# helloybz/CLANE

Hardware: AMD Instinct MI355X
Metric: embedding-update iters/sec (Jacobi sweeps of Z <- X + gamma*P*Z, P frozen) (higher is better)
Workload: dtype f32; 1 GPU; R-MAT |V|=2000000 |E|=40000000 d=256 f32, gamma=0.76, CosineSimilarity (reference mode), seeds 3/4

## Files before the change

### clane_amd/_hip.py

```python
from __future__ import annotations

import abc
import ctypes as C
import os
import threading
from pathlib import Path
from typing import Optional

import torch

LIB_NAME = "libclane_hip.so"
LIB_PATH = Path(__file__).resolve().parent / LIB_NAME
ABI_VERSION = 5

SCORE_REFERENCE, SCORE_PER_EDGE, SCORE_RAW_DOT = 0, 1, 2
SPMM_SINKS_UNTOUCHED = 1
SPMM_TABLE_BEYOND_CACHE = 2
OWNED_EPILOGUE_AHEAD = 1 << 16
SCORE_FUSE_SOFTMAX = 1
SCORE_MODES = {"reference": SCORE_REFERENCE, "per_edge": SCORE_PER_EDGE, "raw_dot": SCORE_RAW_DOT}

_p, _i64, _i32 = C.c_void_p, C.c_int64, C.c_int32

SIGNATURES = {
    "clane_abi_version": (C.c_int, []),
    "clane_last_error": (C.c_char_p, []),
    "clane_build_info": (C.c_char_p, []),
    "clane_xcc_ids": (C.c_int, [_p, _i64, _i32, _p]),
    "clane_check_csr": (C.c_int, [_p, _p, _i64, _i64, _i64, _p, _p]),
    "clane_spmm_partials_len": (_i64, [_i64, _i64]),
    "clane_reduce_ws_len": (_i64, []),
    "clane_reduce_partials": (C.c_int, [_p, _i64, _p, _p, _p]),
    "clane_spmm_split_slab_len": (_i64, [_i64, _i32]),
    "clane_spmm_class_slab_len": (_i64, [_i64, _i32]),
    "clane_device_alloc": (C.c_int, [_i64, C.POINTER(_p)]),
    "clane_device_alloc_contiguous": (C.c_int, [_i64, C.POINTER(_p)]),
    "clane_device_free": (C.c_int, [_p]),
    "clane_ipc_export": (C.c_int, [_p, _p]),
    "clane_ipc_open": (C.c_int, [_p, C.POINTER(_p)]),
    "clane_ipc_close": (C.c_int, [_p]),
}
IPC_HANDLE_BYTES = 64
for _s in ("f32", "f64", "bf16"):
    SIGNATURES[f"clane_row_sqnorm_{_s}"] = (C.c_int, [_p, _i64, _i32, _i64, _p, _p])
    SIGNATURES[f"clane_edge_score_{_s}"] = (
        C.c_int, [_p, _p, _i64, _i64, _p, _i64, _i32, _i32, _p, _p, _p, _i32, _i64, _p, _i64, _p])
    _g = C.c_double if _s == "f64" else C.c_float
    SIGNATURES[f"clane_spmm_update_{_s}"] = (
        C.c_int, [_p, _p, _p, _i64, _i64, _p, _i64, _p, _i64, _g, _p, _i64, _i32, _i64, _i32, _p, _p, _p])
    SIGNATURES[f"clane_spmm_update_long_{_s}"] = (
        C.c_int, [_p, _p, _p, _p, _i64, _i32, _i64, _p, _i64, _p, _i64, _g, _p, _i64, _i32, _p, _p, _p])
    SIGNATURES[f"clane_spmm_update_split_{_s}"] = (
        C.c_int,
        [_p, _p, _p, _p, _p, _p, _i64, _i64, _i64, _i64, _p, _i64, _p, _i64, _g, _p, _i64, _i32, _p, _p, _p, _p])
    SIGNATURES[f"clane_spmm_update_class_{_s}"] = (
        C.c_int,
        [_p, _p, _p, _p, _p, _i64, _i32, _p, _p, _i64, _i64, _p, _i64, _p, _i64, _g, _p, _i64, _i32, _i32, _p, _p, _p, _p])
    SIGNATURES[f"clane_edge_score_class_{_s}"] = (
        C.c_int, [_p, _p, _p, _p, _p, _p, _i64, _i32, _p, _p, _i64, _i64, _p, _i64, _i32, _i32, _p, _p, _p, _i32, _p, _p])
    SIGNATURES[f"clane_gather_rows_{_s}"] = (C.c_int, [_p, _i64, _p, _i64, _i32, _p, _i64, _p])
    SIGNATURES[f"clane_l1_distance_{_s}"] = (C.c_int, [_p, _i64, _p, _i64, _i64, _i32, _p, _p, _p, _p])
SIGNATURES["clane_spmm_update_owned_f32"] = (
    C.c_int, [_p, _p, _p, _i32, _i64, _p, _i64, _p, _i64, C.c_float, _p, _i64, _i32, _i32, _p, _p])
SIGNATURES["clane_spmm_update_tiles_f32"] = (
    C.c_int, [_p, _p, _p, _i64, _i64, _p, _i64, _p, _i64, C.c_float, _p, _i64, _i32, _i32, _i64, _i32, _p, _i64, _p])
SIGNATURES["clane_spmm_update_class_tiles_f32"] = (
    C.c_int, [_p, _p, _p, _p, _p, _i64, _i32, _p, _p, _i64, _i64, _i64, _p, _i64, _p, _i64, C.c_float, _p, _i64, _i32, _i32,
              _i32, _p, _p, _i64, _p])
SIGNATURES["clane_spmm_update_owned_tiles_f32"] = (
    C.c_int, [_p, _p, _p, _i32, _i64, _p, _i64, _p, _i64, C.c_float, _p, _i64, _i32, _i32, _i32, _p, _i64, _p])
SIGNATURES["clane_row_weight_f32"] = SIGNATURES["clane_row_weight_f64"] = (C.c_int, [_p, _p, _i64, _p, _p, _p])
SIGNATURES["clane_spmm_update_rw_f32"] = (
    C.c_int, [_p, _p, _p, _i64, _i64, _p, _i64, _p, _i64, C.c_float, _p, _i64, _i32, _i64, _i32, _p, _p])
SIGNATURES["clane_spmm_update_tiles_rw_f32"] = SIGNATURES["clane_spmm_update_tiles_f32"]
SIGNATURES["clane_spmm_update_class_rw_f32"] = (
    C.c_int, [_p, _p, _p, _p, _p, _p, _i64, _i32, _p, _p, _i64, _i64, _p, _i64, _p, _i64, C.c_float, _p, _i64, _i32, _i32, _p,
              _p, _p])
SIGNATURES["clane_spmm_update_class_tiles_rw_f32"] = (
    C.c_int, [_p, _p, _p, _p, _p, _p, _i64, _i32, _p, _p, _i64, _i64, _i64, _p, _i64, _p, _i64, C.c_float, _p, _i64, _i32,
              _i32, _i32, _p, _p, _i64, _p])
SIGNATURES["clane_spmm_update_owned_rw_f32"] = (
    C.c_int, [_p, _p, _p, _p, _i32, _i64, _p, _i64, _p, _i64, C.c_float, _p, _i64, _i32, _i32, _p, _p])
SIGNATURES["clane_spmm_update_owned_tiles_rw_f32"] = (
    C.c_int, [_p, _p, _p, _p, _i32, _i64, _p, _i64, _p, _i64, C.c_float, _p, _i64, _i32, _i32, _i32, _p, _i64, _p])
for _s in ("f32", "f64"):
    SIGNATURES[f"clane_degree_weighted_sums_{_s}"] = (C.c_int, [_p, _p, _p, _i64, _p, _p, _p])
    SIGNATURES[f"clane_edge_score_finalize_{_s}"] = (C.c_int, [_p, _p, _i64, _i64, _i32, _p, _p, _p, _p])
    SIGNATURES[f"clane_segment_softmax_{_s}"] = (C.c_int, [_p, _i64, _p, _i64, _i64, _p, _i64, _p])
    SIGNATURES[f"clane_pair_cosine_{_s}"] = (C.c_int, [_p, _i64, _p, _i64, _i64, _i32, _p, _p, _p])
    SIGNATURES[f"clane_edge_score_pair_{_s}"] = (
        C.c_int, [_p, _p, _i64, _i64, _p, _i64, _p, _i64, _i32, _p, _i32, _i64, _p, _i64, _p])
    SIGNATURES[f"clane_edge_score_class_pair_{_s}"] = (
        C.c_int, [_p, _p, _p, _p, _p, _p, _i64, _i32, _p, _p, _i64, _i64, _p, _i64, _p, _i64, _i32, _p, _i32, _p, _p])
for _s in ("f32", "f64", "bf16"):
    SIGNATURES[f"clane_project_rows_{_s}"] = (C.c_int, [_p, _i64, _i32, _i64, _p, _p, _i64, _p])
    SIGNATURES[f"clane_pair_project_{_s}"] = (C.c_int, [_p, _i64, _i32, _i64, _p, _p, _i64, _p, _p, _p, _p])
    SIGNATURES[f"clane_pair_grad_{_s}"] = (C.c_int, [_p, _i64, _i32, _i64, _p, _p, _i64, _p, _p, _p, _p, _p, _p, _p])
for _s in ("f32", "f64"):
    SIGNATURES[f"clane_pair_loss_{_s}"] = (C.c_int, [_p, _p, _i64, _i32, _p, _p, _p, _p, _p, _p, _p])
    SIGNATURES[f"clane_adam_step_{_s}"] = (C.c_int, [_p, _p, _p, _p, _i64, C.c_double, _p, _p, _p])
SIGNATURES["clane_pair_grad_ws_len"] = (_i64, [_i64, _i32])
RANK_MAX_K = 32
for _s in ("f32", "f64", "bf16"):
    SIGNATURES[f"clane_rank_scores_{_s}"] = (
        C.c_int, [_p, _i64, _p, _i64, _i64, _i32, _p, _i64, _i32, _p, _p, _p, _p, _p, _i32, _i32, _i32, _p, _p, _p])
    SIGNATURES[f"clane_pair_score_{_s}"] = (C.c_int, [_p, _i64, _p, _i64, _i64, _i32, _p, _p, _i64, _i32, _p, _p, _p, _p])
    SIGNATURES[f"clane_rank_count_{_s}"] = (
        C.c_int, [_p, _i64, _p, _i64, _i64, _i32, _p, _p, _i64, _i32, _p, _p, _p, _p, _p, _i32, _i32, _p, _p, _p])
for _s in ("f32", "f64"):
    SIGNATURES[f"clane_rank_merge_{_s}"] = (C.c_int, [_p, _p, _i64, _i32, _i32, _p, _p, _p])
SIGNATURES["clane_pair_labels"] = (C.c_int, [_p, _p, _i64, _p, _p, _i64, _p, _p])
PROBE_MAX_CLASSES = 64
PROBE_WRITE_G, PROBE_WRITE_PRED = 1, 2
PROBE_PRED_TOPK = 4
for _s in ("f32", "f64", "bf16"):
    SIGNATURES[f"clane_probe_forward_{_s}"] = (
        C.c_int, [_p, _i64, _i32, _i64, _p, _p, _i64, _p, _i64, _p, _p, _i32, _i32, _i32, _p, _p, _p, _p, _i64, _p])
    SIGNATURES[f"clane_probe_grad_{_s}"] = (C.c_int, [_p, _i64, _i32, _i64, _p, _i64, _p, _i32, _p, _p, _p, _p])
    SIGNATURES[f"clane_probe_forward_ovr_{_s}"] = (
        C.c_int, [_p, _i64, _i32, _i64, _p, _p, _i64, _p, _i64, _p, _p, _p, _i32, _i32, _i32, _i32, _p, _p, _p, _p, _i64, _p])
    SIGNATURES[f"clane_probe_predict_{_s}"] = (
        C.c_int, [_p, _i64, _i32, _i64, _p, _i64, _p, _p, _p, _i32, _i32, _i32, _i32, _p, _p, _p, _p])
PREDICT_SIGMOID, PREDICT_WRITE_PROBA = 1, 2
PREDICT_MAX_TOP = 8
SIGNATURES["clane_probe_loss_ws_len"] = (_i64, [_i64, _i32])
SIGNATURES["clane_probe_grad_ws_len"] = (_i64, [_i64, _i32, _i32])
for _s in ("f32", "f64", "bf16"):
    SIGNATURES[f"clane_kmeans_assign_{_s}"] = (
        C.c_int, [_p, _i64, _i32, _i64, _p, _i64, _p, _p, _i32, _i32, _p, _i64, _p, _i64, _p])
    SIGNATURES[f"clane_kmeans_update_{_s}"] = (
        C.c_int, [_p, _i64, _i32, _i64, _p, _p, _i64, _i32, _i32, _p, _p, _p, _p, _p])
SIGNATURES["clane_kmeans_update_ws_len"] = (_i64, [_i64, _i32, _i32, _i32])
MIXTURE_MAX_COMPONENTS = 64
MIXTURE_WRITE_RESP, MIXTURE_WRITE_ASSIGN = 1, 2
for _s in ("f32", "f64", "bf16"):
    SIGNATURES[f"clane_mixture_estep_{_s}"] = (
        C.c_int, [_p, _i64, _i32, _i64, _p, _i64, _p, _p, _p, _i32, _i32, _i32, _p, _p, _p, _p, _i64, _p])
    SIGNATURES[f"clane_mixture_mstep_{_s}"] = (C.c_int, [_p, _i64, _i32, _i64, _p, _i64, _p, _p, _i32, _p, _p, _p, _p])
SIGNATURES["clane_mixture_ll_ws_len"] = (_i64, [_i64, _i32])
SIGNATURES["clane_mixture_mstep_ws_len"] = (_i64, [_i64, _i32, _i32])
for _s in ("f32", "f64", "bf16"):
    _g = C.c_double if _s == "f64" else C.c_float
    SIGNATURES[f"clane_embed_rows_{_s}"] = (
        C.c_int, [_p, _p, _i64, _p, _i64, _p, _i64, _i64, _i32, _i32, _p, _p, _p, _i64, _g, _i32, _i32, _i32, _p, _i64,
                  _p, _p, _p, _p])

PCA_ACCUMULATE = 1
for _s in ("f32", "f64", "bf16"):
    SIGNATURES[f"clane_column_sums_{_s}"] = (C.c_int, [_p, _i64, _i32, _i64, _p, _i64, _i32, _p, _p, _p])
    SIGNATURES[f"clane_gram_{_s}"] = (C.c_int, [_p, _i64, _i32, _i64, _p, _i64, _p, _i32, _p, _p, _p])
    SIGNATURES[f"clane_project_affine_{_s}"] = (C.c_int, [_p, _i64, _i32, _i64, _p, _i64, _p, _p, _i32, _p, _i64, _p])
SIGNATURES["clane_column_sums_ws_len"] = (_i64, [_i64, _i32])
SIGNATURES["clane_gram_ws_len"] = (_i64, [_i64, _i32])
CSR_MAX_L = 512
SIGNATURES["clane_csr_spmm_segment"] = (C.c_int, [])
SIGNATURES["clane_csr_spmm_ws_len"] = (_i64, [_i64, _i64, _i32])
SIGNATURES["clane_csr_spmm_f32"] = (
    C.c_int, [_p, _p, _p, _i64, _i64, _p, _i64, _i64, _i32, _p, _p, _p, _p, _p, _i64, _i64, _p, _i64, _p, _i64, _p])
SIGNATURES["clane_csr_row_sums_f32"] = (C.c_int, [_p, _p, _i64, _i64, _p, _p, _p, _i64, _i64, _p, _i64, _p, _p])
TSNE_MAX_POINTS = 65536
TSNE_FORCES_KL, TSNE_FORCES_CACHED = 1, 2
for _s in ("f32", "bf16"):
    SIGNATURES[f"clane_tsne_sqdist_{_s}"] = (C.c_int, [_p, _i64, _i32, _i64, _p, _i64, _p, _p, _p, _p])
SIGNATURES["clane_tsne_affinities_f32"] = (C.c_int, [_p, _i64, C.c_float, _p, _p])
SIGNATURES["clane_tsne_symmetrize_ws_len"] = (_i64, [_i64])
SIGNATURES["clane_tsne_symmetrize_f32"] = (C.c_int, [_p, _i64, _p, _p])
SIGNATURES["clane_tsne_forces_f32"] = (C.c_int, [_p, _p, _i64, _i32, _p, _p])
# ... 390 lines not shown

    def mixture_mstep_ws_len(self, n: int, K: int, d: int) -> int:
        raise NotImplementedError(f"{type(self).__name__} has no mixture_mstep_ws_len")

    def mixture_mstep(self, Z, d: int, rows, mean, resp, ws, S, nk):
        raise NotImplementedError(f"{type(self).__name__} has no mixture_mstep")

    def column_sums_ws_len(self, n: int, d: int) -> int:
        raise NotImplementedError(f"{type(self).__name__} has no column_sums_ws_len")

    def column_sums(self, Z, d: int, rows, ws, sums, accumulate: bool = False):
        raise NotImplementedError(f"{type(self).__name__} has no column_sums")

    def gram_ws_len(self, n: int, d: int) -> int:
        raise NotImplementedError(f"{type(self).__name__} has no gram_ws_len")

    def gram(self, Z, d: int, rows, mu, ws, G, accumulate: bool = False):
        raise NotImplementedError(f"{type(self).__name__} has no gram")

    def project_affine(self, Z, d: int, rows, mu, W, Y):
        raise NotImplementedError(f"{type(self).__name__} has no project_affine")

    def csr_spmm_segment(self) -> int:
        raise NotImplementedError(f"{type(self).__name__} has no csr_spmm_segment")

    def csr_spmm_ws_len(self, n_rows: int, nnz: int, l: int) -> int:
        raise NotImplementedError(f"{type(self).__name__} has no csr_spmm_ws_len")

    def csr_spmm(self, S, B, l: int, out, a=None, s=None, ws=None):
        raise NotImplementedError(f"{type(self).__name__} has no csr_spmm")

    def csr_row_sums(self, S, sums, ws=None):
        raise NotImplementedError(f"{type(self).__name__} has no csr_row_sums")

    def tsne_sqdist(self, Z, d: int, rows, mu, sq, D):
        raise NotImplementedError(f"{type(self).__name__} has no tsne_sqdist")

    def tsne_affinities(self, D, perplexity: float, beta):
        raise NotImplementedError(f"{type(self).__name__} has no tsne_affinities")

    def tsne_symmetrize_ws_len(self, n: int) -> int:
        raise NotImplementedError(f"{type(self).__name__} has no tsne_symmetrize_ws_len")

    def tsne_symmetrize(self, P, partials):
        raise NotImplementedError(f"{type(self).__name__} has no tsne_symmetrize")

    def tsne_forces(self, P, Y, F, kl: bool = True, cached: bool = False):
        raise NotImplementedError(f"{type(self).__name__} has no tsne_forces")

    def tsne_step(self, F, Y, alpha: float, momentum: float, lr: float, plogp: float, V, G, Y_next, stats):
        raise NotImplementedError(f"{type(self).__name__} has no tsne_step")

    def knn_sqdist(self, Z, d: int, rows, mu, sq, ids, sqdist, n_slabs: int = 1, cand_ids=None, cand_sqdist=None):
        raise NotImplementedError(f"{type(self).__name__} has no knn_sqdist")

    def tsne_nn_affinities(self, sqdist, ids, perplexity: float, p, beta):
        raise NotImplementedError(f"{type(self).__name__} has no tsne_nn_affinities")

    def tsne_nn_plogp(self, rowptr, val, row_plogp):
        raise NotImplementedError(f"{type(self).__name__} has no tsne_nn_plogp")

    def tsne_nn_attract(self, rowptr, cols, val, Y, F, kl: bool = True):
        raise NotImplementedError(f"{type(self).__name__} has no tsne_nn_attract")

    def tsne_repulse(self, Y, F):
        raise NotImplementedError(f"{type(self).__name__} has no tsne_repulse")

    def silhouette_norms(self, Z, d: int, order, mu, metric: str, nrm):
        raise NotImplementedError(f"{type(self).__name__} has no silhouette_norms")

    def silhouette_sums(self, Z, d: int, order, seg, mu, nrm, metric: str, p0: int, p1: int, S):
        raise NotImplementedError(f"{type(self).__name__} has no silhouette_sums")

    def has_spmm_owned(self, dtype, d: int) -> bool:
        return False

    def make_owned_plan(self, plan: dict, chunk: int, device):
        raise NotImplementedError(f"{type(self).__name__} has no make_owned_plan")

    def spmm_update_owned(self, colidx, P, plan, block_threads: int, row0: int, Z_old, X, gamma: float, Z_new, d: int,
                          partials, beyond_cache: bool = False, loads: int = 0, ahead: bool = False):
        raise NotImplementedError(f"{type(self).__name__} has no spmm_update_owned")

    def has_spmm_tiles(self, dtype, d: int, tile_cols: int) -> bool:
        return False

    owned_epilogue_ahead = False

    def spmm_update_tiles(self, rowptr, colidx, P, nrows: int, row0: int, Z_old, X, gamma: float, Z_new, d: int,
                          tile_cols: int, long_threshold: int, partials, partials_stride: int,
                          sinks_untouched: bool = False, beyond_cache: bool = False):
        raise NotImplementedError(f"{type(self).__name__} has no spmm_update_tiles")

    def spmm_update_class_tiles(self, colidx, P, item_e0, item_len, item_slot, items_per_block: int, class_rows, slot_ptr,
                                n_slots: int, row0: int, Z_old, X, gamma: float, Z_new, d: int, tile_cols: int, slab,
                                partials, partials_stride: int, beyond_cache: bool = False):
        raise NotImplementedError(f"{type(self).__name__} has no spmm_update_class_tiles")

    def spmm_update_owned_tiles(self, colidx, P, plan, block_threads: int, row0: int, Z_old, X, gamma: float, Z_new,
                                d: int, tile_cols: int, partials, partials_stride: int, beyond_cache: bool = False,
                                loads: int = 0, ahead: bool = False):
        raise NotImplementedError(f"{type(self).__name__} has no spmm_update_owned_tiles")

    def has_row_weight(self, dtype) -> bool:
        return False

    def row_weight(self, rowptr, P, nrows: int, w, mixed):
        raise NotImplementedError(f"{type(self).__name__} has no row_weight")

    def bind(self, method: str, *args, **kwargs):
        fn = getattr(self, method)
        return lambda: fn(*args, **kwargs)

    def embed_rows(self, rowptr, colidx, X_new, Z, table_rows: int, d: int, mode: int, sums2, sq, S, gamma: float,
                   tolerence: int, max_rounds: int, Z_out, rounds, delta, P_out=None, flags: int = 0):
        raise NotImplementedError(f"{type(self).__name__} has no embed_rows")


class HipKernels(KernelBackend):

    owned_epilogue_ahead = True

    def __init__(self, lib: Optional[C.CDLL] = None):
        self.lib = lib if lib is not None else load_library()
        self._tls = threading.local()

    def _invoke(self, fn, what: str, *cargs):
        rec = getattr(self._tls, "recording", None)
        if rec is not None:
            rec.append((fn, cargs, what))
        else:
            self._check(fn(*cargs), what)

    def bind(self, method: str, *args, **kwargs):
        self._tls.recording = []
        try:
            getattr(self, method)(*args, **kwargs)
            (fn, cargs, what), = self._tls.recording
        finally:
            self._tls.recording = None
        check = self._check
        return lambda: check(fn(*cargs), what)

    def _check(self, rc: int, what: str):
        if rc != 0:
            raise ClaneHipError(f"{what} failed ({rc}): {self.lib.clane_last_error().decode()}")

    @staticmethod
    def _stream(t: torch.Tensor):
        if not t.is_cuda:
            raise ClaneHipError("HipKernels needs tensors in GPU memory (got a CPU tensor); there is no CPU path")
        return torch.cuda.current_stream(t.device).cuda_stream

    def _fn(self, base: str, dtype: torch.dtype):
        try:
            return getattr(self.lib, f"{base}_{_SUFFIX[dtype]}")
        except KeyError:
            raise TypeError(f"{base}: unsupported dtype {dtype}") from None

    def spmm_partials_len(self, nrows: int, n_long: int) -> int:
        return int(self.lib.clane_spmm_partials_len(nrows, n_long))

    def xcc_ids(self, n_blocks: int, block_threads: int = 256, device=None) -> torch.Tensor:
        out = torch.full((n_blocks,), -1, dtype=torch.int32, device=device if device is not None else "cuda")
        self._check(self.lib.clane_xcc_ids(out.data_ptr(), n_blocks, block_threads, self._stream(out)), "clane_xcc_ids")
        return out
# ... 256 lines not shown
        return _vec(w, torch.float32, "row_weight")

    def spmm_update_rw(self, rowptr, colidx, row_weight, nrows: int, row0: int, Z_old, X, gamma: float, Z_new, d: int,
                       long_threshold: int, partials, sinks_untouched: bool = False, beyond_cache: bool = False):
        zo, ldz, xp, ldx, zn, ldo = self._tables("spmm_update_rw", Z_old, X, Z_new, f32_only=True)
        self._invoke(self.lib.clane_spmm_update_rw_f32, "clane_spmm_update_rw",
                     _vec(rowptr, torch.int64, "rowptr"), _vec(colidx, torch.int32, "colidx"),
                     self._row_weights("spmm_update_rw", row_weight, nrows), nrows, row0, zo, ldz, xp, ldx, gamma, zn, ldo,
                     d, long_threshold, self._spmm_flags(sinks_untouched, beyond_cache),
                     _vec(partials, torch.float64, "partials"), self._stream(Z_old))

    def spmm_update_tiles_rw(self, rowptr, colidx, row_weight, nrows: int, row0: int, Z_old, X, gamma: float, Z_new,
                             d: int, tile_cols: int, long_threshold: int, partials, partials_stride: int,
                             sinks_untouched: bool = False, beyond_cache: bool = False):
        zo, ldz, xp, ldx, zn, ldo = self._tile_args("spmm_update_tiles_rw", Z_old, X, Z_new, d, tile_cols, partials,
                                                    partials_stride, self.spmm_partials_len(nrows, 0))
        self._invoke(self.lib.clane_spmm_update_tiles_rw_f32, "clane_spmm_update_tiles_rw",
                     _vec(rowptr, torch.int64, "rowptr"), _vec(colidx, torch.int32, "colidx"),
                     self._row_weights("spmm_update_tiles_rw", row_weight, nrows), nrows, row0, zo, ldz, xp, ldx, gamma,
                     zn, ldo, d, tile_cols, long_threshold, self._spmm_flags(sinks_untouched, beyond_cache),
                     _vec(partials, torch.float64, "partials"), partials_stride, self._stream(Z_old))

    def spmm_update_class_rw(self, colidx, row_weight, item_e0, item_len, item_slot, item_row, items_per_block: int,
                             class_rows, slot_ptr, row0: int, Z_old, X, gamma: float, Z_new, d: int, slab, partials,
                             beyond_cache: bool = False):
        zo, ldz, xp, ldx, zn, ldo = self._tables("spmm_update_class_rw", Z_old, X, Z_new, f32_only=True)
        n_blocks = self._item_blocks("spmm_update_class_rw", items_per_block, item_e0, item_len, item_slot, item_row)
        rows = int(class_rows.max()) + 1 if class_rows.numel() else 0
        self._invoke(self.lib.clane_spmm_update_class_rw_f32, "clane_spmm_update_class_rw",
                     _vec(colidx, torch.int32, "colidx"), self._row_weights("spmm_update_class_rw", row_weight, rows),
                     _vec(item_e0, torch.int64, "item_e0"), _vec(item_len, torch.int32, "item_len"),
                     _vec(item_slot, torch.int32, "item_slot"), _vec(item_row, torch.int32, "item_row"), n_blocks,
                     items_per_block, _vec(class_rows, torch.int32, "class_rows"), _vec(slot_ptr, torch.int64, "slot_ptr"),
                     class_rows.numel(), row0, zo, ldz, xp, ldx, gamma, zn, ldo, d,
                     self._spmm_flags(beyond_cache=beyond_cache), _vec(slab, torch.float32, "slab"),
                     _vec(partials, torch.float64, "partials"), self._stream(Z_old))

    def spmm_update_class_tiles_rw(self, colidx, row_weight, item_e0, item_len, item_slot, item_row, items_per_block: int,
                                   class_rows, slot_ptr, n_slots: int, row0: int, Z_old, X, gamma: float, Z_new, d: int,
                                   tile_cols: int, slab, partials, partials_stride: int, beyond_cache: bool = False):
        zo, ldz, xp, ldx, zn, ldo = self._tile_args("spmm_update_class_tiles_rw", Z_old, X, Z_new, d, tile_cols, partials,
                                                    partials_stride, class_rows.numel())
        n_blocks = self._item_blocks("spmm_update_class_tiles_rw", items_per_block, item_e0, item_len, item_slot, item_row)
        if slab.numel() < -(-d // tile_cols) * self.spmm_class_slab_len(n_slots, tile_cols):
            raise ValueError("spmm_update_class_tiles_rw: the slab does not hold every tile's chunk sums")
        rows = int(class_rows.max()) + 1 if class_rows.numel() else 0
        self._invoke(self.lib.clane_spmm_update_class_tiles_rw_f32, "clane_spmm_update_class_tiles_rw",
                     _vec(colidx, torch.int32, "colidx"), self._row_weights("spmm_update_class_tiles_rw", row_weight, rows),
                     _vec(item_e0, torch.int64, "item_e0"), _vec(item_len, torch.int32, "item_len"),
                     _vec(item_slot, torch.int32, "item_slot"), _vec(item_row, torch.int32, "item_row"), n_blocks,
                     items_per_block, _vec(class_rows, torch.int32, "class_rows"), _vec(slot_ptr, torch.int64, "slot_ptr"),
                     class_rows.numel(), n_slots, row0, zo, ldz, xp, ldx, gamma, zn, ldo, d, tile_cols,
                     self._spmm_flags(beyond_cache=beyond_cache), _vec(slab, torch.float32, "slab"),
                     _vec(partials, torch.float64, "partials"), partials_stride, self._stream(Z_old))

    def spmm_update_owned_rw(self, colidx, row_weight, plan: OwnedPlan, block_threads: int, row0: int, Z_old, X,
                             gamma: float, Z_new, d: int, partials, beyond_cache: bool = False, loads: int = 0,
                             ahead: bool = False):
        zo, ldz, xp, ldx, zn, ldo = self._tables("spmm_update_owned_rw", Z_old, X, Z_new, f32_only=True)
        self._owned_plan_fits("spmm_update_owned_rw", plan, d, colidx, colidx, row0, Z_old, X, Z_new, partials)
        self._invoke(self.lib.clane_spmm_update_owned_rw_f32, "clane_spmm_update_owned_rw",
                     _vec(colidx, torch.int32, "colidx"),
                     self._row_weights("spmm_update_owned_rw", row_weight, plan.max_row + 1),
                     C.cast(C.pointer(plan.c), _p), _vec(plan.seg_row, torch.int32, "seg_row"), int(block_threads), row0,
                     zo, ldz, xp, ldx, gamma, zn, ldo, d,
                     self._spmm_flags(beyond_cache=beyond_cache, loads=loads, ahead=ahead),
                     _vec(partials, torch.float64, "partials"), self._stream(Z_old))

    def spmm_update_owned_tiles_rw(self, colidx, row_weight, plan: OwnedPlan, block_threads: int, row0: int, Z_old, X,
                                   gamma: float, Z_new, d: int, tile_cols: int, partials, partials_stride: int,
                                   beyond_cache: bool = False, loads: int = 0, ahead: bool = False):
        zo, ldz, xp, ldx, zn, ldo = self._tile_args("spmm_update_owned_tiles_rw", Z_old, X, Z_new, d, tile_cols, partials,
                                                    partials_stride, plan.max_part + 1)
        if not self.has_spmm_owned(torch.float32, tile_cols):
            raise ValueError(f"spmm_update_owned_tiles_rw: no owned instance for tiles of {tile_cols} columns")
        self._owned_plan_fits("spmm_update_owned_tiles_rw", plan, tile_cols, colidx, colidx, row0, Z_old, X, Z_new)
        self._invoke(self.lib.clane_spmm_update_owned_tiles_rw_f32, "clane_spmm_update_owned_tiles_rw",
                     _vec(colidx, torch.int32, "colidx"),
                     self._row_weights("spmm_update_owned_tiles_rw", row_weight, plan.max_row + 1),
                     C.cast(C.pointer(plan.c), _p), _vec(plan.seg_row, torch.int32, "seg_row"), int(block_threads), row0,
                     zo, ldz, xp, ldx, gamma, zn, ldo, d, tile_cols,
                     self._spmm_flags(beyond_cache=beyond_cache, loads=loads, ahead=ahead),
                     _vec(partials, torch.float64, "partials"), partials_stride, self._stream(Z_old))

    def reduce_partials(self, partials, n: int, ws, out):
        self._invoke(self.lib.clane_reduce_partials, "clane_reduce_partials",
                     _vec(partials, torch.float64, "partials"), n, _vec(ws, torch.float64, "ws"),
                     _vec(out, torch.float64, "out"), self._stream(out))

    def l1_distance(self, A, B, d: int, ws, out, sq_a: Optional[torch.Tensor] = None):
        ap, lda = _mat(A, "A")
        bp, ldb = _mat(B, "B")
        self._check(self._fn("clane_l1_distance", A.dtype)(
            ap, lda, bp, ldb, A.shape[0], d, self._sq_arg(sq_a, A.dtype), _vec(ws, torch.float64, "ws"),
            _vec(out, torch.float64, "out"), self._stream(A)), "clane_l1_distance")

    def gather_rows(self, src, idx, d: int, dst):
        sp, lds = _mat(src, "src")
        dp, ldd = _mat(dst, "dst")
        self._invoke(self._fn("clane_gather_rows", src.dtype), "clane_gather_rows",
                     sp, lds, _vec(idx, torch.int32, "idx"), idx.numel(), d, dp, ldd, self._stream(src))

    def project_rows(self, Z, d: int, W, Y):
        zp, ldz = _mat(Z, "Z")
        yp, ldy = _mat(Y, "Y")
        acc = acc_dtype(Z.dtype)
        if tuple(W.shape) != (2 * d, d):
            raise ValueError(f"project_rows: W must be [2d, d] = [{2 * d}, {d}], got {tuple(W.shape)}")
        if Y.dtype != acc or Y.shape[0] < Z.shape[0]:
            raise ValueError(f"project_rows: Y must be {acc} with at least {Z.shape[0]} rows")
        self._check(self._fn("clane_project_rows", Z.dtype)(
            zp, Z.shape[0], d, ldz, _vec(W, acc, "W"), yp, ldy, self._stream(Z)), "clane_project_rows")

    def edge_score_pair(self, rowptr, colidx, nrows: int, row0: int, S, N, d: int, scores, long_threshold: int = 0,
                        long_rows=None, fuse_softmax: bool = False):
        sp, lds = _mat(S, "S")
        np_, ldn = _mat(N, "N")
        if S.dtype != N.dtype:
            raise ValueError("edge_score_pair: S and N must share a dtype")
        n_long = 0 if long_rows is None else long_rows.numel()
        self._check(self._fn("clane_edge_score_pair", S.dtype)(
            _vec(rowptr, torch.int64, "rowptr"), _vec(colidx, torch.int32, "colidx"), nrows, row0, sp, lds, np_, ldn, d,
            _vec(scores, S.dtype, "scores"), SCORE_FUSE_SOFTMAX if fuse_softmax else 0, long_threshold,
            None if n_long == 0 else _vec(long_rows, torch.int32, "long_rows"), n_long,
            self._stream(S)), "clane_edge_score_pair")

    def edge_score_class_pair(self, rowptr, colidx, item_e0, item_len, item_slot, item_row, items_per_block: int,
                              class_rows, slot_ptr, row0: int, S, N, d: int, scores, stats=None,
                              fuse_softmax: bool = False, n_slots: Optional[int] = None, row_parts: int = 1):
        sp, lds = _mat(S, "S")
        np_, ldn = _mat(N, "N")
        if S.dtype != N.dtype:
            raise ValueError("edge_score_class_pair: S and N must share a dtype")
        n_blocks = self._item_blocks("edge_score_class_pair", items_per_block, item_e0, item_len, item_slot, item_row)
        if fuse_softmax and (stats is None or stats.numel() < 2 * (int(slot_ptr[-1]) if n_slots is None else n_slots)):
            raise ValueError("edge_score_class_pair: stats needs 2 elements per slot")
        self._check(self._fn("clane_edge_score_class_pair", S.dtype)(
            _vec(rowptr, torch.int64, "rowptr"), _vec(colidx, torch.int32, "colidx"),
            _vec(item_e0, torch.int64, "item_e0"), _vec(item_len, torch.int32, "item_len"),
            _vec(item_slot, torch.int32, "item_slot"), _vec(item_row, torch.int32, "item_row"),
            n_blocks, items_per_block, _vec(class_rows, torch.int32, "class_rows"),
            _vec(slot_ptr, torch.int64, "slot_ptr"), class_rows.numel(), row0, sp, lds, np_, ldn, d,
            _vec(scores, S.dtype, "scores"),
            (SCORE_FUSE_SOFTMAX | ((max(1, min(255, int(row_parts))) & 0xff) << 8)) if fuse_softmax else 0,
            None if stats is None else _vec(stats, S.dtype, "stats"), self._stream(S)), "clane_edge_score_class_pair")

    @staticmethod
    def _pairs(src, dst, what: str) -> int:
        if src.numel() != dst.numel():
            raise ValueError(f"{what}: src and dst must have one entry per pair")
        return src.numel()

    def _pair_mats(self, A, Bm, B: int, d: int, acc, what: str):
        for t, name in ((A, "A"), (Bm, "Bm")):
            if t.dtype != acc or not t.is_contiguous() or t.numel() < B * d:
                raise ValueError(f"{what}: {name} must be a contiguous {acc} tensor of at least B * d elements")
        return A.data_ptr(), Bm.data_ptr()

    def pair_project(self, Z, d: int, src, dst, W, A, Bm):
        zp, ldz = _mat(Z, "Z")
        acc = acc_dtype(Z.dtype)
        B = self._pairs(src, dst, "pair_project")
        if tuple(W.shape) != (2 * d, d):
            raise ValueError(f"pair_project: W must be [2d, d] = [{2 * d}, {d}], got {tuple(W.shape)}")
        ap, bp = self._pair_mats(A, Bm, B, d, acc, "pair_project")
        self._invoke(self._fn("clane_pair_project", Z.dtype), "clane_pair_project",
# ... 616 lines not shown
```

### clane_amd/blocks.py

```python
from __future__ import annotations

import itertools
from dataclasses import dataclass
from typing import NamedTuple, Optional

import numpy as np
import torch


class ClassItems(NamedTuple):
    rows: torch.Tensor
    slot_ptr: torch.Tensor
    e0: torch.Tensor
    len: torch.Tensor
    slot: torch.Tensor
    row: torch.Tensor
    items_per_block: int

    @classmethod
    def upload(cls, items: dict, rows: np.ndarray, device) -> "ClassItems":
        up = lambda name: torch.from_numpy(items[name]).to(device)
        return cls(torch.from_numpy(rows.astype(np.int32)).to(device), up("slot_ptr"), up("e0"), up("len"), up("slot"),
                   up("row"), items["items_per_block"])


class SplitRows(NamedTuple):
    rows: torch.Tensor
    seg_ptr: torch.Tensor
    seg_row: torch.Tensor


class OwnedRows(NamedTuple):
    plan: object
    rest: Optional[ClassItems]
    n_rest: int


@dataclass(frozen=True)
class PartialLayout:
    main: int
    mid: int
    hub: int
    split: int
    klass: int
    end: int

    @classmethod
    def of(cls, row_pass: int, n_mid: int, n_hub: int, n_split: int, n_class: int, length: int) -> "PartialLayout":
        starts = list(itertools.accumulate((row_pass, n_mid, n_hub, n_split, n_class), initial=0))
        assert starts[-1] == length, (starts, length)
        return cls(*starts)

    def owned(self, n_rest: int) -> int:
        return self.klass + n_rest

    def owned_slots(self, n_rest: int, n_owned: int) -> np.ndarray:
        assert self.owned(n_rest) + n_owned == self.end, (self, n_rest, n_owned)
        return self.owned(n_rest) - self.klass + np.arange(n_owned)


@dataclass
class BlockRows:
    long: Optional[torch.Tensor]
    k1_long: Optional[torch.Tensor]
    mid: Optional[torch.Tensor]
    hub: Optional[torch.Tensor]
    partials: PartialLayout
    split: Optional[SplitRows] = None
    klass: Optional[ClassItems] = None
    n_slots: int = 0
    owned: Optional[OwnedRows] = None
    owned_inputs: Optional[tuple] = None
```

### clane_amd/csrc/clane_abi.hip

```cpp
#include "../../include/clane_hip.h"

#include <hip/hip_runtime.h>

#include <climits>
#include <cstdarg>
#include <cstdio>
#include <cstring>

#include "build_p.h"
#include "content_pca.h"
#include "edge_score.h"
#include "device_utils.h"
#include "kmeans.h"
#include "label_predict.h"
#include "label_probe.h"
#include "multilabel_probe.h"
#include "new_rows.h"
#include "link_eval.h"
#include "link_rank.h"
#include "mixture.h"
#include "pair_train.h"
#include "projection.h"
#include "sparse_rows.h"
#include "spmm_update.h"
#include "silhouette.h"
#include "tsne.h"
#include "tsne_nn.h"

namespace {

using namespace clane;

thread_local char g_err[512] = "";

int fail(int code, const char *fmt, ...) {
    va_list ap;
    va_start(ap, fmt);
    vsnprintf(g_err, sizeof(g_err), fmt, ap);
    va_end(ap);
    return code;
}

int check_launch(const char *what) {
    const hipError_t e = hipGetLastError();
    if (e != hipSuccess) return fail(CLANE_ERR_LAUNCH, "%s: %s", what, hipGetErrorString(e));
    return CLANE_OK;
}

constexpr int kReduceGrid = 1024;
constexpr int64_t kReduceWs = 2 * kReduceGrid + 2;
#ifndef CLANE_LONG_U
#define CLANE_LONG_U CLANE_SPMM_U
#endif
#ifndef CLANE_SUBROW_U32
#define CLANE_SUBROW_U32 4
#endif
#ifndef CLANE_CLASS_U16B
#define CLANE_CLASS_U16B 4
#endif
#ifndef CLANE_CLASS_U32
#define CLANE_CLASS_U32 6
#endif
#ifndef CLANE_LONG_WAVES
#define CLANE_LONG_WAVES 16
#endif
constexpr int kLongWaves = CLANE_LONG_WAVES;
#ifndef CLANE_ROWS_PER_BLOCK
#define CLANE_ROWS_PER_BLOCK 32
#endif

inline bool aligned16(const void *p) { return (reinterpret_cast<uintptr_t>(p) & 15u) == 0; }

#ifndef CLANE_TARGET_GRID
#define CLANE_TARGET_GRID 32768
#endif
inline int rows_per_block(int64_t nrows) {
    const int64_t r = ceil_div(ceil_div(nrows, CLANE_TARGET_GRID), kWavesPerBlock) * kWavesPerBlock;
    return int(r < CLANE_ROWS_PER_BLOCK ? CLANE_ROWS_PER_BLOCK : r > kMaxRowsPerBlock ? kMaxRowsPerBlock : r);
}
inline int row_grid(int64_t nrows) { return int(ceil_div(nrows > 0 ? nrows : 1, rows_per_block(nrows))); }

inline int grid_for_waves(int64_t nwaves_wanted) {
    int64_t g = ceil_div(nwaves_wanted, kWavesPerBlock);
    if (g > kMaxGrid) g = kMaxGrid;
    if (g < 1) g = 1;
    return int(g);
}

struct Layout {
    bool vec;
    int lpr;
};

template <typename T>
Layout pick_layout(int d, std::initializer_list<const void *> ptrs, std::initializer_list<int64_t> lds) {
    constexpr int KV = Elem<T>::kVec;
    bool vec = true;
    for (const void *p : ptrs) vec = vec && aligned16(p);
    for (int64_t ld : lds) vec = vec && (ld % KV == 0);
    Layout L;
    L.vec = vec;
    if (vec) {
        const int packs = int(ceil_div(d, KV));
        L.lpr = packs <= 8 ? 8 : packs <= 16 ? 16 : packs <= 32 ? 32 : 64;
    } else {
        L.lpr = d <= 4 ? 4 : d <= 16 ? 16 : 64;
    }
    return L;
}

template <typename T, typename F>
void dispatch_layout(const Layout &L, F &&f) {
    constexpr int KV = Elem<T>::kVec;
    if (L.vec) {
        switch (L.lpr) {
            case 8: f.template operator()<KV, 8>(); break;
            case 16: f.template operator()<KV, 16>(); break;
            case 32: f.template operator()<KV, 32>(); break;
            default: f.template operator()<KV, 64>(); break;
        }
    } else {
        switch (L.lpr) {
            case 4: f.template operator()<1, 4>(); break;
            case 16: f.template operator()<1, 16>(); break;
            default: f.template operator()<1, 64>(); break;
        }
    }
}

template <typename T>
Mirror<T> make_mirror(const clane_mirror_t *m) {
    if (m == nullptr || m->row_ptr == nullptr) return Mirror<T>{nullptr, nullptr, nullptr, 0};
    return Mirror<T>{m->row_ptr, m->slot, reinterpret_cast<T *const *>(m->bufs), m->ld};
}
inline const void *mirror_alignment_probe(const clane_mirror_t *m, const void *aligned) {
    return (m && m->row_ptr && !m->aligned16) ? reinterpret_cast<const void *>(uintptr_t(1)) : aligned;
}
inline bool mirror_ok(const clane_mirror_t *m, int d) {
    return m == nullptr || m->row_ptr == nullptr || (m->slot != nullptr && m->bufs != nullptr && m->ld >= d);
}

// ... 375 lines not shown
            "spmm_update_split: null pointer");
    REQUIRE(!t.aliased(), "spmm_update_split: Z_new must not alias Z_old");
    REQUIRE(aligned16(slab), "spmm_update_split: slab must be 16-byte aligned");
    const Layout L = t.layout(d);
    const int64_t ld_slab = ceil_div(d, 8) * 8;
    dispatch_layout<T>(L, [&]<int VEC, int LPR>() {
        constexpr int U = VEC > 1 ? CLANE_LONG_U : 4;
        spmm_split_segment_kernel<T, PT, VEC, LPR, U, kLongWaves>
            <<<unsigned(n_segments), kLongWaves * kWave, 0, (hipStream_t)stream>>>(
                rowptr, colidx, P, split_rows, seg_ptr, seg_row, edges_per_segment, t.Z_old, t.ldz, d, slab, ld_slab);
        spmm_class_combine_kernel<T, VEC, LPR>
            <<<unsigned(ceil_div(n_split, kWave / LPR)), kCombineWaves * kWave, 0, (hipStream_t)stream>>>(
                split_rows, seg_ptr, n_split, row0, slab, ld_slab, t.Z_old, t.ldz, t.X, t.ldx, t.gamma, t.Z_new, t.ldo, d,
                t.mir(), false, delta_partials);
    });
    return check_launch("spmm_update_split");
}

template <typename T, typename PT, bool FUSED, bool UNIFORM = false>
int spmm_update_class_impl(const char *what, const int32_t *colidx, const PT *P, const int64_t *item_e0,
                           const int32_t *item_len, const int32_t *item_slot, int64_t n_blocks, int32_t items_per_block,
                           const int32_t *class_rows, const int64_t *slot_ptr, int64_t n_rows, int64_t n_slots,
                           int64_t row0, const Tables<T> &t, Tiles tiles, int32_t flags,
                           typename Elem<T>::acc_t *slab, double *delta_partials, void *stream,
                           const int32_t *item_row = nullptr) {
    const int32_t d = t.d;
    constexpr int kPad = FUSED ? 8 : 1;
    REQUIRE(t.mirror_complete(), "%s: incomplete mirror descriptor", what);
    REQUIRE(n_blocks >= 0 && n_blocks <= INT32_MAX - (FUSED ? 8 : 0) && n_rows >= 0 && n_rows <= INT32_MAX &&
                n_slots >= 0 && row0 >= 0 && d > 0, "%s: bad shape", what);
    if constexpr (FUSED) REQUIRE_TILES(T, d, tiles, what, true, "");
    REQUIRE(items_per_block >= kWavesPerBlock && items_per_block <= kMaxItemsPerBlock,
            "%s: items_per_block must be in [%d, %d]", what, kWavesPerBlock, kMaxItemsPerBlock);
    REQUIRE(t.wide_enough(), "%s: leading dimension < d", what);
    const int n_tiles = tile_count(d, tiles.cols);
    REQUIRE(tiles.part_stride >= (n_tiles > 1 ? n_rows : 0), "%s: the tiles' partials overlap", what);
    if (n_rows == 0) return CLANE_OK;
    REQUIRE(colidx && P && item_e0 && item_len && item_slot && class_rows && slot_ptr && t.present() && slab &&
                delta_partials, "%s: null pointer", what);
    if constexpr (UNIFORM) REQUIRE(item_row && t.mirror == nullptr, "%s: per-row weights need item_row and no mirror", what);
    REQUIRE(!t.aliased(), "%s: Z_new must not alias Z_old", what);
    REQUIRE(aligned16(slab), "%s: slab must be 16-byte aligned", what);
    const Layout L = t.layout(tiles.cols);
    if constexpr (FUSED) REQUIRE(L.vec, "%s: the tables must allow 16-byte packs", what);
    const int64_t ld_slab = ceil_div(tiles.cols, 8) * 8;
    const int64_t slab_stride = n_slots * ld_slab;
    const int chunk_blocks = int(ceil_div(n_blocks, kPad) * kPad);
    const bool beyond = (flags & CLANE_SPMM_TABLE_BEYOND_CACHE) != 0;
    REQUIRE(int64_t(n_tiles) * chunk_blocks <= INT32_MAX, "%s: grid too large", what);
    dispatch_layout<T>(L, [&]<int VEC, int LPR>() {
        constexpr int U = VEC > 1 ? CLANE_LONG_U : 4;
        constexpr int kDeepU = (LPR == 32 && VEC == 4 && sizeof(T) == 4) ? CLANE_CLASS_U32
                               : (LPR == 16 && VEC == 8 && sizeof(T) == 2) ? CLANE_CLASS_U16B : 0;
        const unsigned chunk_grid = unsigned(n_tiles) * unsigned(chunk_blocks);
        const int combine_blocks = int(ceil_div(n_rows, kWave / LPR));
        const unsigned combine_grid = unsigned(n_tiles) * unsigned(combine_blocks);
        auto chunks = [&]<int CU>() {
            if constexpr (!FUSED)
                spmm_class_chunk_kernel<T, PT, VEC, LPR, CU, UNIFORM><<<chunk_grid, kBlock, 0, (hipStream_t)stream>>>(
                    colidx, P, item_e0, item_len, item_slot, items_per_block, t.Z_old, t.ldz, d, slab, ld_slab, item_row);
            else if constexpr (VEC > 1)
                spmm_class_chunk_tiles_kernel<T, PT, VEC, LPR, CU, UNIFORM><<<chunk_grid, kBlock, 0, (hipStream_t)stream>>>(
                    colidx, P, item_e0, item_len, item_slot, int(n_blocks), items_per_block, t.Z_old, t.ldz, d, slab,
                    ld_slab, slab_stride, TileGrid{chunk_blocks, tiles.cols, 0}, item_row);
        };
        if (n_blocks > 0 && kDeepU > 0 && beyond) chunks.template operator()<(kDeepU > 0 ? kDeepU : U)>();
        else if (n_blocks > 0) chunks.template operator()<U>();
        if constexpr (!FUSED)
            spmm_class_combine_kernel<T, VEC, LPR><<<combine_grid, kCombineWaves * kWave, 0, (hipStream_t)stream>>>(
                class_rows, slot_ptr, n_rows, row0, slab, ld_slab, t.Z_old, t.ldz, t.X, t.ldx, t.gamma, t.Z_new, t.ldo, d,
                t.mir(), beyond, delta_partials);
        else if constexpr (VEC > 1)
            spmm_class_combine_tiles_kernel<T, VEC, LPR><<<combine_grid, kCombineWaves * kWave, 0, (hipStream_t)stream>>>(
                class_rows, slot_ptr, n_rows, row0, slab, ld_slab, slab_stride, t.Z_old, t.ldz, t.X, t.ldx, t.gamma,
                t.Z_new, t.ldo, d, beyond, TileGrid{combine_blocks, tiles.cols, tiles.part_stride}, delta_partials);
    });
    return check_launch(what);
}

constexpr int64_t kOwnedLdsReserve = 1024;
constexpr int64_t kLdsPerCU = 160 * 1024;
constexpr int64_t kLdsDefaultLimit = 64 * 1024;

template <typename T, typename PT, bool UNIFORM = false>
int spmm_update_owned_impl(const char *what, const int32_t *colidx, const PT *P, const clane_owned_plan_t *plan,
                           int32_t block_threads, int64_t row0, const Tables<T> &t, Tiles tiles, bool fused, int32_t flags,
                           double *delta_partials, void *stream, const int32_t *seg_row = nullptr) {
    using A = typename Elem<T>::acc_t;
    const int32_t d = tiles.cols;
    if (fused) REQUIRE_TILES(T, t.d, tiles, what, tiles.part_stride >= 0, ", the partials' stride >= 0");
    REQUIRE(plan, "spmm_update_owned: null plan");
    REQUIRE(plan->n_groups >= 0 && row0 >= 0 && d > 0, "spmm_update_owned: bad shape");
    REQUIRE(plan->n_steps >= 1 && plan->n_steps <= kOwnedMaxSteps, "spmm_update_owned: n_steps must be in [1, %d]",
            kOwnedMaxSteps);
    REQUIRE(plan->chunk >= kWave && plan->chunk % kWave == 0, "spmm_update_owned: chunk must be a positive multiple of 64");
    REQUIRE(block_threads >= kWave && block_threads <= kOwnedMaxBlock && block_threads % kWave == 0,
            "spmm_update_owned: block_threads must be a multiple of 64 in [64, %d]", kOwnedMaxBlock);
    REQUIRE(t.wide_enough(), "spmm_update_owned: leading dimension < d");
    REQUIRE(plan->max_batch_vrows >= 0, "spmm_update_owned: negative max_batch_vrows");
    if (plan->n_groups == 0) return CLANE_OK;
    REQUIRE(colidx && P && plan->grp_bat_ptr && plan->bat_vrow_ptr && plan->bat_row_ptr && plan->bat_seg_ptr &&
                plan->seg_e0 && plan->seg_len && plan->seg_vrow && plan->row_id && plan->row_part && plan->row_vptr &&
                t.present() && delta_partials,
            "spmm_update_owned: null pointer");
    if constexpr (UNIFORM) REQUIRE(seg_row, "spmm_update_owned: per-row weights need seg_row");
    REQUIRE(!t.aliased(), "spmm_update_owned: Z_new must not alias Z_old");
    const Layout L = t.layout(d);
    REQUIRE(L.vec && (L.lpr == 32 || L.lpr == 64) && d <= L.lpr * Elem<T>::kVec,
            "spmm_update_owned: no instance for d=%d with these operands (16-byte packs, 17..64 packs per row)", d);
    const int64_t lds = int64_t(plan->max_batch_vrows) * L.lpr * Elem<T>::kVec * int64_t(sizeof(A));
    REQUIRE(lds + kOwnedLdsReserve <= kLdsPerCU, "spmm_update_owned: %lld virtual rows per batch need %lld bytes of LDS",
            (long long)plan->max_batch_vrows, (long long)lds);
    const OwnedPlan op{plan->grp_bat_ptr, plan->bat_vrow_ptr, plan->bat_row_ptr, plan->bat_seg_ptr, plan->seg_e0,
                       plan->seg_len, plan->seg_vrow, plan->row_id, plan->row_part, plan->row_vptr, plan->n_steps,
                       plan->chunk};
    const bool beyond = (flags & CLANE_SPMM_TABLE_BEYOND_CACHE) != 0;
    int rc = CLANE_OK;
    auto launch = [&]<int VEC, int LPR, int U>() {
        auto *kernel = spmm_owned_kernel<T, PT, VEC, LPR, U, UNIFORM>;
        if (lds > kLdsDefaultLimit) {
            static int64_t granted = 0;
            if (lds > granted) {
                const hipError_t e = hipFuncSetAttribute(reinterpret_cast<const void *>(kernel),
                                                         hipFuncAttributeMaxDynamicSharedMemorySize, int(lds));
                if (e != hipSuccess) {
                    rc = fail(CLANE_ERR_LAUNCH, "spmm_update_owned: %lld bytes of LDS: %s", (long long)lds,
                              hipGetErrorString(e));
                    return;
                }
                granted = lds;
            }
        }
        kernel<<<unsigned(plan->n_groups), unsigned(block_threads), size_t(lds), (hipStream_t)stream>>>(
            colidx, P, op, row0, t.Z_old, t.ldz, t.X, t.ldx, t.gamma, t.Z_new, t.ldo, t.d, tiles.cols, tiles.part_stride,
            (flags & CLANE_OWNED_EPILOGUE_AHEAD) != 0, beyond, delta_partials, seg_row);
    };
    constexpr int KV = Elem<T>::kVec;
    const int asked = (flags >> 8) & 0xff;
    REQUIRE(asked == 0 || asked == 8 || asked == 12 || (L.lpr == 32 && asked == 6),
            "spmm_update_owned: no instance with %d row loads in flight", asked);
    const int loads = asked ? asked : (L.lpr == 32 && beyond) ? CLANE_CLASS_U32 : CLANE_LONG_U;
    if (L.lpr == 32) {
        if (loads == 6) launch.template operator()<KV, 32, 6>();
        else if (loads == 12) launch.template operator()<KV, 32, 12>();
        else launch.template operator()<KV, 32, 8>();
    } else {
        if (loads == 12) launch.template operator()<KV, 64, 12>();
        else launch.template operator()<KV, 64, 8>();
    }
    if (rc != CLANE_OK) return rc;
    return check_launch(what);
}

template <typename T>
int l1_distance(const T *A, int64_t lda, const T *B, int64_t ldb, int64_t nrows, int32_t d,
                typename Elem<T>::acc_t *sq_a, double *ws, double *out, void *stream) {
    REQUIRE(nrows >= 0 && d > 0 && lda >= d && ldb >= d, "l1_distance: bad shape");
    REQUIRE(ws && out, "l1_distance: null workspace/output");
    REQUIRE(nrows == 0 || (A && B), "l1_distance: null pointer");
    const Layout L = pick_layout<T>(d, {A, B}, {lda, ldb});
    if (sq_a != nullptr) {
        const Layout LA = pick_layout<T>(d, {A}, {lda});
        REQUIRE(LA.vec == L.vec && LA.lpr == L.lpr,
                "l1_distance: sq_a needs B as aligned as A (the lane layout of row_sqnorm on A)");
    }
    int grid = 1;
    dispatch_layout<T>(L, [&]<int VEC, int LPR>() {
        grid = grid_for_waves(ceil_div(nrows > 0 ? nrows : 1, (kWave / LPR) * stream_rows(LPR)));
        if (grid > kReduceGrid) grid = kReduceGrid;
        l1_distance_kernel<T, VEC, LPR><<<grid, kBlock, 0, (hipStream_t)stream>>>(A, lda, B, ldb, nrows, d, sq_a, ws);
    });
    reduce_fixed_kernel<<<1, 1024, 0, (hipStream_t)stream>>>(ws, grid, grid, 1, out);
    return check_launch("l1_distance");
}

template <typename T>
int gather_rows(const T *src, int64_t lds, const int32_t *idx, int64_t n, int32_t d, T *dst, int64_t ldd, void *stream) {
    REQUIRE(n >= 0 && d > 0 && lds >= d && ldd >= d, "gather_rows: bad shape");
    if (n == 0) return CLANE_OK;
    REQUIRE(src && idx && dst, "gather_rows: null pointer");
    const Layout L = pick_layout<T>(d, {src, dst}, {lds, ldd});
    dispatch_layout<T>(L, [&]<int VEC, int LPR>() {
        const int grid = grid_for_waves(ceil_div(n, kWave / LPR));
        gather_rows_kernel<T, VEC, LPR><<<grid, kBlock, 0, (hipStream_t)stream>>>(src, lds, idx, n, d, dst, ldd);
    });
    return check_launch("gather_rows");
}

template <typename T>
int pair_cosine(const T *A, int64_t lda, const T *B, int64_t ldb, int64_t nrows, int32_t d,
                typename Elem<T>::acc_t *out, double *ws, void *stream) {
    REQUIRE(nrows >= 0 && d > 0 && lda >= d && ldb >= d, "pair_cosine: bad shape");
    if (nrows == 0) return CLANE_OK;
    REQUIRE(A && B && out && ws, "pair_cosine: null pointer");
    const Layout L = pick_layout<T>(d, {A, B}, {lda, ldb});
    int grid = 1;
    dispatch_layout<T>(L, [&]<int VEC, int LPR>() {
        grid = grid_for_waves(ceil_div(nrows, kWave / LPR));
        if (grid > kReduceGrid) grid = kReduceGrid;
        pair_dot_kernel<T, VEC, LPR><<<grid, kBlock, 0, (hipStream_t)stream>>>(A, lda, B, ldb, nrows, d, out, ws);
    });
    double *sums2 = ws + 2 * kReduceGrid;
    reduce_fixed_kernel<<<1, 1024, 0, (hipStream_t)stream>>>(ws, grid, grid, 2, sums2);
    int sgrid = int(ceil_div(nrows, kBlock));
    if (sgrid > kMaxGrid) sgrid = kMaxGrid;
    pair_scale_kernel<typename Elem<T>::acc_t><<<sgrid, kBlock, 0, (hipStream_t)stream>>>(out, nrows, sums2);
    return check_launch("pair_cosine");
}

template <typename T, typename A>
int pair_project(const T *Z, int64_t table_rows, int32_t d, int64_t ldz, const int32_t *src, const int32_t *dst,
                 int64_t B, const A *W, A *PA, A *PB, void *stream) {
    REQUIRE(table_rows >= 0 && B >= 0 && d > 0 && d <= 32768 && ldz >= d, "pair_project: bad shape rows=%lld B=%lld d=%d ldz=%lld",
            (long long)table_rows, (long long)B, d, (long long)ldz);
    if (B == 0) return CLANE_OK;
    REQUIRE(Z && src && dst && W && PA && PB, "pair_project: null pointer");
    const int n_tiles = int(ceil_div(int64_t(d), int64_t(kProjBN)));
    const int64_t blocks = ceil_div(B, int64_t(kProjBM)) * n_tiles;
    REQUIRE(blocks <= INT32_MAX, "pair_project: %lld pairs is too many for one launch", (long long)B);
    pair_project_kernel<T, A><<<dim3(unsigned(blocks), 2), kBlock, 0, (hipStream_t)stream>>>(
        Z, table_rows, d, ldz, src, dst, B, W, PA, PB, n_tiles);
    return check_launch("pair_project");
}

template <typename A>
int pair_loss(const A *PA, const A *PB, int64_t B, int32_t d, const uint8_t *linked, const A *u, A *g, uint8_t *mask,
              double *ws, double *stats, void *stream) {
    REQUIRE(B >= 0 && d > 0, "pair_loss: bad shape B=%lld d=%d", (long long)B, d);
    REQUIRE(ws && stats, "pair_loss: null workspace/output");
    REQUIRE(B == 0 || (PA && PB && linked && u && g && mask), "pair_loss: null pointer");
    int grid = int(ceil_div(B > 0 ? B : 1, kBlock / kPairLanes));
// ... 898 lines not shown
                                      const float *X, int64_t ldx, float gamma, float *Z_new, int64_t ldo, int32_t d,
                                      int32_t tile_cols, int32_t flags, float *slab, double *delta_partials,
                                      int64_t partials_tile_stride, void *stream) {
    return spmm_update_class_impl<float, float, true>("spmm_update_class_tiles", colidx, P, item_e0, item_len, item_slot,
                                                      n_blocks, items_per_block, class_rows, slot_ptr, n_rows, n_slots,
                                                      row0, TABLES(float), Tiles{tile_cols, partials_tile_stride}, flags,
                                                      slab, delta_partials, stream);
}
int clane_spmm_update_owned_tiles_f32(const int32_t *colidx, const float *P, const clane_owned_plan_t *plan,
                                      int32_t block_threads, int64_t row0, const float *Z_old, int64_t ldz,
                                      const float *X, int64_t ldx, float gamma, float *Z_new, int64_t ldo, int32_t d,
                                      int32_t tile_cols, int32_t flags, double *delta_partials,
                                      int64_t partials_tile_stride, void *stream) {
    return spmm_update_owned_impl<float, float>("spmm_update_owned_tiles", colidx, P, plan, block_threads, row0,
                                                TABLES(float), Tiles{tile_cols, partials_tile_stride}, true, flags,
                                                delta_partials, stream);
}
int clane_row_weight_f32(const int64_t *rowptr, const float *P, int64_t nrows, float *row_weight, int32_t *mixed,
                         void *stream) {
    return row_weights<float>(rowptr, P, nrows, row_weight, mixed, stream);
}
int clane_row_weight_f64(const int64_t *rowptr, const double *P, int64_t nrows, double *row_weight, int32_t *mixed,
                         void *stream) {
    return row_weights<double>(rowptr, P, nrows, row_weight, mixed, stream);
}
int clane_spmm_update_rw_f32(const int64_t *rowptr, const int32_t *colidx, const float *row_weight, int64_t nrows,
                             int64_t row0, const float *Z_old, int64_t ldz, const float *X, int64_t ldx, float gamma,
                             float *Z_new, int64_t ldo, int32_t d, int64_t long_threshold, int32_t flags,
                             double *delta_partials, void *stream) {
    return spmm_update_impl<float, float, false, true>("spmm_update_rw", rowptr, colidx, row_weight, nrows, row0,
                                                       TABLES(float), Tiles{d, 0}, long_threshold, flags, delta_partials,
                                                       stream);
}
int clane_spmm_update_tiles_rw_f32(const int64_t *rowptr, const int32_t *colidx, const float *row_weight, int64_t nrows,
                                   int64_t row0, const float *Z_old, int64_t ldz, const float *X, int64_t ldx, float gamma,
                                   float *Z_new, int64_t ldo, int32_t d, int32_t tile_cols, int64_t long_threshold,
                                   int32_t flags, double *delta_partials, int64_t partials_tile_stride, void *stream) {
    return spmm_update_impl<float, float, true, true>("spmm_update_tiles_rw", rowptr, colidx, row_weight, nrows, row0,
                                                      TABLES(float), Tiles{tile_cols, partials_tile_stride}, long_threshold,
                                                      flags, delta_partials, stream);
}
int clane_spmm_update_class_rw_f32(const int32_t *colidx, const float *row_weight, const int64_t *item_e0,
                                   const int32_t *item_len, const int32_t *item_slot, const int32_t *item_row,
                                   int64_t n_blocks, int32_t items_per_block, const int32_t *class_rows,
                                   const int64_t *slot_ptr, int64_t n_rows, int64_t row0, const float *Z_old, int64_t ldz,
                                   const float *X, int64_t ldx, float gamma, float *Z_new, int64_t ldo, int32_t d,
                                   int32_t flags, float *slab, double *delta_partials, void *stream) {
    return spmm_update_class_impl<float, float, false, true>("spmm_update_class_rw", colidx, row_weight, item_e0, item_len,
                                                             item_slot, n_blocks, items_per_block, class_rows, slot_ptr,
                                                             n_rows, 0, row0, TABLES(float), Tiles{d, 0}, flags, slab,
                                                             delta_partials, stream, item_row);
}
int clane_spmm_update_class_tiles_rw_f32(const int32_t *colidx, const float *row_weight, const int64_t *item_e0,
                                         const int32_t *item_len, const int32_t *item_slot, const int32_t *item_row,
                                         int64_t n_blocks, int32_t items_per_block, const int32_t *class_rows,
                                         const int64_t *slot_ptr, int64_t n_rows, int64_t n_slots, int64_t row0,
                                         const float *Z_old, int64_t ldz, const float *X, int64_t ldx, float gamma,
                                         float *Z_new, int64_t ldo, int32_t d, int32_t tile_cols, int32_t flags,
                                         float *slab, double *delta_partials, int64_t partials_tile_stride,
                                         void *stream) {
    return spmm_update_class_impl<float, float, true, true>("spmm_update_class_tiles_rw", colidx, row_weight, item_e0,
                                                            item_len, item_slot, n_blocks, items_per_block, class_rows,
                                                            slot_ptr, n_rows, n_slots, row0, TABLES(float),
                                                            Tiles{tile_cols, partials_tile_stride}, flags, slab,
                                                            delta_partials, stream, item_row);
}
int clane_spmm_update_owned_rw_f32(const int32_t *colidx, const float *row_weight, const clane_owned_plan_t *plan,
                                   const int32_t *seg_row, int32_t block_threads, int64_t row0, const float *Z_old,
                                   int64_t ldz, const float *X, int64_t ldx, float gamma, float *Z_new, int64_t ldo,
                                   int32_t d, int32_t flags, double *delta_partials, void *stream) {
    return spmm_update_owned_impl<float, float, true>("spmm_update_owned_rw", colidx, row_weight, plan, block_threads, row0,
                                                      TABLES(float), Tiles{d, 0}, false, flags, delta_partials, stream,
                                                      seg_row);
}
int clane_spmm_update_owned_tiles_rw_f32(const int32_t *colidx, const float *row_weight, const clane_owned_plan_t *plan,
                                         const int32_t *seg_row, int32_t block_threads, int64_t row0, const float *Z_old,
                                         int64_t ldz, const float *X, int64_t ldx, float gamma, float *Z_new, int64_t ldo,
                                         int32_t d, int32_t tile_cols, int32_t flags, double *delta_partials,
                                         int64_t partials_tile_stride, void *stream) {
    return spmm_update_owned_impl<float, float, true>("spmm_update_owned_tiles_rw", colidx, row_weight, plan, block_threads,
                                                      row0, TABLES(float), Tiles{tile_cols, partials_tile_stride}, true,
                                                      flags, delta_partials, stream, seg_row);
}

int64_t clane_spmm_class_slab_len(int64_t n_slots, int32_t d) { return n_slots * (ceil_div(d, 8) * 8); }
int64_t clane_spmm_split_slab_len(int64_t n_segments, int32_t d) { return n_segments * (ceil_div(d, 8) * 8); }

CLANE_SPMM_WRAPPERS(f32, float, float, float, float)
CLANE_SPMM_WRAPPERS(f64, double, double, double, double)
CLANE_SPMM_WRAPPERS(bf16, uint16_t, bf16_t, float, float)
#undef CLANE_SPMM_WRAPPERS
#undef TABLES

int clane_reduce_partials(const double *partials, int64_t n, double *ws, double *out, void *stream) {
    if (n < 0 || !out || !ws || (n > 0 && !partials))
        return fail(CLANE_ERR_INVALID_ARGUMENT, "reduce_partials: bad arguments");
    if (n <= 8192) {
        reduce_fixed_kernel<<<1, 1024, 0, (hipStream_t)stream>>>(partials, n, n, 1, out);
    } else {
        const int64_t slice = ceil_div(n, kReduceGrid);
        const int grid = int(ceil_div(n, slice));
        reduce_slices_kernel<<<grid, kBlock, 0, (hipStream_t)stream>>>(partials, n, slice, ws);
        reduce_fixed_kernel<<<1, 1024, 0, (hipStream_t)stream>>>(ws, grid, grid, 1, out);
    }
    return check_launch("reduce_partials");
}

int clane_l1_distance_f32(const float *A, int64_t lda, const float *B, int64_t ldb, int64_t nrows, int32_t d,
                          float *sq_a, double *ws, double *out, void *stream) {
    return l1_distance<float>(A, lda, B, ldb, nrows, d, sq_a, ws, out, stream);
}
int clane_l1_distance_f64(const double *A, int64_t lda, const double *B, int64_t ldb, int64_t nrows, int32_t d,
                          double *sq_a, double *ws, double *out, void *stream) {
    return l1_distance<double>(A, lda, B, ldb, nrows, d, sq_a, ws, out, stream);
}
int clane_l1_distance_bf16(const uint16_t *A, int64_t lda, const uint16_t *B, int64_t ldb, int64_t nrows, int32_t d,
                           float *sq_a, double *ws, double *out, void *stream) {
    return l1_distance<bf16_t>(reinterpret_cast<const bf16_t *>(A), lda, reinterpret_cast<const bf16_t *>(B), ldb,
                               nrows, d, sq_a, ws, out, stream);
}

int clane_gather_rows_f32(const float *src, int64_t lds, const int32_t *idx, int64_t n, int32_t d, float *dst,
                          int64_t ldd, void *stream) {
    return gather_rows<float>(src, lds, idx, n, d, dst, ldd, stream);
}
int clane_gather_rows_f64(const double *src, int64_t lds, const int32_t *idx, int64_t n, int32_t d, double *dst,
                          int64_t ldd, void *stream) {
    return gather_rows<double>(src, lds, idx, n, d, dst, ldd, stream);
}
int clane_gather_rows_bf16(const uint16_t *src, int64_t lds, const int32_t *idx, int64_t n, int32_t d, uint16_t *dst,
                           int64_t ldd, void *stream) {
    return gather_rows<bf16_t>(reinterpret_cast<const bf16_t *>(src), lds, idx, n, d,
                               reinterpret_cast<bf16_t *>(dst), ldd, stream);
}

int clane_pair_cosine_f32(const float *A, int64_t lda, const float *B, int64_t ldb, int64_t nrows, int32_t d,
                          float *out, double *ws, void *stream) {
    return pair_cosine<float>(A, lda, B, ldb, nrows, d, out, ws, stream);
}
int clane_pair_cosine_f64(const double *A, int64_t lda, const double *B, int64_t ldb, int64_t nrows, int32_t d,
                          double *out, double *ws, void *stream) {
    return pair_cosine<double>(A, lda, B, ldb, nrows, d, out, ws, stream);
}

#define CLANE_PAIR_TRAIN_WRAPPERS(SUF, CT, T, AT)                                                                      \
    int clane_pair_project_##SUF(const CT *Z, int64_t table_rows, int32_t d, int64_t ldz, const int32_t *src,         \
                                 const int32_t *dst, int64_t B, const AT *W, AT *A, AT *Bm, void *stream) {           \
        return pair_project<T, AT>(reinterpret_cast<const T *>(Z), table_rows, d, ldz, src, dst, B, W, A, Bm,         \
                                   stream);                                                                           \
    }                                                                                                                 \
    int clane_pair_grad_##SUF(const CT *Z, int64_t table_rows, int32_t d, int64_t ldz, const int32_t *src,            \
                              const int32_t *dst, int64_t B, const AT *A, const AT *Bm, const AT *g,                  \
                              const double *stats, AT *ws, AT *dW, void *stream) {                                    \
        return pair_grad<T, AT>(reinterpret_cast<const T *>(Z), table_rows, d, ldz, src, dst, B, A, Bm, g, stats, ws, \
                                dW, stream);                                                                          \
    }
CLANE_PAIR_TRAIN_WRAPPERS(f32, float, float, float)
CLANE_PAIR_TRAIN_WRAPPERS(f64, double, double, double)
CLANE_PAIR_TRAIN_WRAPPERS(bf16, uint16_t, bf16_t, float)
#undef CLANE_PAIR_TRAIN_WRAPPERS
#define CLANE_PAIR_LOSS_WRAPPERS(SUF, AT)                                                                              \
    int clane_pair_loss_##SUF(const AT *A, const AT *Bm, int64_t B, int32_t d, const uint8_t *linked, const AT *u,    \
                              AT *g, uint8_t *mask, double *ws, double *stats, void *stream) {                        \
        return pair_loss<AT>(A, Bm, B, d, linked, u, g, mask, ws, stats, stream);                                     \
    }                                                                                                                 \
    int clane_adam_step_##SUF(AT *W, AT *m, AT *v, const AT *dW, int64_t n, double lr, const double *stats,           \
// ... 317 lines not shown
```

### clane_amd/csrc/spmm_update.h

```cpp
#pragma once

#include "device_utils.h"

#ifndef CLANE_SPMM_U
#define CLANE_SPMM_U 8
#endif
#ifndef CLANE_SPMM_DYNAMIC
#define CLANE_SPMM_DYNAMIC 1
#endif
#ifndef CLANE_COMBINE_WAVES
#define CLANE_COMBINE_WAVES 2
#endif
#ifndef CLANE_SPMM_PREFETCH
#define CLANE_SPMM_PREFETCH 1
#endif
#ifndef CLANE_SPMM_MIN_WAVES
#define CLANE_SPMM_MIN_WAVES 0
#endif

namespace clane {

template <typename A>
struct EdgeChunk {
    int c;
// ... 797 lines not shown
                }
            }
#pragma unroll 4
            for (; s < b; ++s) {
                const Pack<A, VEC> part = slab_load<A, VEC>(slab + s * ld_slab + c0);
#pragma unroll
                for (int k = 0; k < VEC; ++k) acc[k] += part.v[k];
            }
        }
        if constexpr (kCombineWaves > 1) {
            if (t0 > 0) __syncthreads();
            if (wave > 0) {
#pragma unroll
                for (int k = 0; k < VEC; ++k) s_part[wave - 1][lane][k] = acc[k];
            }
            __syncthreads();
        }
        if (wave == 0) {
            Pack<T, VEC> out{};
            if (ok) {
                if constexpr (kCombineWaves > 1) {
#pragma unroll
                    for (int w = 1; w < kCombineWaves; ++w) {
#pragma unroll
                        for (int k = 0; k < VEC; ++k) acc[k] += s_part[w - 1][lane][k];
                    }
                }
                const Pack<T, VEC> x = load_pack_stream<T, VEC>(X + r * ldx + c0);
                const Pack<T, VEC> zo = load_pack_stream<T, VEC>(Zold + (row0 + r) * ldz + c0);
                rsum += finish_pack<T, VEC>(x, zo, acc, gamma, true, Znew + r * ldo + c0, out, nt_store);
            }
            if (live) mirror_store<T, VEC, LPR>(mirror, r, c0, out, ok, sl, sub * LPR);
        }
    }
    if (wave == 0) {
        rsum = group_sum<LPR>(rsum);
        if (live && sl == 0) partials[i] = double(rsum);
    }
}

template <typename T, int VEC, int LPR>
__global__ __launch_bounds__(kCombineWaves *kWave) void spmm_class_combine_kernel(
    const int32_t *__restrict__ class_rows, const int64_t *__restrict__ slot_ptr, int64_t n_rows, int64_t row0,
    const typename Elem<T>::acc_t *__restrict__ slab, int64_t ld_slab, const T *__restrict__ Zold, int64_t ldz,
    const T *__restrict__ X, int64_t ldx, typename Elem<T>::acc_t gamma, T *__restrict__ Znew, int64_t ldo, int d,
    Mirror<T> mirror, bool nt_store, double *__restrict__ partials) {
    spmm_class_combine_block<T, VEC, LPR>(class_rows, slot_ptr, n_rows, row0, slab, ld_slab, Zold, ldz, X, ldx, gamma,
                                          Znew, ldo, d, mirror, nt_store, blockIdx.x, partials);
}

template <typename T, int VEC, int LPR>
__global__ __launch_bounds__(kCombineWaves *kWave) void spmm_class_combine_tiles_kernel(
    const int32_t *__restrict__ class_rows, const int64_t *__restrict__ slot_ptr, int64_t n_rows, int64_t row0,
    const typename Elem<T>::acc_t *__restrict__ slab, int64_t ld_slab, int64_t slab_stride, const T *__restrict__ Zold,
    int64_t ldz, const T *__restrict__ X, int64_t ldx, typename Elem<T>::acc_t gamma, T *__restrict__ Znew, int64_t ldo,
    int d, bool nt_store, TileGrid tg, double *__restrict__ partials) {
    const int tile = tg.tile();
    const int block = int(blockIdx.x) - tile * tg.per_tile;
    const int c = tile * tg.tile_cols;
    spmm_class_combine_block<T, VEC, LPR>(class_rows, slot_ptr, n_rows, row0, slab + tile * slab_stride, ld_slab, Zold + c,
                                          ldz, X + c, ldx, gamma, Znew + c, ldo, tg.width(tile, d),
                                          Mirror<T>{nullptr, nullptr, nullptr, 0}, nt_store, block,
                                          partials + tile * tg.part_stride);
}

constexpr int kOwnedMaxSteps = 64;
constexpr int kOwnedMaxBlock = 1024;

struct OwnedPlan {
    const int32_t *grp_bat_ptr;
    const int32_t *bat_vrow_ptr;
    const int32_t *bat_row_ptr;
    const int32_t *bat_seg_ptr;
    const int64_t *seg_e0;
    const int32_t *seg_len;
    const int32_t *seg_vrow;
    const int32_t *row_id;
    const int32_t *row_part;
    const int32_t *row_vptr;
    int n_steps;
    int chunk;
};

template <typename T, typename PT, int VEC, int LPR, int U, bool UNIFORM = false>
__global__ __launch_bounds__(kOwnedMaxBlock) void spmm_owned_kernel(
    const int32_t *__restrict__ colidx, const PT *__restrict__ P, OwnedPlan plan, int64_t row0,
    const T *__restrict__ Zold, int64_t ldz, const T *__restrict__ X, int64_t ldx, typename Elem<T>::acc_t gamma,
    T *__restrict__ Znew, int64_t ldo, int d_left, int tile_cols, int64_t part_stride, bool ahead, bool nt_store,
    double *__restrict__ partials, [[maybe_unused]] const int32_t *__restrict__ seg_row) {
    using A = typename Elem<T>::acc_t;
    constexpr int W = LPR * VEC;
    constexpr int kRows = kWave / LPR;
    extern __shared__ __align__(16) unsigned char s_owned_raw[];
    A *s_sum = reinterpret_cast<A *>(s_owned_raw);
    __shared__ int s_cnt[kOwnedMaxSteps];

    const int lane = lane_id();
    const int wave = __builtin_amdgcn_readfirstlane(threadIdx.x / kWave);
    const int nwaves = int(blockDim.x) / kWave;
    const int sub = lane / LPR, sl = lane % LPR;
    const int c0 = sl * VEC;
    const int n_steps = plan.n_steps;
    const int64_t chunk = plan.chunk;
    const int b0 = plan.grp_bat_ptr[blockIdx.x], b1 = plan.grp_bat_ptr[blockIdx.x + 1];

    for (; d_left > 0; d_left -= tile_cols, Zold += tile_cols, X += tile_cols, Znew += tile_cols, partials += part_stride) {
    const int d = d_left < tile_cols ? d_left : tile_cols;
    const bool col_ok = c0 < d;
    const T *zcol = Zold + (col_ok ? c0 : 0);
    for (int b = b0; b < b1; ++b) {
        const int v0 = plan.bat_vrow_ptr[b];
        const int nv = plan.bat_vrow_ptr[b + 1] - v0;
        for (int i = threadIdx.x; i < nv * W; i += int(blockDim.x)) s_sum[i] = A(0);
        if (int(threadIdx.x) < n_steps) s_cnt[threadIdx.x] = 0;
        __syncthreads();
        for (int s = 0; s < n_steps; ++s) {
            const int sa = plan.bat_seg_ptr[b * n_steps + s];
            const int n = plan.bat_seg_ptr[b * n_steps + s + 1] - sa;
            auto claim = [&]() -> int {
                int v = 0;
                if (lane == 0) v = atomicAdd(&s_cnt[s], 1);
                return __builtin_amdgcn_readfirstlane(v);
            };
            int cur = claim();
            int64_t e0 = 0, e1 = 0;
            int vr = 0;
            EdgeChunk<A> ch{0, A(0)};
            [[maybe_unused]] A w = A(0);
            if (cur < n) {
                e0 = plan.seg_e0[sa + cur];
                e1 = e0 + plan.seg_len[sa + cur];
                vr = plan.seg_vrow[sa + cur];
                ch = load_chunk<A, PT, UNIFORM>(colidx, P, e0, e0 + chunk < e1 ? e0 + chunk : e1);
                if constexpr (UNIFORM) w = A(P[seg_row[sa + cur]]);
            }
            while (cur < n) {
                const int nxt = claim();
                int64_t n0 = 0, n1 = 0;
                int vn = 0;
                EdgeChunk<A> chn{0, A(0)};
                [[maybe_unused]] A wn = A(0);
                if (nxt < n) {
                    n0 = plan.seg_e0[sa + nxt];
                    n1 = n0 + plan.seg_len[sa + nxt];
                    vn = plan.seg_vrow[sa + nxt];
                    chn = load_chunk<A, PT, UNIFORM>(colidx, P, n0, n0 + chunk < n1 ? n0 + chunk : n1);
                    if constexpr (UNIFORM) wn = A(P[seg_row[sa + nxt]]);
                }
                A *sum = s_sum + vr * W + c0;
                for (int64_t p = e0; p < e1; p += chunk) {
                    const int64_t pe = p + chunk < e1 ? p + chunk : e1;
                    A acc[VEC];
#pragma unroll
                    for (int k = 0; k < VEC; ++k) acc[k] = A(0);
                    gather_accumulate<T, PT, VEC, LPR, U, UNIFORM>(colidx, P, p, pe, zcol, ldz, col_ok, acc, ch, p == e0, w);
                    fold_subwaves<LPR>(acc);
                    if (col_ok && sub == 0) {
                        Pack<A, VEC> t = load_pack<A, VEC>(sum);
#pragma unroll
                        for (int k = 0; k < VEC; ++k) t.v[k] += acc[k];
                        store_pack<A, VEC>(sum, t);
                    }
                }
                cur = nxt;
                e0 = n0;
                e1 = n1;
                vr = vn;
                ch = chn;
                if constexpr (UNIFORM) w = wn;
            }
            __syncthreads();
        }
        const int r0 = plan.bat_row_ptr[b];
        const int nr = plan.bat_row_ptr[b + 1] - r0;
        if (ahead) {
            struct RowIds {
                int r, va, vb, part;
                bool live;
            };
            const int stride = nwaves * kRows;
            auto ids_of = [&](int j0) -> RowIds {
                RowIds m{0, 0, 0, 0, false};
                const int j = j0 + sub;
                if (j0 < nr && j < nr) {
                    m.r = plan.row_id[r0 + j];
                    m.va = plan.row_vptr[r0 + j] - v0;
                    m.vb = plan.row_vptr[r0 + j + 1] - v0;
                    m.part = plan.row_part[r0 + j];
                    m.live = true;
                }
                return m;
            };
            auto request = [&](const RowIds &m, Pack<T, VEC> &x, Pack<T, VEC> &zo) {
                if (m.live && col_ok) {
                    x = load_pack_stream<T, VEC>(X + int64_t(m.r) * ldx + c0);
                    zo = load_pack_stream<T, VEC>(Zold + (row0 + m.r) * ldz + c0);
                }
            };
            int j0 = wave * kRows;
            RowIds cur = ids_of(j0), nxt = ids_of(j0 + stride);
            Pack<T, VEC> x{}, zo{};
            request(cur, x, zo);
            for (; j0 < nr; j0 += stride) {
                const RowIds far = ids_of(j0 + 2 * stride);
                Pack<T, VEC> xn{}, zon{};
                request(nxt, xn, zon);
                A rsum = A(0);
                if (cur.live && col_ok) {
                    A acc[VEC];
                    const Pack<A, VEC> first = load_pack<A, VEC>(s_sum + cur.va * W + c0);
#pragma unroll
                    for (int k = 0; k < VEC; ++k) acc[k] = first.v[k];
                    for (int v = cur.va + 1; v < cur.vb; ++v) {
                        const Pack<A, VEC> t = load_pack<A, VEC>(s_sum + v * W + c0);
#pragma unroll
                        for (int k = 0; k < VEC; ++k) acc[k] += t.v[k];
                    }
                    Pack<T, VEC> out{};
                    rsum = finish_pack<T, VEC>(x, zo, acc, gamma, true, Znew + int64_t(cur.r) * ldo + c0, out, nt_store);
                }
                rsum = group_sum<LPR>(rsum);
                if (cur.live && sl == 0) partials[cur.part] = double(rsum);
                cur = nxt;
                nxt = far;
                x = xn;
                zo = zon;
            }
        } else
        for (int j0 = wave * kRows; j0 < nr; j0 += nwaves * kRows) {
            const int j = j0 + sub;
            const bool live = j < nr;
            const bool ok = live && col_ok;
            A rsum = A(0);
            if (ok) {
                const int64_t r = plan.row_id[r0 + j];
                const Pack<T, VEC> x = load_pack_stream<T, VEC>(X + r * ldx + c0);
                const Pack<T, VEC> zo = load_pack_stream<T, VEC>(Zold + (row0 + r) * ldz + c0);
                const int va = plan.row_vptr[r0 + j] - v0, vb = plan.row_vptr[r0 + j + 1] - v0;
                A acc[VEC];
                const Pack<A, VEC> first = load_pack<A, VEC>(s_sum + va * W + c0);
#pragma unroll
                for (int k = 0; k < VEC; ++k) acc[k] = first.v[k];
                for (int v = va + 1; v < vb; ++v) {
                    const Pack<A, VEC> t = load_pack<A, VEC>(s_sum + v * W + c0);
#pragma unroll
                    for (int k = 0; k < VEC; ++k) acc[k] += t.v[k];
                }
                Pack<T, VEC> out{};
                rsum = finish_pack<T, VEC>(x, zo, acc, gamma, true, Znew + r * ldo + c0, out, nt_store);
            }
            rsum = group_sum<LPR>(rsum);
            if (live && sl == 0) partials[plan.row_part[r0 + j]] = double(rsum);
        }
        __syncthreads();
    }
    }
}

}
```

### clane_amd/diagnostics.py

```python
from __future__ import annotations

import numpy as np

from .plan import lanes_per_row


class DiagnosticsMixin:

    def kernel_times_ms(self):
        t = np.array([(e0.elapsed_time(e4), e4.elapsed_time(e1), e1.elapsed_time(e2), e2.elapsed_time(e3))
                      for _, e0, e1, e2, e3, e4 in self.kernel_events]).reshape(-1, 4)
        self.kernel_events = []
        if not len(t):
            return {}
        per_sweep = t.reshape(-1, len(self.blocks), 4).sum(1).mean(0)
        return dict(zip(("split", "hub", "mid", "main"), per_sweep.tolist()))

    def collective_times_ms(self):
        ev, self.collective_events = self.collective_events, []
        if not ev:
            return {}
        t = np.array([(a.elapsed_time(b), b.elapsed_time(c)) for a, b, c in ev])
        return {"exchange_exposed": float(t[:, 0].mean()), "allreduce": float(t[:, 1].mean()), "sweeps_timed": len(ev)}

    def kernel_bytes(self):
        s, ps = self.Zcur.element_size(), self.P.element_size()
        deg = np.diff(self.local.rowptr)
        per_row = deg * (self.d * s + 4 + ps) + np.where(deg > 0, 3 * self.d * s, 0) + 8
        is_long = deg > self.long_threshold if self.long_threshold > 0 else np.zeros_like(deg, dtype=bool)
        is_class = deg > self.class_threshold if self.class_threshold > 0 else np.zeros_like(deg, dtype=bool)
        is_long = is_long | is_class
        is_split = (is_long & (deg > self.split_edges) if self.split_edges > 0 else np.zeros_like(is_long)) & ~is_class
        is_hub = is_long & (deg > self.hub_threshold) & ~is_split & ~is_class
        return {"main": int(per_row[~is_long].sum()) + 8,
                "mid": int(per_row[is_long & ~is_hub & ~is_split & ~is_class].sum()),
                "hub": int(per_row[is_hub].sum()), "split": int(per_row[is_split | is_class].sum())}

    def launches_per_sweep(self) -> int:
        return len(self.blocks) * (1 if getattr(self, "fused_tiles", None) else len(self.tiles))

    def kernel_names(self):
        narrow = self.d > 0 and lanes_per_row(self.d_plan if len(self.tiles) > 1 else self.d, self.dtype) < 64
        fused = getattr(self, "fused_tiles", frozenset())
        return {"main": ("spmm_update_subrow" if narrow else "spmm_update") + ("_tiles_kernel" if "row" in fused else "_kernel"),
                "mid": "spmm_long_kernel<4 waves>", "hub": "spmm_long_kernel<16 waves>",
                "split": ("spmm_owned_kernel+spmm_class_chunk_kernel+combine" if getattr(self, "class_owned", False)
                          else "spmm_class_chunk_kernel+combine") if self.class_threshold > 0
                else "spmm_split_segment_kernel+combine"}

    def estimated_sweep_seconds(self) -> float:
        s = self.Zcur.element_size()
        d = self.d_full
        total = self.E_total * (d * s + 8) + self.V * 3 * d * s
        return total / max(self.world, 1) / 8e12

    def _sweeps_read_row_weights(self) -> bool:
        if getattr(self, "uniform_weights", False) is False or not getattr(self, "P_valid", False):
            return False
        return self._uniform if self._uniform is not None else self._resolve_uniform()

    def kernel_config(self) -> dict:
        return {"build": self.k.build_info(), "dtype": str(self.dtype).replace("torch.", ""), "d": self.d,
                "lanes_per_row": lanes_per_row(self.d, self.dtype) if self.d > 0 else 0,
                "rows": int(self.part.n_local), "edges": int(self.E_loc), "launch_blocks": len(self.blocks),
                "long_threshold": self.long_threshold, "score_threshold": self.score_threshold,
                "hub_threshold": self.hub_threshold,
                "split_edges": self.split_edges, "segment_edges": self.segment_edges,
                "class_threshold": self.class_threshold, "class_chunk": self.class_chunk, "class_k1": self.class_k1,
                "class_phases": self.class_phases, "phase_threshold": self.phase_threshold,
                "class_of_row": "xor-fold of 3-bit groups" if self.class_threshold else None,
                "class_affinity": self.class_affinity, "mega_segment_edges": self.mega_segment_edges,
                "class_items_per_block": [c.items_per_block for c in self.class_rows if c is not None][:1],
                "column_tiles": len(self.tiles),
                "fewer_loads_in_flight": bool(self.beyond_cache and self.d > 0 and (str(self.dtype), lanes_per_row(
                    self.d_plan if len(self.tiles) > 1 else self.d, self.dtype)) in (("torch.float32", 32), ("torch.bfloat16", 16))),
                "hot_rows_first": self.hot_rows_first, "exchange": self.exchange,
                **({"class_owned": {"max_edges": self.owned_max_edges, "row_edges": self.owned_row_edges,
                                    "groups": self.owned_groups, "block_threads": self.owned_block_threads,
                                    "batch_vrows": self.owned_batch_vrows, "chunk": self.owned_chunk,
                                    "loads": self.owned_loads}}
                   if getattr(self, "class_owned", False) else {}),
                **({"fused_tiles": sorted(self.fused_tiles)} if getattr(self, "fused_tiles", None) else {}),
                **({"owned_ahead": True} if getattr(self, "class_owned", False) and getattr(self, "owned_ahead", False)
                   else {}),
                **({"uniform_weights": True} if self._sweeps_read_row_weights() else {}),
                }

    def exchange_bytes_per_sweep(self) -> int:
        s = self.Zcur.element_size()
        if self.halo:
            return self.part.recv_rows_per_sweep() * self.ld * s
        if self.columns:
            return 0
        return sum((b.span[1] - b.span[0] - b.nrows) * self.ld * s for b in self.blocks if b.span is not None)
```

### clane_amd/engine.py

```python
from __future__ import annotations

import contextlib
import itertools
import threading
from typing import List, Optional

import numpy as np
import torch

from . import _hip, fused, owned, uniform, xcd
from .blocks import BlockRows, ClassItems, PartialLayout, SplitRows
from .comm import TorchComm
from .diagnostics import DiagnosticsMixin
from .halo import build_halo_layout
from .partition import Block, HostCSR, LocalCSR, RowPartition, localize
from .plan import (HEAVY_ROW_EDGES, HUB_FACTOR, INFINITY_CACHE_BYTES, L2_BYTES_ALL_XCDS,
                   LONG_THRESHOLD_BY_ROWS_PER_WAVE, MIN_HOT_READ_SHARE, MIN_SEGMENT_EDGES, MIN_SLICE_ROW_BYTES,
                   SOFTMAX_EDGES_PER_WORKGROUP, SPLIT_EDGES, TARGET_SEGMENTS, UNSKEWED_LONG_THRESHOLD, _round_up,
                   column_slice, hot_read_share, lanes_per_row, pick_exchange)
from .staging import StagedZ, StagingMixin, place_piece
from .xcd import (CLASS_CHUNK, CLASS_THRESHOLD_BY_ROWS_PER_WAVE, PHASE_THRESHOLD, PHASES_BY_ROWS_PER_WAVE,
                  class_items)

class SweepEngine(StagingMixin, DiagnosticsMixin):
    STAGE_SLOTS = 3
    N_TABLES = 3
    MAX_TIMED_SWEEPS = 32

    EXCHANGES = ("auto", "columns", "halo", "halo_p2p", "allgather", "allgather_all")

    def __init__(self, csr: HostCSR, X: torch.Tensor, device, kernels=None, *, cosine_mode: str = "reference",
                 process_group=None, chunks: Optional[int] = None, long_threshold: Optional[int] = None,
                 hub_threshold: Optional[int] = None, shuffle: Optional[bool] = None, seed: int = 0,
                 exchange: str = "auto", comm=None, hot_rows_first: bool = True, split_hubs: bool = True,
                 overlap_chunks: bool = True, fused_pack: bool = True, class_threshold: Optional[int] = None,
                 class_chunk: int = CLASS_CHUNK, class_k1: bool = True, class_phases: Optional[int] = None,
                 phase_threshold: int = PHASE_THRESHOLD, delta_stream: bool = False, table_skew=None,
                 table_alloc: str = "torch", column_tiles: Optional[int] = None, class_owned: Optional[bool] = None,
                 owned_max_edges: int = xcd.OWNED_MAX_EDGES, owned_row_edges: int = xcd.OWNED_ROW_EDGES,
                 owned_groups: int = xcd.OWNED_GROUPS, owned_lds_bytes: int = xcd.OWNED_LDS_BYTES,
                 owned_block_threads: int = xcd.OWNED_BLOCK_THREADS, owned_chunk: Optional[int] = None,
                 owned_loads: int = xcd.OWNED_LOADS, owned_ahead: Optional[bool] = None, fused_tiles=None,
                 uniform_weights=None):
        if X.dim() != 2 or X.shape[0] != csr.num_vertices:
            raise ValueError(f"X must be [V, d] with V={csr.num_vertices}, got {tuple(X.shape)}")
        if cosine_mode not in ("reference", "per_edge"):
            raise ValueError(f"cosine_mode must be 'reference' or 'per_edge', got {cosine_mode!r}")
        csr.validate()
        csr.indeg(device)
        self.k = kernels if kernels is not None else _hip.kernels()
        self.device = torch.device(device)
        self.dtype = X.dtype
        self.acc_dtype = _hip.acc_dtype(X.dtype)
        self.cosine_mode = cosine_mode
        self.table_skew = table_skew
        if table_alloc not in ("torch", "contiguous"):
            raise ValueError("table_alloc must be 'torch' or 'contiguous'")
        self.table_alloc, self._own_tables, self.table_alloc_note = table_alloc, [], None
        self._column_tiles_asked = column_tiles
        X = self._choose_division(csr, X, process_group, comm, exchange)
        self._choose_class_pass(csr, class_threshold, class_chunk, class_k1, class_phases, phase_threshold)
        self._choose_owned(class_owned, owned_max_edges, owned_row_edges, owned_groups, owned_lds_bytes,
                           owned_block_threads, owned_chunk)
        self.owned_loads = int(owned_loads)
        ahead = xcd.OWNED_EPILOGUE_AHEAD if owned_ahead is None else bool(owned_ahead)
        self.owned_ahead = bool(ahead and self.k.owned_epilogue_ahead)
        self._choose_fused_tiles(fused_tiles)
        self._choose_uniform(uniform_weights)
        self._build_layout(csr, chunks, shuffle, seed, hot_rows_first)
        self._choose_row_bins(long_threshold, hub_threshold)
        deg = self._upload_structure()
        self._bin_rows(deg, split_hubs)
        self._setup_exchange(deg, fused_pack)
        self._alloc_tables(X, deg)
        self._alloc_scratch(delta_stream, overlap_chunks)
        self._Y = None

    def _choose_division(self, csr: HostCSR, X: torch.Tensor, process_group, comm, exchange: str) -> torch.Tensor:
        self.pg = process_group
        self.comm = comm if comm is not None else (TorchComm(process_group) if process_group is not None else None)
        self.world = self.comm.world if self.comm is not None else 1
        rank = self.comm.rank if self.comm is not None else 0
        if exchange not in self.EXCHANGES:
            raise ValueError("exchange must be 'auto', 'columns', 'halo', 'halo_p2p', 'allgather' or "
                             f"'allgather_all', got {exchange!r}")
        self._forced = self.world == 1 and self.comm is not None and bool(self.comm.force) and exchange in (
            "columns", "allgather", "allgather_all")
        divided = self.world > 1 or self._forced
        if exchange == "auto":
            exchange = pick_exchange(int(X.shape[1]), X.dtype, self.world)
        self._exchange_asked = exchange
        self.exchange = exchange if divided else "none"
        self.columns = divided and exchange == "columns"
        self.C = self.world if self.columns else 1
        self.c = rank if self.columns else 0
        self.V, self.d_full = csr.num_vertices, int(X.shape[1])
        self.E_total = csr.num_edges
        self.col0, self.col1 = column_slice(self.d_full, X.dtype, self.C, self.c) if self.columns else (0, self.d_full)
        if self.columns:
            X = X[:, self.col0:self.col1]
            self.ld_max = _round_up(column_slice(self.d_full, X.dtype, self.C, 0)[1], _hip.VEC_ELEMS[X.dtype])
        self.d = self.col1 - self.col0
        self.ld = _round_up(self.d, _hip.VEC_ELEMS[X.dtype])
        self.row_world, self.row_rank = (1, 0) if self.columns else (self.world, rank)
        self.halo = self.row_world > 1 and exchange in ("halo", "halo_p2p")
        self.p2p = self.halo and exchange == "halo_p2p"
        if self.p2p and self.world > 8:
            raise ValueError("halo_p2p addresses at most 8 GPUs (one box)")
        self.d_plan = self.d
        if self.columns:
            c0, c1 = column_slice(self.d_full, X.dtype, self.C, 0)
            self.d_plan = c1 - c0
        T = self._pick_tiles(csr, X.dtype) if not divided else 1
        cuts = [column_slice(self.d, X.dtype, T, t) for t in range(T)] if self.d > 0 else [(0, 0)]
        self.tiles = [c for c in cuts if c[1] > c[0]] or [(0, self.d)]
        if len(self.tiles) > 1:
            self.d_plan = max(c1 - c0 for c0, c1 in self.tiles)
        self.beyond_cache = csr.num_vertices * self.ld * torch.empty(0, dtype=X.dtype).element_size() > 2 * INFINITY_CACHE_BYTES
        self.ld_plan = _round_up(self.d_plan, _hip.VEC_ELEMS[X.dtype])
        self.rows_per_wave = 64 // lanes_per_row(self.d_plan, X.dtype) if self.d_plan > 0 else 1
        return X

    def _pick_tiles(self, csr: HostCSR, dtype: torch.dtype) -> int:
        asked = self._column_tiles_asked
        if asked is not None:
            if asked < 1:
                raise ValueError("column_tiles must be >= 1")
            return int(asked)
        if dtype != torch.float32 or self.d < 256 or self.d % 128:
            return 1
        if csr.num_vertices * self.ld * 4 <= 2 * INFINITY_CACHE_BYTES:
            return 1
        return min(8, self.d // 128) if hot_read_share(csr, 512) >= MIN_HOT_READ_SHARE else 1

    def _choose_class_pass(self, csr: HostCSR, class_threshold, class_chunk, class_k1, class_phases,
                           phase_threshold) -> None:
        row_bytes = self.ld_plan * torch.empty(0, dtype=self.dtype).element_size()
        self.hot_read_share = hot_read_share(csr, row_bytes) if self.d_plan > 0 else 1.0
        self.class_affinity = True
        if class_threshold is None:
            class_threshold = CLASS_THRESHOLD_BY_ROWS_PER_WAVE[self.rows_per_wave]
            if self.rows_per_wave == 2 and csr.num_vertices * row_bytes <= INFINITY_CACHE_BYTES:
                class_threshold = max(class_threshold, 128)
            if self.hot_read_share < MIN_HOT_READ_SHARE:
                class_threshold = max(class_threshold, HEAVY_ROW_EDGES)
                self.class_affinity = False
        self.class_threshold = int(class_threshold)
        self.class_chunk = int(class_chunk)
        self.class_k1 = bool(class_k1) and self.class_threshold > 0
        if class_phases is None:
            class_phases = (xcd.PHASES_UNDER_COLUMN_TILES if len(self.tiles) > 1 else 0) or \
                PHASES_BY_ROWS_PER_WAVE[self.rows_per_wave]
        self.class_phases = int(class_phases)
        if self.class_threshold == 0 or self.class_phases < 1:
            self.class_phases = 1
        if self.class_phases & (self.class_phases - 1) or self.class_phases > 8:
            raise ValueError("class_phases must be 1, 2, 4 or 8")
        self.phase_threshold = max(int(phase_threshold), self.class_threshold) if self.class_phases > 1 else 0
        if self.class_threshold and not (64 <= self.class_chunk <= 4096 and self.class_chunk % 64 == 0):
            raise ValueError("class_chunk must be a multiple of 64 in [64, 4096]")
        self.mega_segment_edges = int(L2_BYTES_ALL_XCDS // 8 // max(row_bytes, 1)) if self.d_plan > 0 else 0

    def _choose_owned(self, class_owned, max_edges, row_edges, groups, lds_bytes, block_threads, chunk) -> None:
        can = owned.possible(self)
        want = (xcd.OWNED_DEFAULT and self.beyond_cache and self.class_affinity) if class_owned is None else bool(class_owned)
        self.class_owned, self.owned_possible = bool(want and can), bool(can)
        self._lds_bytes = int(lds_bytes)
        self.owned_max_edges, self.owned_row_edges = int(max_edges), int(row_edges)
        self.owned_groups, self.owned_block_threads = int(groups), int(block_threads)
        self.owned_chunk = int(chunk) if chunk is not None else self.class_chunk
        if self.class_owned:
            self._check_owned_settings()

    FUSED_PASSES = ("row", "class", "owned")

    def _choose_fused_tiles(self, asked) -> None:
        w = self.tiles[0][1] - self.tiles[0][0]
        even = all(c0 == t * w and c1 == c0 + w for t, (c0, c1) in enumerate(self.tiles))
        self.fused_possible = bool(len(self.tiles) > 1 and even and self.world == 1 and not self._forced
                                   and self.dtype == torch.float32
                                   and fused.backend_has(self, w))
        if asked is None:
            want = xcd.FUSED_TILES_DEFAULT
        elif isinstance(asked, bool):
            want = self.FUSED_PASSES if asked else ()
        else:
            want = tuple(asked)
            if any(p not in self.FUSED_PASSES for p in want):
                raise ValueError(f"fused_tiles: passes are {self.FUSED_PASSES}, got {asked!r}")
        self.fused_tiles = frozenset(want) if self.fused_possible else frozenset()

    def _choose_uniform(self, asked) -> None:
        if asked is None:
            asked = xcd.UNIFORM_WEIGHTS_DEFAULT if self.beyond_cache else False
        if asked not in (False, True, "auto"):
            raise ValueError(f"uniform_weights must be None, True, False or 'auto', got {asked!r}")
        self.uniform_possible = uniform.possible(self)
        if asked is True and not self.uniform_possible:
            raise ValueError("uniform_weights=True: one GPU, fp32 tables and a backend with the per-row-weight calls only")
        self.uniform_weights = asked if self.uniform_possible else False
        self._uniform = None

    def set_uniform_weights(self, asked) -> None:
        if self.device.type == "cuda":
            torch.cuda.synchronize(self.device)
        self._choose_uniform(asked)

    @property
    def P_valid(self) -> bool:
        return self._P_valid

    @P_valid.setter
    def P_valid(self, ok: bool) -> None:
        self._P_valid = bool(ok)
        self._uniform = None

    def _resolve_uniform(self) -> bool:
        self._uniform = uniform.resolve(self)
        return self._uniform

    def set_fused_tiles(self, on, ahead: Optional[bool] = None) -> None:
        if self.device.type == "cuda":
            torch.cuda.synchronize(self.device)
        self._choose_fused_tiles(on)
        if ahead is not None:
            self.owned_ahead = bool(ahead and self.k.owned_epilogue_ahead)
        self._plans = {}

    def _check_owned_settings(self) -> None:
        widths = [c1 - c0 for c0, c1 in self.tiles]
        if self.owned_groups < 1 or self.owned_row_edges < 64 or not (
                64 <= self.owned_block_threads <= 1024 and self.owned_block_threads % 64 == 0):
            raise ValueError("owned_groups must be >= 1, owned_row_edges >= 64, owned_block_threads a multiple of 64 "
                             "in [64, 1024]")
        if not (64 <= self.owned_chunk <= 4096 and self.owned_chunk % 64 == 0):
            raise ValueError("owned_chunk must be a multiple of 64 in [64, 4096]")
        sum_bytes = 16 * lanes_per_row(max(widths), self.dtype)
        self.owned_batch_vrows = self._lds_bytes // sum_bytes
        if self.owned_batch_vrows < 1 or self.owned_batch_vrows * sum_bytes > _hip.OWNED_LDS_LIMIT:
            raise ValueError(f"owned_lds_bytes must hold one sum of {sum_bytes} bytes and stay within "
                             f"{_hip.OWNED_LDS_LIMIT}")

    def _build_layout(self, csr: HostCSR, chunks, shuffle, seed: int, hot_rows_first: bool) -> None:
        if chunks is None:
            chunks = 1 if self.row_world == 1 else 4
        self.hot_rows_first = bool(hot_rows_first)
        if self.halo:
            self.part = build_halo_layout(csr, self.row_world, self.row_rank, chunks, shuffle=shuffle is not False, seed=seed,
                                          hot_rows_first=hot_rows_first, class_threshold=self.class_threshold,
                                          phase_threshold=self.phase_threshold, phases=self.class_phases)
            self.blocks: List[Block] = self.part.blocks
            self.local: LocalCSR = self.part.local
        else:
            live = csr.live_mask() if (self.row_world > 1 and self._exchange_asked == "allgather") else None
            hot = csr.indeg() if (self.row_world == 1 and hot_rows_first and not shuffle) else None
            self.part = RowPartition.create(self.V, self.row_world, self.row_rank, chunks, live_mask=live, shuffle=shuffle,
                                            seed=seed, priority=hot)
            self.blocks = self.part.blocks(spans_for_one_rank=self._forced and not self.columns)
            self.local = localize(csr, self.part, self.device, class_threshold=self.class_threshold,
                                  phase_threshold=self.phase_threshold, phases=self.class_phases)
        if self.part.padded_vertices >= 2 ** 31:
            raise ValueError(f"{self.part.padded_vertices} table rows: column indices are 32-bit (ABI v1); divide the "
                             "rows over more GPUs (exchange='halo') or wait for 64-bit indices")

    def _choose_row_bins(self, long_threshold, hub_threshold) -> None:
        if long_threshold is None:
            long_threshold = LONG_THRESHOLD_BY_ROWS_PER_WAVE[self.rows_per_wave]
            if self.rows_per_wave == 1 and self.class_threshold and self.class_affinity:
                long_threshold = max(long_threshold, self.class_threshold)
            elif self.rows_per_wave == 1 and not self.class_affinity:
                long_threshold = max(long_threshold, UNSKEWED_LONG_THRESHOLD)
            if self.rows_per_wave > 1:
                by_size = 1 << max(7, int(self.local.colidx.shape[0] // 32768).bit_length() - 1)
                long_threshold = min(long_threshold, by_size)
        self.score_threshold = int(long_threshold)
        self.k1_threshold = (min(self.score_threshold, self.class_threshold) if self.score_threshold > 0
                             else self.class_threshold) if self.class_k1 else self.score_threshold
        if self.class_threshold:
            long_threshold = min(long_threshold, self.class_threshold) if long_threshold > 0 else self.class_threshold
        self.long_threshold = int(long_threshold)
        self.hub_threshold = int(hub_threshold) if hub_threshold is not None else HUB_FACTOR * self.long_threshold

    def _upload_structure(self) -> np.ndarray:
        dev = self.device
        self.rowptr = torch.from_numpy(self.local.rowptr).to(dev)
        self.colidx = torch.from_numpy(self.local.colidx).to(dev)
        if self.colidx.numel() == 0:
            self.colidx = torch.zeros(1, dtype=torch.int32, device=dev)
        self.indeg = torch.from_numpy(self.local.indeg).to(dev)
        self.E_loc = int(self.local.colidx.shape[0])
        self.k.check_csr(self.rowptr, self.colidx, self.part.n_local, self.E_loc, self.part.padded_vertices)
        self.P = torch.zeros(max(self.E_loc, 1), dtype=self.acc_dtype, device=dev)
        self.P_valid = False
        deg = np.diff(self.local.rowptr)
        self.max_degree = int(deg.max()) if deg.size else 0
        self.softmax_row_parts = int(min(64, max(1, -(-self.max_degree // SOFTMAX_EDGES_PER_WORKGROUP))))
        return deg

    def _bin_rows(self, deg: np.ndarray, split_hubs: bool) -> None:
        dev = self.device
        self.block_rows: List[BlockRows] = []
        self.split_edges = SPLIT_EDGES if split_hubs else 0
        hub_edges = int(deg[deg > SPLIT_EDGES].sum()) // max(1, len(self.blocks))
        self.segment_edges = int(min(SPLIT_EDGES, max(MIN_SEGMENT_EDGES, hub_edges // TARGET_SEGMENTS // 1024 * 1024)))
        max_segments = max_slots = 0
        to_dev = lambda a: torch.from_numpy(a.astype(np.int32)).to(dev) if a.size else None
        for b in self.blocks:
            db = deg[b.local_start:b.local_start + b.nrows]
            is_long = db > self.long_threshold if self.long_threshold > 0 else np.zeros_like(db, dtype=bool)
            is_class = db > self.class_threshold if self.class_threshold > 0 else np.zeros_like(db, dtype=bool)
            is_long = is_long | is_class
            is_split = (is_long & (db > self.split_edges) if self.split_edges > 0 else np.zeros_like(is_long)) & ~is_class
            is_hub = is_long & (db > self.hub_threshold) & ~is_split & ~is_class
            is_mid = is_long & ~is_hub & ~is_split & ~is_class
            k1_long = (db > self.k1_threshold) & ~(is_class if self.class_k1 else np.zeros_like(is_class)) \
                if self.k1_threshold > 0 else np.zeros_like(is_class)
            rows_c, rows_s = np.nonzero(is_class)[0], np.nonzero(is_split)[0]
            layout = PartialLayout.of(row_pass=self.k.spmm_partials_len(b.nrows, 0), n_mid=int(is_mid.sum()),
                                      n_hub=int(is_hub.sum()), n_split=rows_s.size, n_class=rows_c.size,
                                      length=self.k.spmm_partials_len(b.nrows, int(is_long.sum())))
            rows = BlockRows(long=to_dev(np.nonzero(db > self.score_threshold)[0] if self.score_threshold > 0
                                         else np.empty(0, dtype=np.int64)),
                             k1_long=to_dev(np.nonzero(k1_long)[0]), mid=to_dev(np.nonzero(is_mid)[0]),
                             hub=to_dev(np.nonzero(is_hub)[0]), partials=layout)
            if rows_c.size:
                rows_abs = rows_c + b.local_start
                phased = dict(phase_threshold=self.phase_threshold, phases=self.class_phases,
                              mega_segment_edges=self.mega_segment_edges,
                              mega_min_edges=self.part.padded_vertices // 4)
                segments = xcd.row_segments(self.local.rowptr, self.local.colidx, rows_abs, self.colidx,
                                            self.phase_threshold, self.class_phases)
                items = class_items(self.local.rowptr, self.local.colidx, rows_abs, self.class_chunk, None,
                                    row_ids=rows_c, colidx_dev=self.colidx, segments=segments, **phased)
                if self.owned_possible:
                    rows.owned_inputs = (rows_c, rows_abs, segments, phased)
                if self.class_owned:
                    rows.owned = owned.plan_block(self, layout, *rows.owned_inputs)
                rows.klass, rows.n_slots = ClassItems.upload(items, rows_c, dev), int(items["slot_ptr"][-1])
                max_slots = max(max_slots, rows.n_slots)
            if rows_s.size:
                nseg = -(-db[rows_s] // self.segment_edges)
                seg_ptr = np.zeros(rows_s.size + 1, dtype=np.int64)
                np.cumsum(nseg, out=seg_ptr[1:])
                seg_row = np.repeat(np.arange(rows_s.size, dtype=np.int32), nseg)
                rows.split = SplitRows(to_dev(rows_s), torch.from_numpy(seg_ptr).to(dev), torch.from_numpy(seg_row).to(dev))
                max_segments = max(max_segments, int(seg_ptr[-1]))
            self.block_rows.append(rows)
        self.partials = torch.zeros(self.partial_off[-1] * len(self.tiles), dtype=torch.float64, device=dev)
        slab_len = max(1, self.k.spmm_split_slab_len(max_segments, max(self.d_plan, 1)))
        if max_slots:
            slab_len = max(slab_len, (len(self.tiles) if self.fused_possible else 1)
                           * self.k.spmm_class_slab_len(max_slots, max(self.d_plan, 1)), 2 * max_slots)
        self.slabs = [torch.zeros(slab_len, dtype=self.acc_dtype, device=dev)
                      for _ in range(2 if len(self.blocks) > 1 else 1)]

    def _per_block(name):
        return property(lambda self: [getattr(r, name) for r in self.block_rows])

    long_rows, k1_long_rows = _per_block("long"), _per_block("k1_long")
    mid_rows, hub_rows, split_rows = _per_block("mid"), _per_block("hub"), _per_block("split")
    class_rows, class_slots, owned_rows = _per_block("klass"), _per_block("n_slots"), _per_block("owned")
    del _per_block

    @property
    def partial_off(self) -> List[int]:
        return list(itertools.accumulate((r.partials.end for r in self.block_rows), initial=0))

    def set_owned(self, on: bool, **settings) -> None:
        if on and not self.owned_possible:
            raise ValueError("this engine has no owned pass: one GPU, fp32, rows or tiles of 65..256 elements")
        if self.device.type == "cuda":
            torch.cuda.synchronize(self.device)
        for name, value in settings.items():
            if name == "lds_bytes":
                self._lds_bytes = int(value)
            elif name in ("max_edges", "row_edges", "groups", "block_threads", "chunk", "loads"):
                setattr(self, "owned_" + name, int(value))
            else:
                raise TypeError(f"set_owned: unknown setting {name!r}")
        self.class_owned = bool(on)
        if on:
            self._check_owned_settings()
        for r in self.block_rows:
            r.owned = owned.plan_block(self, r.partials, *r.owned_inputs) if on and r.owned_inputs is not None else None
        self._plans = {}

    def _setup_exchange(self, deg: np.ndarray, fused_pack: bool) -> None:
        dev = self.device
        self.send_rows: List[Optional[torch.Tensor]] = []
        self.send_buf: List[Optional[torch.Tensor]] = []
        self.mirrors: List[Optional[object]] = []
        self.fused_pack = bool(fused_pack)
        for b in self.blocks:
            ex = b.exchange
            has = ex is not None and ex.send_rows.size > 0 and not self.p2p
            self.send_rows.append(torch.from_numpy(ex.send_rows).to(dev) if has else None)
            self.send_buf.append(torch.zeros(ex.send_rows.size, self.ld, dtype=self.dtype, device=dev) if has
                                 else (torch.zeros(0, self.ld, dtype=self.dtype, device=dev) if ex is not None else None))
            mirror = None
            if has and self.fused_pack:
                rel = ex.send_rows.astype(np.int64) - b.local_start
                if rel.min() < 0 or rel.max() >= b.nrows or (deg[ex.send_rows] == 0).any():
                    raise AssertionError("halo send list holds a row outside its chunk or a row that never changes")
                row_ptr = np.zeros(b.nrows + 1, dtype=np.int64)
                np.cumsum(np.bincount(rel, minlength=b.nrows), out=row_ptr[1:])
                slot = np.argsort(rel, kind="stable").astype(np.int32)
                mirror = self._make_mirror(torch.from_numpy(row_ptr).to(dev), torch.from_numpy(slot).to(dev),
                                           self.send_buf[-1])
            self.mirrors.append(mirror)

    def _new_table(self, tag: str, rows: int) -> torch.Tensor:
        skew = (self.table_skew or {}).get(tag)
        if self.table_alloc == "contiguous":
            try:
                buf = self.k.contiguous_matrix((rows, self.ld), self.dtype, self.device)
                self._own_tables.append(buf)
                return buf.tensor
            except _hip.ClaneHipError as exc:
                self.table_alloc_note = f"{tag}: {exc}"
        if skew is None or self.device.type != "cuda":
            return torch.zeros(rows, self.ld, dtype=self.dtype, device=self.device)
        es = torch.empty(0, dtype=self.dtype).element_size()
        nbytes = rows * self.ld * es
        raw = torch.zeros(nbytes + (4 << 20) + int(skew), dtype=torch.uint8, device=self.device)
        start = (-raw.data_ptr()) % (2 << 20) + int(skew)
        return raw[start:start + nbytes].view(self.dtype).view(rows, self.ld)

    def _alloc_tables(self, X: torch.Tensor, deg: np.ndarray) -> None:
        dev = self.device
        if self.halo:
            self.table_vertex = torch.from_numpy(self.part.table_vertex).to(dev)
            self.slot = torch.from_numpy(self.part.vertex_slot).to(dev)
        else:
            self.pos = torch.from_numpy(self.part.position_of_vertex()).to(dev)
        if self.p2p:
            self._shared = [self.k.shareable_matrix((self.part.padded_vertices, self.ld), self.dtype, dev)
                            for _ in range(self.N_TABLES)]
            self.Zbuf = [b.tensor for b in self._shared]
            self.peer_tables, self._mapped = self.comm.share_matrices(self.k, self._shared)
            self._build_p2p_mirrors(deg)
        else:
            self.Zbuf = [self._new_table(f"Z{i}", self.part.padded_vertices) for i in range(2)]
        self.cur, self.hold, self._prev_cur, self._tick = 0, None, 0, 0
        Xd = X.to(dev)
        verts = torch.from_numpy(self.local.vertex).to(dev)
        ok = verts >= 0
        self.X_loc = self._new_table("X", self.part.n_local)
        self.X_loc[ok, :self.d] = Xd[verts[ok]]
        self.quiet_stale = False
        self._load_Z(Xd)

    def _alloc_scratch(self, delta_stream: bool, overlap_chunks: bool) -> None:
        dev = self.device
        self.ws = torch.zeros(self.k.reduce_ws_len(), dtype=torch.float64, device=dev)
        self.sums2 = torch.zeros(2, dtype=torch.float64, device=dev)
        self.delta = torch.zeros(1, dtype=torch.float64, device=dev)
        self.delta_pp = torch.zeros(2, dtype=torch.float64, device=dev)
        self._delta_host = torch.zeros(2, dtype=torch.float64)
        self._delta_ev = None
        if self.device.type == "cuda":
            self._delta_host = self._delta_host.pin_memory()
            self._delta_ev = [torch.cuda.Event() for _ in range(2)]
        self._delta_stream = None
        self._delta_busy = [False, False]
        if self.device.type == "cuda" and (self.world > 1 or self._forced) and delta_stream:
            self._delta_stream = torch.cuda.Stream(self.device)
        self.block_out = torch.zeros(len(self.blocks), dtype=torch.float64, device=dev)
# ... 161 lines not shown
                    k.edge_score_class(rp, self.colidx, it.e0, it.len, it.slot, it.row, it.items_per_block, it.rows,
                                       it.slot_ptr, b.row0, Z, self.d, mode, self.sums2, sq, self.P,
                                       self.slabs[i % len(self.slabs)], fuse_softmax=True,
                                       n_slots=rows.n_slots, row_parts=self.softmax_row_parts)
        elif self.E_loc > 0:
            if busy:
                for b, rows in zip(self.blocks, self.block_rows):
                    k.edge_score(self.rowptr[b.local_start:], self.colidx, b.nrows, b.row0, Z, self.d,
                                 _hip.SCORE_RAW_DOT, None, None, self.P, self.k1_threshold, rows.k1_long)
                    if self.class_k1 and rows.klass is not None:
                        it = rows.klass
                        k.edge_score_class(self.rowptr[b.local_start:], self.colidx, it.e0, it.len, it.slot, it.row,
                                           it.items_per_block, it.rows, it.slot_ptr, b.row0, Z, self.d,
                                           _hip.SCORE_RAW_DOT, None, None, self.P)
            else:
                self.P.zero_()
            self._all_reduce(self.P)
            for b, rows in zip(self.blocks, self.block_rows):
                rp = self.rowptr[b.local_start:]
                k.edge_score_finalize(rp, self.colidx, b.nrows, b.row0, mode, self.sums2, sq, self.P)
                k.segment_softmax(rp, b.nrows, self.P, 0, self.score_threshold if rows.long is not None else 0,
                                  rows.long)
        self.P_valid = True

    def build_P_bilinear(self, W: torch.Tensor) -> None:
        from .bilinear import build_P_bilinear
        build_P_bilinear(self, W)

    def similarity_trainer(self, W0: torch.Tensor, lr: float, batch_size: int = 4):
        from .train import SimilarityTrainer
        return SimilarityTrainer(self, W0, lr, batch_size)

    def set_cosine_mode(self, mode: str) -> None:
        if mode not in ("reference", "per_edge"):
            raise ValueError(f"cosine_mode must be 'reference' or 'per_edge', got {mode!r}")
        if mode != self.cosine_mode:
            self.cosine_mode, self.P_valid = mode, False

    def P_global(self) -> torch.Tensor:
        out = torch.zeros(int(self.local.edge_origin.max()) + 1 if self.E_loc else 0, dtype=self.acc_dtype)
        out[torch.from_numpy(self.local.edge_origin)] = self.P[:self.E_loc].to("cpu")
        return out

    def _bind(self, method: str, *args, **kwargs):
        return self.k.bind(method, *args, **kwargs)

    def _build_plan(self, cur: int, dst: int, tick: int, gamma: float, per_row: bool = False):
        Zold, Znew = self.Zbuf[cur], self.Zbuf[dst]
        per_block = []
        partial_off = self.partial_off
        for i, (b, rows) in enumerate(zip(self.blocks, self.block_rows)):
            steps = []
            ctx = torch.cuda.stream(self.side_streams[i % 2]) if self.side_streams else contextlib.nullcontext()
            with ctx:
                rp, Xb, Zn = self.rowptr[b.local_start:], self.X_loc[self._rows(b)], self._zrows(Znew, b)
                po, lay = partial_off[i], rows.partials
                mir = self.mirrors_p2p[dst][i] if self.p2p else self.mirrors[i]
                w = self.row_w[b.local_start:] if per_row else None
                steps.append(("event", i, 0))
                if self.d == 0:
                    per_block.append(steps + [("event", i, e) for e in (4, 1, 2, 3)])
                    continue
                T = len(self.tiles)
                if mir is not None and T > 1:
                    raise AssertionError("column tiles and mirrored launches do not combine")
                cut = (lambda M, t: M) if T == 1 else (lambda M, t: M[:, self.tiles[t][0]:self.tiles[t][1]])
                cuts = [fused.Tables(cut(Zold, t), cut(Xb, t), cut(Zn, t), self.d if T == 1 else c1 - c0, t)
                        for t, (c0, c1) in enumerate(self.tiles)]
                on = self.fused_tiles if (T > 1 and mir is None) else frozenset()
                whole = fused.Tables(Zold, Xb, Zn, self.d, 0, (cuts[0].d,), (partial_off[-1],))
                slab = self.slabs[i % len(self.slabs)]

                def over_tiles(name, listed, start, bind):
                    call = lambda v: ("call", bind(v, self.partials[v.tile * partial_off[-1] + po + start:]))
                    if listed is None:
                        return [], [[]] * T
                    return ([call(whole)], [[]] * T) if name in on else ([], [[call(v)] for v in cuts])

                def long_rows(listed, waves, start):
                    return sum(over_tiles(None, listed, start, lambda v, p: self._bind(
                        "spmm_update_long", rp, self.colidx, self.P, listed, waves, b.row0, v.Zold, v.X, gamma, v.Znew, v.d,
                        p, mirror=mir))[1], [])
                own, split = rows.owned, rows.split
                klass = rows.klass if own is None else own.rest
                own_all, own_t = over_tiles("owned", own, lay.klass, lambda v, p: owned.bind_launch(
                    self, own.plan, b.row0, v, gamma, p, w))
                class_all, class_t = over_tiles("class", klass, lay.klass, lambda v, p: fused.bind_class(
                    self, klass, b.row0, v, gamma, slab, p, mir, w))
                _, split_t = over_tiles(None, split, lay.split, lambda v, p: self._bind(
                    "spmm_update_split", rp, self.colidx, self.P, split.rows, split.seg_ptr, split.seg_row,
                    self.segment_edges, b.row0, v.Zold, v.X, gamma, v.Znew, v.d, slab, p, mirror=mir))
                steps += own_all + class_all
                for t in range(T):
                    steps += own_t[t] + class_t[t] + split_t[t]
                steps.append(("event", i, 4))
                steps += long_rows(rows.hub, 16, lay.hub)
                steps.append(("event", i, 1))
                steps += long_rows(rows.mid, 4, lay.mid)
                steps.append(("event", i, 2))
                row_all, row_t = over_tiles("row", b, lay.main, lambda v, p: fused.bind_row(
                    self, rp, b.nrows, b.row0, v, gamma, p, mir, w))
                steps += sum(row_t, row_all)
                steps.append(("event", i, 3))
                if b.span is not None:
                    steps.append(("allgather", Znew[b.span[0]:b.span[1]], Zn))
                elif b.exchange is not None and not self.p2p:
                    ex = b.exchange
                    if self.send_rows[i] is not None and mir is None:
                        steps.append(("call", self._bind("gather_rows", Znew, self.send_rows[i], self.d,
                                                         self.send_buf[i])))
                    steps.append(("alltoall", Znew[ex.recv_start:ex.recv_start + ex.recv_rows], self.send_buf[i],
                                  ex.out_splits, ex.in_splits))
            per_block.append(steps)
        final = self._bind("reduce_partials", self.partials, self.partials.numel(), self.ws,
                           self.delta_pp[tick:tick + 1])
        return per_block, final

    def sweep(self, gamma: float) -> float:
        return self.sweep_wait(self.sweep_launch(gamma))

    def sweep_launch(self, gamma: float) -> int:
        if not self.P_valid:
            raise RuntimeError("sweep() before build_P()")
        stream = torch.cuda.current_stream(self.device).cuda_stream if self.device.type == "cuda" else 0
        src = self.cur
        dst = next(i for i in range(len(self.Zbuf)) if i != src and i != self.hold)
        parity = self._tick
        self._tick ^= 1
        if self._delta_stream is not None and self._delta_busy[parity]:
            torch.cuda.current_stream(self.device).wait_event(self._delta_ev[parity])
            self._delta_busy[parity] = False
        per_row = self._uniform if self._uniform is not None else self._resolve_uniform()
        key = (src, dst, parity, float(gamma), stream, per_row)
        plan = self._plans.get(key)
        if plan is None:
            plan = self._plans[key] = self._build_plan(src, dst, parity, float(gamma), per_row)
        events = None
        if self.time_kernels and len(self.kernel_events) < self.MAX_TIMED_SWEEPS * len(self.blocks):
            events = [[torch.cuda.Event(enable_timing=True) for _ in range(5)] for _ in self.blocks]
            self.kernel_events.extend((i,) + tuple(ev) for i, ev in enumerate(events))
        per_block, final = plan
        works = []
        side = self.side_streams
        if side:
            main = torch.cuda.current_stream(self.device)
            start = torch.cuda.Event()
            start.record(main)
            for st in side:
                st.wait_event(start)
        for i, steps in enumerate(per_block):
            ctx = torch.cuda.stream(side[i % 2]) if side else contextlib.nullcontext()
            with ctx:
                for step in steps:
                    kind = step[0]
                    if kind == "call":
                        step[1]()
                    elif kind == "event":
                        if events is not None:
                            events[step[1]][step[2]].record()
                    elif kind == "allgather":
                        works.append(self.comm.all_gather_into(step[1], step[2], async_op=True))
                    else:
                        works.append(self.comm.all_to_all_rows(step[1], step[2], step[3], step[4], async_op=True))
        if side:
            for st in side:
                done = torch.cuda.Event()
                done.record(st)
                main.wait_event(done)
        final()
        mine = self.delta_pp[parity:parity + 1]
        cev = None
        if self.time_collectives and self._delta_stream is None and len(self.collective_events) < self.MAX_TIMED_SWEEPS:
            cev = [torch.cuda.Event(enable_timing=True) for _ in range(3)]
            self.collective_events.append(cev)
            cev[0].record()
        for w in works:
            w.wait()
# ... 64 lines not shown
```

### clane_amd/fused.py

```python
from __future__ import annotations

from dataclasses import dataclass
from typing import Any


@dataclass(frozen=True)
class Tables:
    Zold: Any
    X: Any
    Znew: Any
    d: int
    tile: int = 0
    cols: tuple = ()
    strides: tuple = ()

    @property
    def fused(self) -> bool:
        return bool(self.cols)

    def method(self, per_tile: str, w=None) -> str:
        return per_tile + ("_tiles" if self.fused else "") + ("_rw" if w is not None else "")

    def mirrored(self, mirror) -> dict:
        assert not (self.fused and mirror is not None)
        return {} if self.fused else {"mirror": mirror}


def backend_has(eng, tile_cols: int) -> bool:
    return bool(eng.k.has_spmm_tiles(eng.dtype, eng.d, tile_cols))


def bind_row(eng, rowptr, nrows: int, row0: int, v: Tables, gamma: float, partials, mirror=None, w=None):
    assert w is None or mirror is None
    return eng._bind(v.method("spmm_update", w), rowptr, eng.colidx, eng.P if w is None else w, nrows, row0, v.Zold, v.X,
                     gamma, v.Znew, v.d, *v.cols, eng.long_threshold, partials, *v.strides, sinks_untouched=True,
                     **({} if w is not None else v.mirrored(mirror)), beyond_cache=eng.beyond_cache)


def bind_class(eng, items, row0: int, v: Tables, gamma: float, slab, partials, mirror=None, w=None):
    assert w is None or mirror is None
    n_slots = (int(items.slot_ptr[-1]),) if v.fused else ()
    item_row = () if w is None else (items.row,)
    return eng._bind(v.method("spmm_update_class", w), eng.colidx, eng.P if w is None else w, items.e0, items.len,
                     items.slot, *item_row, items.items_per_block, items.rows, items.slot_ptr, *n_slots, row0, v.Zold, v.X,
                     gamma, v.Znew, v.d, *v.cols, slab, partials, *v.strides,
                     **({} if w is not None else v.mirrored(mirror)), beyond_cache=eng.beyond_cache)
```

### clane_amd/owned.py

```python
from __future__ import annotations

from typing import Optional

import numpy as np

from . import xcd
from .blocks import ClassItems, OwnedRows, PartialLayout


def possible(eng) -> bool:
    widths = [c1 - c0 for c0, c1 in eng.tiles]
    return bool(eng.world == 1 and not eng._forced and eng.class_threshold > 0 and eng.d > 0
                and all(eng.k.has_spmm_owned(eng.dtype, w) for w in widths))


def plan_block(eng, layout: PartialLayout, rows_c: np.ndarray, rows_abs: np.ndarray, segments,
               phased: dict) -> Optional[OwnedRows]:
    dev = eng.device
    sizes, seg_len, seg_e0 = segments
    NS = seg_len.size // max(1, sizes.size)
    own = sizes <= eng.owned_max_edges
    if not own.any():
        return None
    n_rest = int((~own).sum())
    pick = lambda a, m: a.reshape(sizes.size, NS)[m].reshape(-1)
    plan = xcd.owned_plan(sizes[own], pick(seg_len, own), pick(seg_e0, own), rows_c[own],
                          layout.owned_slots(n_rest, int(own.sum())), row_edges=eng.owned_row_edges,
                          groups=eng.owned_groups, batch_vrows=eng.owned_batch_vrows)
    eng.owned_balance = plan["group_step_edges"]
    rest = None
    if n_rest:
        keep = ~own
        items = xcd.class_items(eng.local.rowptr, eng.local.colidx, rows_abs[keep], eng.class_chunk, None,
                                row_ids=rows_c[keep], segments=(sizes[keep], pick(seg_len, keep), pick(seg_e0, keep)),
                                **phased)
        rest = ClassItems.upload(items, rows_c[keep], dev)
    return OwnedRows(eng.k.make_owned_plan(plan, eng.owned_chunk, dev), rest, n_rest)


def bind_launch(eng, plan, row0: int, v, gamma: float, partials, w=None):
    ahead = {"ahead": True} if getattr(eng, "owned_ahead", False) else {}
    return eng._bind(v.method("spmm_update_owned", w), eng.colidx, eng.P if w is None else w, plan,
                     eng.owned_block_threads, row0, v.Zold, v.X, gamma, v.Znew, v.d, *v.cols, partials, *v.strides,
                     beyond_cache=eng.beyond_cache, loads=eng.owned_loads, **ahead)
```

### clane_amd/partition.py

```python
from __future__ import annotations

from dataclasses import dataclass, field
from typing import List, Optional, Tuple

import numpy as np

from .xcd import XCD_CLASSES, row_pieces, xcd_subclass


@dataclass
class HostCSR:
    num_vertices: int
    rowptr: np.ndarray
    colidx: np.ndarray
    _indeg: Optional[np.ndarray] = field(default=None, repr=False, compare=False)

    @property
    def num_edges(self) -> int:
        return int(self.colidx.shape[0])

    def validate(self) -> None:
        V, rp, ci = self.num_vertices, self.rowptr, self.colidx
        if rp.dtype != np.int64 or ci.dtype != np.int32 or rp.shape != (V + 1,) or ci.ndim != 1:
            raise ValueError("HostCSR: rowptr must be int64 [V + 1] and colidx int32 [E]")
# ... 57 lines not shown
            shuffle = world_size > 1
        if world_size == 1 or live_mask is None:
            live = np.ones(num_vertices, dtype=bool)
        else:
            live = np.asarray(live_mask, dtype=bool)
            if live.shape != (num_vertices,):
                raise ValueError("live_mask must have one entry per vertex")
        rng = np.random.default_rng(seed)
        slot = np.empty(num_vertices, dtype=np.int64)
        for mask in (live, ~live):
            ids = np.nonzero(mask)[0]
            if shuffle:
                order = rng.permutation(ids.size)
            elif priority is not None:
                order = np.argsort(-np.asarray(priority)[ids], kind="stable")
            else:
                order = np.arange(ids.size)
            slot[ids[order]] = np.arange(ids.size, dtype=np.int64)
        n_live, n_quiet = int(live.sum()), int((~live).sum())
        live_per_rank = max(1, -(-n_live // world_size))
        lc = -(-live_per_rank // chunks)
        q = -(-n_quiet // world_size)
        return cls(num_vertices, world_size, rank, chunks, lc, q, live_per_rank, slot, live)

    @property
    def live_total(self) -> int:
        return self.world_size * self.chunks * self.live_per_chunk

    @property
    def n_local(self) -> int:
        return self.chunks * self.live_per_chunk + self.quiet_per_rank

    @property
    def padded_vertices(self) -> int:
        return self.live_total + self.world_size * self.quiet_per_rank

    def _live_position(self, r, l):
        c, i = np.divmod(l, self.live_per_chunk)
        return c * (self.world_size * self.live_per_chunk) + r * self.live_per_chunk + i

    def position_of_vertex(self) -> np.ndarray:
        s = self.vertex_slot
        r_live, l_live = np.divmod(s, self.live_per_rank)
        pos_live = self._live_position(r_live, l_live)
        pos_quiet = self.live_total + s
        return np.where(self.vertex_live, pos_live, pos_quiet).astype(np.int64)

    def local_positions(self, rank: Optional[int] = None) -> np.ndarray:
        r = self.rank if rank is None else rank
        live = self._live_position(r, np.arange(self.chunks * self.live_per_chunk, dtype=np.int64))
        quiet = self.live_total + r * self.quiet_per_rank + np.arange(self.quiet_per_rank, dtype=np.int64)
        return np.concatenate([live, quiet])

    def blocks(self, spans_for_one_rank: bool = False) -> List[Block]:
        lc, w = self.live_per_chunk, self.world_size
        out = []
        for c in range(self.chunks):
            b = c * w * lc
            span = (b, b + w * lc) if (w > 1 or spans_for_one_rank) else None
            out.append(Block(c * lc, lc, b + self.rank * lc, span))
        if self.quiet_per_rank:
            out.append(Block(self.chunks * lc, self.quiet_per_rank,
                             self.live_total + self.rank * self.quiet_per_rank, None))
        return out

    def quiet_span(self) -> Optional[Tuple[int, int, int]]:
        if self.world_size == 1 or self.quiet_per_rank == 0:
            return None
        return self.live_total, self.padded_vertices, self.quiet_per_rank


@dataclass
class LocalCSR:
    rowptr: np.ndarray
    colidx: np.ndarray
    indeg: np.ndarray
    vertex: np.ndarray
    edge_origin: np.ndarray


LOCALIZE_PIECE_EDGES = 1 << 28


def edge_order(row_of, cols, sub, table_rows: int, n_sub: int = XCD_CLASSES, two_pass: Optional[bool] = None):
    import torch
    n_rows = int(row_of.max()) + 1 if row_of.numel() else 1
    width = table_rows * (n_sub if sub is not None else 1)
    if two_pass is None:
        two_pass = n_rows * width >= 2 ** 62
    if not two_pass:
        key = row_of * width + cols
        if sub is not None:
            key = key + sub * table_rows
        return torch.argsort(key)
    first = torch.argsort(cols, stable=True)
    major = row_of if sub is None else row_of * n_sub + sub
    return first[torch.argsort(major[first], stable=True)]


def localize(csr: HostCSR, part: RowPartition, device=None, class_threshold: int = 0, phase_threshold: int = 0,
             phases: int = 1) -> LocalCSR:
    V = csr.num_vertices
    if V != part.num_vertices:
        raise ValueError("partition built for a different vertex count")
    pos = part.position_of_vertex()
    vertex_at = np.full(part.padded_vertices, -1, dtype=np.int64)
    vertex_at[pos] = np.arange(V, dtype=np.int64)
    verts = vertex_at[part.local_positions()]
    valid = verts >= 0
    safe = np.where(valid, verts, 0)
    deg = np.where(valid, csr.outdeg()[safe], 0).astype(np.int64)
    rowptr = np.zeros(part.n_local + 1, dtype=np.int64)
    np.cumsum(deg, out=rowptr[1:])
    indeg = np.where(valid, csr.indeg()[safe], 0).astype(np.int32)
    by_class = deg > class_threshold if class_threshold > 0 else np.zeros_like(deg, dtype=bool)
    identity = (part.world_size == 1 and part.chunks == 1 and not by_class.any()
                and np.array_equal(pos, np.arange(V)))
    if identity:
        return LocalCSR(rowptr, csr.colidx.astype(np.int32), indeg, verts, np.arange(csr.num_edges, dtype=np.int64))
    import torch
    dev = torch.device(device) if device is not None and torch.device(device).type == "cuda" else torch.device("cpu")
    t = lambda a: torch.from_numpy(np.ascontiguousarray(a)).to(dev)
    pos_t, start_t = t(pos), t(csr.rowptr[safe])
    colidx_t = t(csr.colidx)
    E_loc = int(rowptr[-1])
    cols_out = np.empty(E_loc, dtype=np.int32)
    origin_out = np.empty(E_loc, dtype=np.int64)
    for a, b in row_pieces(rowptr, LOCALIZE_PIECE_EDGES):
        e0, e1 = int(rowptr[a]), int(rowptr[b])
        if e1 == e0:
            continue
        deg_t = t(deg[a:b])
        row_of = torch.repeat_interleave(torch.arange(b - a, device=dev), deg_t)
        origin = start_t[a:b][row_of] + (torch.arange(e1 - e0, device=dev) - (t(rowptr[a:b]) - e0)[row_of])
        cols = pos_t[colidx_t[origin].long()]
        sub = (xcd_subclass(cols, deg_t[row_of], class_threshold, phase_threshold, phases)
               if by_class[a:b].any() else None)
        order = edge_order(row_of, cols, sub, part.padded_vertices, XCD_CLASSES * max(1, phases))
        cols_out[e0:e1] = cols[order].to(torch.int32).cpu().numpy()
        origin_out[e0:e1] = origin[order].cpu().numpy()
    return LocalCSR(rowptr, cols_out, indeg, verts, origin_out)
```

### clane_amd/plan.py

```python
from __future__ import annotations

import numpy as np
import torch

from . import _hip
from .partition import HostCSR

LONG_THRESHOLD_BY_ROWS_PER_WAVE = {1: 32, 2: 1024, 4: 1024, 8: 512}
HUB_FACTOR = 1
SPLIT_EDGES = 4096
MIN_SEGMENT_EDGES = 1024
TARGET_SEGMENTS = 512
SOFTMAX_EDGES_PER_WORKGROUP = 1 << 17
L2_BYTES_ALL_XCDS = 8 * 4 * 1024 * 1024
INFINITY_CACHE_BYTES = 256 * 1024 * 1024
MIN_HOT_READ_SHARE = 0.2
HEAVY_ROW_EDGES = 4096
UNSKEWED_LONG_THRESHOLD = 128


def hot_read_share(csr: HostCSR, row_bytes: int) -> float:
    V, E = csr.num_vertices, csr.num_edges
    k = L2_BYTES_ALL_XCDS // max(int(row_bytes), 1)
    if E == 0 or k >= V:
        return 1.0
    indeg = csr.indeg()
    return float(np.partition(indeg, V - k)[V - k:].sum(dtype=np.int64)) / E


def lanes_per_row(d: int, dtype: torch.dtype) -> int:
    packs = -(-d // _hip.VEC_ELEMS[dtype])
    return 8 if packs <= 8 else 16 if packs <= 16 else 32 if packs <= 32 else 64


def _round_up(a: int, b: int) -> int:
    return -(-a // b) * b


MIN_SLICE_ROW_BYTES = 64


def pick_exchange(d: int, dtype: torch.dtype, world: int) -> str:
    row_bytes = d * torch.empty(0, dtype=dtype).element_size()
    return "columns" if row_bytes // max(world, 1) >= MIN_SLICE_ROW_BYTES else "halo"


def column_slice(d: int, dtype: torch.dtype, world: int, rank: int):
    vec = _hip.VEC_ELEMS[dtype]
    packs = -(-d // vec)
    base, rem = divmod(packs, world)
    p0 = rank * base + min(rank, rem)
    p1 = p0 + base + (1 if rank < rem else 0)
    return min(d, p0 * vec), min(d, p1 * vec)


RANK_QUERY_TILE = 128
RANK_CANDIDATE_TILE = 128
RANK_WORKGROUPS_PER_CU = 4
COMPUTE_UNITS = 256


def rank_slabs(n_queries: int, table_rows: int, query_tile: int = RANK_QUERY_TILE) -> int:
    q_tiles = max(1, -(-int(n_queries) // query_tile))
    tiles = max(1, -(-int(table_rows) // RANK_CANDIDATE_TILE))
    want = -(-RANK_WORKGROUPS_PER_CU * COMPUTE_UNITS // q_tiles)
    return max(1, min(want, tiles))
```

### clane_amd/xcd.py

```python
from __future__ import annotations

from typing import Optional

import numpy as np
import torch

XCD_CLASSES = 8


def xcd_class(position):
    p = position
    return (p ^ (p >> 3) ^ (p >> 6) ^ (p >> 9)) & (XCD_CLASSES - 1)


def xcd_subclass(position, row_degree, class_threshold: int, phase_threshold: int = 0, phases: int = 1):
    cls = xcd_class(position)
    if phases > 1 and phase_threshold > 0:
        cls = cls + XCD_CLASSES * (((position >> 6) % phases) * (row_degree > phase_threshold))
    return cls * (row_degree > class_threshold)


CLASS_THRESHOLD_BY_ROWS_PER_WAVE = {1: 64, 2: 64, 4: 256, 8: 256}
CLASS_CHUNK = 256
PHASES_BY_ROWS_PER_WAVE = {1: 4, 2: 2, 4: 1, 8: 1}
PHASES_UNDER_COLUMN_TILES = 0
PHASE_THRESHOLD = 512
CLASS_ITEMS_PIECE_EDGES = 1 << 28
CLASS_ITEMS_PER_BLOCK = 16



def row_pieces(rowptr: np.ndarray, max_edges: int):
    n = rowptr.size - 1
    a = 0
    while a < n:
        b = int(np.searchsorted(rowptr, rowptr[a] + max_edges, side="right")) - 1
        b = min(max(b, a + 1), n)
        yield a, b
        a = b


def class_items(rowptr: np.ndarray, colidx: np.ndarray, rows: np.ndarray, chunk: int, items_per_block: Optional[int],
                row_ids: Optional[np.ndarray] = None, colidx_dev: Optional[torch.Tensor] = None,
                phase_threshold: int = 0, phases: int = 1, mega_segment_edges: int = 0, mega_min_edges: int = 0,
                segments=None) -> dict:
    n = rows.size
    NS = XCD_CLASSES * max(1, phases)
    sizes, seg_len, seg_e0 = segments if segments is not None else \
        row_segments(rowptr, colidx, rows, colidx_dev, phase_threshold, phases)
    nchunk = -(-seg_len // chunk)
    tot = int(nchunk.sum())
    if items_per_block is None:
        items_per_block = items_per_block_for(tot)
    seg_of = np.repeat(np.arange(n * NS), nchunk)
    within = np.arange(tot, dtype=np.int64) - np.repeat(np.cumsum(nchunk) - nchunk, nchunk)
    e0 = seg_e0[seg_of] + within * chunk
    ln = np.minimum(chunk, seg_len[seg_of] - within * chunk)
    slot_ptr = np.zeros(n + 1, dtype=np.int64)
    np.cumsum(nchunk.reshape(n, NS).sum(1), out=slot_ptr[1:])
    item_cls = (seg_of % NS) % XCD_CLASSES
    heavy = sizes > phase_threshold if (phases > 1 and phase_threshold > 0) else np.zeros(n, dtype=bool)
    mega = ((sizes > mega_segment_edges * XCD_CLASSES * np.where(heavy, max(1, phases), 1)) & (sizes >= mega_min_edges)) \
        if mega_segment_edges > 0 else np.zeros(n, dtype=bool)
    item_group = np.where(heavy[seg_of // NS], (seg_of % NS) // XCD_CLASSES, max(1, phases))
    ids = (rows if row_ids is None else row_ids).astype(np.int32)
    item_row = ids[seg_of // NS]
    pieces = []
    for g in range(max(1, phases) + 1):
        in_group = item_group == g
        if not in_group.any():
            continue
        per_class = [np.nonzero(in_group & (item_cls == c))[0] for c in range(XCD_CLASSES)]
        if mega.any():
            ordered = []
            for pc in per_class:
                is_mega = mega[seg_of[pc] // NS]
                first = pc[is_mega]
                ordered.append(np.concatenate([first[np.argsort(colidx[e0[first]], kind="stable")], pc[~is_mega]]))
            per_class = ordered
        nblk = max(-(-len(pc) // items_per_block) for pc in per_class)
        flat = XCD_CLASSES * nblk * items_per_block
        g_e0 = np.zeros(flat, dtype=np.int64)
        g_len = np.zeros(flat, dtype=np.int32)
        g_slot = np.full(flat, -1, dtype=np.int32)
        g_row = np.zeros(flat, dtype=np.int32)
        for c, pc in enumerate(per_class):
            t = np.arange(len(pc))
            where = (t // items_per_block) * (XCD_CLASSES * items_per_block) + c * items_per_block + t % items_per_block
            g_e0[where], g_len[where], g_slot[where], g_row[where] = e0[pc], ln[pc], pc, item_row[pc]
        pieces.append((g_e0, g_len, g_slot, g_row))
    if not pieces:
        flat = XCD_CLASSES * items_per_block
        pieces.append((np.zeros(flat, dtype=np.int64), np.zeros(flat, dtype=np.int32),
                       np.full(flat, -1, dtype=np.int32), np.zeros(flat, dtype=np.int32)))
    out_e0, out_len, out_slot, out_row = (np.concatenate([p[i] for p in pieces]) for i in range(4))
    return {"e0": out_e0, "len": out_len, "slot": out_slot, "row": out_row, "slot_ptr": slot_ptr,
            "items_per_block": int(items_per_block)}


def row_segments(rowptr: np.ndarray, colidx: np.ndarray, rows: np.ndarray, colidx_dev: Optional[torch.Tensor] = None,
                 phase_threshold: int = 0, phases: int = 1):
    n = rows.size
    NS = XCD_CLASSES * max(1, phases)
    sizes = (rowptr[rows + 1] - rowptr[rows]).astype(np.int64)
    start = np.concatenate([[0], np.cumsum(sizes)[:-1]])
    if colidx_dev is not None and colidx_dev.is_cuda:
        dev = colidx_dev.device
        seg_len = np.empty(n * NS, dtype=np.int64)
        unsorted = False
        bounds = np.concatenate([[0], np.cumsum(sizes)])
        for a, b in row_pieces(bounds, CLASS_ITEMS_PIECE_EDGES):
            if bounds[b] == bounds[a]:
                seg_len[a * NS:b * NS] = 0
                continue
            sizes_t = torch.from_numpy(sizes[a:b]).to(dev)
            rid = torch.repeat_interleave(torch.arange(b - a, device=dev), sizes_t)
            idx = (torch.from_numpy(rowptr[rows[a:b]] - (start[a:b] - bounds[a])).to(dev)[rid]
                   + torch.arange(int(bounds[b] - bounds[a]), device=dev))
            sub = xcd_subclass(colidx_dev[idx].long(), sizes_t[rid], 0, phase_threshold, phases)
            key = rid * NS + sub
            unsorted = unsorted or (bool((key[1:] < key[:-1]).any()) if key.numel() > 1 else False)
            seg_len[a * NS:b * NS] = torch.bincount(key, minlength=(b - a) * NS).cpu().numpy()
    else:
        idx = np.repeat(rowptr[rows] - start, sizes) + np.arange(int(sizes.sum()), dtype=np.int64)
        rid = np.repeat(np.arange(n, dtype=np.int64), sizes)
        sub = xcd_subclass(colidx[idx].astype(np.int64), sizes[rid], 0, phase_threshold, phases)
        unsorted = idx.size > 1 and bool((np.diff(rid * NS + sub) < 0).any())
        seg_len = np.bincount(rid * NS + sub, minlength=n * NS)
    if unsorted:
        raise AssertionError("class rows must have their edges sorted by (xcd_subclass(column), column)")
    seg_e0 = np.repeat(rowptr[rows], NS) + (np.cumsum(seg_len) - seg_len - np.repeat(start, NS))
    return sizes, seg_len.astype(np.int64), seg_e0


def items_per_block_for(n_items: int) -> int:
    return int(min(CLASS_ITEMS_PER_BLOCK, max(4, 4 * -(-n_items // (4 * 4096)))))


OWNED_MAX_EDGES = 512
OWNED_ROW_EDGES = 1024
OWNED_GROUPS = 256
OWNED_BLOCK_THREADS = 1024
OWNED_LDS_BYTES = 152 * 1024
OWNED_LOADS = 12
OWNED_DEFAULT = True
FUSED_TILES_DEFAULT = ("row", "class", "owned")
UNIFORM_WEIGHTS_DEFAULT = "auto"
OWNED_EPILOGUE_AHEAD = True


def owned_plan(sizes: np.ndarray, seg_len: np.ndarray, seg_e0: np.ndarray, row_ids: np.ndarray, row_parts: np.ndarray,
               *, row_edges: int, groups: int, batch_vrows: int) -> Optional[dict]:
    n = int(sizes.size)
    if n == 0:
        return None
    if groups < 1 or row_edges < 64:
        raise ValueError("owned_plan: groups must be >= 1 and row_edges >= 64")
    NS = seg_len.size // n
    seg_len = seg_len.reshape(n, NS).astype(np.int64)
    seg_e0 = seg_e0.reshape(n, NS).astype(np.int64)
    keys = np.nonzero(seg_len.sum(0) > 0)[0]
    if keys.size == 0:
        keys = np.zeros(1, dtype=np.int64)
    S = int(keys.size)
    seg_len, seg_e0 = seg_len[:, keys], seg_e0[:, keys]
    nv = np.maximum(1, -(-sizes // row_edges)).astype(np.int64)
    while True:
        over = (-(-seg_len // nv[:, None])).sum(1) > row_edges
        if not over.any():
            break
        nv[over] += 1
    if int(nv.max()) > batch_vrows:
        raise ValueError(f"owned_plan: a row of {int(nv.max())} virtual rows does not fit a batch of {batch_vrows}")
    row_cum = np.cumsum(seg_len, 1).astype(np.float64)
    share = np.maximum(row_cum.sum(0) / groups, 1.0)
    row_cum /= share
    cum = np.zeros((groups, S))
    group_of = np.empty(n, dtype=np.int64)
    dealt = np.argsort(-sizes, kind="stable")
    for i in dealt.tolist():
        g = int((cum + row_cum[i]).max(1).argmin())
        group_of[i] = g
        cum[g] += row_cum[i]
    order = dealt[np.argsort(group_of[dealt], kind="stable")]
    g_sorted, nv_sorted = group_of[order], nv[order]
    bat_of_row = np.empty(n, dtype=np.int64)
    b, used, g_prev = -1, 0, -1
    for j, (g, k) in enumerate(zip(g_sorted.tolist(), nv_sorted.tolist())):
        if g != g_prev or used + k > batch_vrows:
            b, used, g_prev = b + 1, 0, g
        used += k
        bat_of_row[j] = b
    B = b + 1
    bat_row_ptr = np.zeros(B + 1, dtype=np.int64)
    np.cumsum(np.bincount(bat_of_row, minlength=B), out=bat_row_ptr[1:])
    row_vptr = np.zeros(n + 1, dtype=np.int64)
    np.cumsum(nv_sorted, out=row_vptr[1:])
    bat_vrow_ptr = row_vptr[bat_row_ptr]
    bat_group = g_sorted[bat_row_ptr[:-1]]
    grp_bat_ptr = np.zeros(groups + 1, dtype=np.int64)
    np.cumsum(np.bincount(bat_group, minlength=groups), out=grp_bat_ptr[1:])
    nvirt = int(row_vptr[-1])
    v_row = np.repeat(np.arange(n), nv_sorted)
    v_j = np.arange(nvirt) - row_vptr[v_row]
    L, E0, NV = seg_len[order][v_row], seg_e0[order][v_row], nv_sorted[v_row][:, None]
    lo = (v_j[:, None] * L) // NV
    hi = ((v_j[:, None] + 1) * L) // NV
    v_len, v_e0 = hi - lo, E0 + lo
    v_idx, s_idx = np.nonzero(v_len > 0)
    v_bat = bat_of_row[v_row]
    key = v_bat[v_idx] * S + s_idx
    by = np.lexsort((v_idx, key))
    v_idx, s_idx, key = v_idx[by], s_idx[by], key[by]
    bat_seg_ptr = np.zeros(B * S + 1, dtype=np.int64)
    np.cumsum(np.bincount(key, minlength=B * S), out=bat_seg_ptr[1:])
    group_step = np.zeros((groups, S), dtype=np.int64)
    np.add.at(group_step, (g_sorted[v_row][v_idx], s_idx), v_len[v_idx, s_idx])
    i32 = lambda a: np.ascontiguousarray(a, dtype=np.int32)
    return {"grp_bat_ptr": i32(grp_bat_ptr), "bat_vrow_ptr": i32(bat_vrow_ptr), "bat_row_ptr": i32(bat_row_ptr),
            "bat_seg_ptr": i32(bat_seg_ptr), "seg_e0": np.ascontiguousarray(v_e0[v_idx, s_idx], dtype=np.int64),
            "seg_len": i32(v_len[v_idx, s_idx]), "seg_vrow": i32(v_idx - bat_vrow_ptr[v_bat[v_idx]]),
            "row_id": i32(row_ids[order]), "row_part": i32(row_parts[order]), "row_vptr": i32(row_vptr),
            "n_groups": int(groups), "n_steps": S, "max_batch_vrows": int(np.diff(bat_vrow_ptr).max()),
            "steps": keys.astype(np.int64), "group_step_edges": group_step}
```

### include/clane_hip.h

```cpp
#ifndef CLANE_HIP_H_
#define CLANE_HIP_H_

#include <stdint.h>

#ifdef __cplusplus
extern "C" {
#endif

#define CLANE_ABI_VERSION 5

#define CLANE_OK 0
#define CLANE_ERR_INVALID_ARGUMENT (-1)
#define CLANE_ERR_LAUNCH (-2)

#define CLANE_SCORE_REFERENCE 0
#define CLANE_SCORE_PER_EDGE 1
#define CLANE_SCORE_RAW_DOT 2

#define CLANE_SCORE_FUSE_SOFTMAX 1
#define CLANE_SCORE_ROW_PARTS(n) (((n) & 0xff) << 8)

#define CLANE_SPMM_SINKS_UNTOUCHED 1
#define CLANE_SPMM_TABLE_BEYOND_CACHE 2

// ... 132 lines not shown
                                double *delta_partials, void *stream);
int clane_spmm_update_class_bf16(const int32_t *colidx, const float *P, const int64_t *item_e0, const int32_t *item_len,
                                 const int32_t *item_slot, int64_t n_blocks, int32_t items_per_block,
                                 const int32_t *class_rows, const int64_t *slot_ptr, int64_t n_rows, int64_t row0,
                                 const uint16_t *Z_old, int64_t ldz, const uint16_t *X, int64_t ldx, float gamma,
                                 uint16_t *Z_new, int64_t ldo, int32_t d, int32_t flags, float *slab, const clane_mirror_t *mirror,
                                 double *delta_partials, void *stream);

#define CLANE_OWNED_LOADS(n) (((n) & 0xff) << 8)
#define CLANE_OWNED_EPILOGUE_AHEAD (1 << 16)
typedef struct {
    const int32_t *grp_bat_ptr;
    const int32_t *bat_vrow_ptr;
    const int32_t *bat_row_ptr;
    const int32_t *bat_seg_ptr;
    const int64_t *seg_e0;
    const int32_t *seg_len;
    const int32_t *seg_vrow;
    const int32_t *row_id;
    const int32_t *row_part;
    const int32_t *row_vptr;
    int32_t n_groups;
    int32_t n_steps;
    int32_t chunk;
    int32_t max_batch_vrows;
} clane_owned_plan_t;
int clane_spmm_update_owned_f32(const int32_t *colidx, const float *P, const clane_owned_plan_t *plan,
                                int32_t block_threads, int64_t row0, const float *Z_old, int64_t ldz, const float *X,
                                int64_t ldx, float gamma, float *Z_new, int64_t ldo, int32_t d, int32_t flags,
                                double *delta_partials, void *stream);

int clane_spmm_update_tiles_f32(const int64_t *rowptr, const int32_t *colidx, const float *P, int64_t nrows, int64_t row0,
                                const float *Z_old, int64_t ldz, const float *X, int64_t ldx, float gamma, float *Z_new,
                                int64_t ldo, int32_t d, int32_t tile_cols, int64_t long_threshold, int32_t flags,
                                double *delta_partials, int64_t partials_tile_stride, void *stream);
int clane_spmm_update_class_tiles_f32(const int32_t *colidx, const float *P, const int64_t *item_e0,
                                      const int32_t *item_len, const int32_t *item_slot, int64_t n_blocks,
                                      int32_t items_per_block, const int32_t *class_rows, const int64_t *slot_ptr,
                                      int64_t n_rows, int64_t n_slots, int64_t row0, const float *Z_old, int64_t ldz,
                                      const float *X, int64_t ldx, float gamma, float *Z_new, int64_t ldo, int32_t d,
                                      int32_t tile_cols, int32_t flags, float *slab, double *delta_partials,
                                      int64_t partials_tile_stride, void *stream);
int clane_spmm_update_owned_tiles_f32(const int32_t *colidx, const float *P, const clane_owned_plan_t *plan,
                                      int32_t block_threads, int64_t row0, const float *Z_old, int64_t ldz,
                                      const float *X, int64_t ldx, float gamma, float *Z_new, int64_t ldo, int32_t d,
                                      int32_t tile_cols, int32_t flags, double *delta_partials,
                                      int64_t partials_tile_stride, void *stream);

int clane_row_weight_f32(const int64_t *rowptr, const float *P, int64_t nrows, float *row_weight, int32_t *mixed,
                         void *stream);
int clane_row_weight_f64(const int64_t *rowptr, const double *P, int64_t nrows, double *row_weight, int32_t *mixed,
                         void *stream);
int clane_spmm_update_rw_f32(const int64_t *rowptr, const int32_t *colidx, const float *row_weight, int64_t nrows,
                             int64_t row0, const float *Z_old, int64_t ldz, const float *X, int64_t ldx, float gamma,
                             float *Z_new, int64_t ldo, int32_t d, int64_t long_threshold, int32_t flags,
                             double *delta_partials, void *stream);
int clane_spmm_update_tiles_rw_f32(const int64_t *rowptr, const int32_t *colidx, const float *row_weight, int64_t nrows,
                                   int64_t row0, const float *Z_old, int64_t ldz, const float *X, int64_t ldx, float gamma,
                                   float *Z_new, int64_t ldo, int32_t d, int32_t tile_cols, int64_t long_threshold,
                                   int32_t flags, double *delta_partials, int64_t partials_tile_stride, void *stream);
int clane_spmm_update_class_rw_f32(const int32_t *colidx, const float *row_weight, const int64_t *item_e0,
                                   const int32_t *item_len, const int32_t *item_slot, const int32_t *item_row,
                                   int64_t n_blocks, int32_t items_per_block, const int32_t *class_rows,
                                   const int64_t *slot_ptr, int64_t n_rows, int64_t row0, const float *Z_old, int64_t ldz,
                                   const float *X, int64_t ldx, float gamma, float *Z_new, int64_t ldo, int32_t d,
                                   int32_t flags, float *slab, double *delta_partials, void *stream);
int clane_spmm_update_class_tiles_rw_f32(const int32_t *colidx, const float *row_weight, const int64_t *item_e0,
                                         const int32_t *item_len, const int32_t *item_slot, const int32_t *item_row,
                                         int64_t n_blocks, int32_t items_per_block, const int32_t *class_rows,
                                         const int64_t *slot_ptr, int64_t n_rows, int64_t n_slots, int64_t row0,
                                         const float *Z_old, int64_t ldz, const float *X, int64_t ldx, float gamma,
                                         float *Z_new, int64_t ldo, int32_t d, int32_t tile_cols, int32_t flags,
                                         float *slab, double *delta_partials, int64_t partials_tile_stride,
                                         void *stream);
int clane_spmm_update_owned_rw_f32(const int32_t *colidx, const float *row_weight, const clane_owned_plan_t *plan,
                                   const int32_t *seg_row, int32_t block_threads, int64_t row0, const float *Z_old,
                                   int64_t ldz, const float *X, int64_t ldx, float gamma, float *Z_new, int64_t ldo,
                                   int32_t d, int32_t flags, double *delta_partials, void *stream);
int clane_spmm_update_owned_tiles_rw_f32(const int32_t *colidx, const float *row_weight, const clane_owned_plan_t *plan,
                                         const int32_t *seg_row, int32_t block_threads, int64_t row0, const float *Z_old,
                                         int64_t ldz, const float *X, int64_t ldx, float gamma, float *Z_new, int64_t ldo,
                                         int32_t d, int32_t tile_cols, int32_t flags, double *delta_partials,
                                         int64_t partials_tile_stride, void *stream);

int clane_reduce_partials(const double *partials, int64_t n, double *ws, double *out, void *stream);

int clane_l1_distance_f32(const float *A, int64_t lda, const float *B, int64_t ldb, int64_t nrows, int32_t d,
                          float *sq_a, double *ws, double *out, void *stream);
int clane_l1_distance_f64(const double *A, int64_t lda, const double *B, int64_t ldb, int64_t nrows, int32_t d,
                          double *sq_a, double *ws, double *out, void *stream);
int clane_l1_distance_bf16(const uint16_t *A, int64_t lda, const uint16_t *B, int64_t ldb, int64_t nrows, int32_t d,
                           float *sq_a, double *ws, double *out, void *stream);

int clane_gather_rows_f32(const float *src, int64_t lds, const int32_t *idx, int64_t n, int32_t d, float *dst,
                          int64_t ldd, void *stream);
int clane_gather_rows_f64(const double *src, int64_t lds, const int32_t *idx, int64_t n, int32_t d, double *dst,
                          int64_t ldd, void *stream);
int clane_gather_rows_bf16(const uint16_t *src, int64_t lds, const int32_t *idx, int64_t n, int32_t d, uint16_t *dst,
                           int64_t ldd, void *stream);

int clane_pair_cosine_f32(const float *A, int64_t lda, const float *B, int64_t ldb, int64_t nrows, int32_t d,
                          float *out, double *ws, void *stream);
int clane_pair_cosine_f64(const double *A, int64_t lda, const double *B, int64_t ldb, int64_t nrows, int32_t d,
                          double *out, double *ws, void *stream);

int clane_project_rows_f32(const float *Z, int64_t rows, int32_t d, int64_t ldz, const float *W, float *Y, int64_t ldy,
                           void *stream);
int clane_project_rows_f64(const double *Z, int64_t rows, int32_t d, int64_t ldz, const double *W, double *Y,
                           int64_t ldy, void *stream);
int clane_project_rows_bf16(const uint16_t *Z, int64_t rows, int32_t d, int64_t ldz, const float *W, float *Y,
                            int64_t ldy, void *stream);

int clane_edge_score_pair_f32(const int64_t *rowptr, const int32_t *colidx, int64_t nrows, int64_t row0, const float *S,
                              int64_t lds, const float *N, int64_t ldn, int32_t d, float *scores, int32_t flags,
                              int64_t long_threshold, const int32_t *long_rows, int64_t n_long, void *stream);
int clane_edge_score_pair_f64(const int64_t *rowptr, const int32_t *colidx, int64_t nrows, int64_t row0,
                              const double *S, int64_t lds, const double *N, int64_t ldn, int32_t d, double *scores,
                              int32_t flags, int64_t long_threshold, const int32_t *long_rows, int64_t n_long,
                              void *stream);
int clane_edge_score_class_pair_f32(const int64_t *rowptr, const int32_t *colidx, const int64_t *item_e0,
                                    const int32_t *item_len, const int32_t *item_slot, const int32_t *item_row,
                                    int64_t n_blocks, int32_t items_per_block, const int32_t *class_rows,
                                    const int64_t *slot_ptr, int64_t n_rows, int64_t row0, const float *S, int64_t lds,
                                    const float *N, int64_t ldn, int32_t d, float *scores, int32_t flags, float *stats,
                                    void *stream);
int clane_edge_score_class_pair_f64(const int64_t *rowptr, const int32_t *colidx, const int64_t *item_e0,
                                    const int32_t *item_len, const int32_t *item_slot, const int32_t *item_row,
                                    int64_t n_blocks, int32_t items_per_block, const int32_t *class_rows,
                                    const int64_t *slot_ptr, int64_t n_rows, int64_t row0, const double *S,
                                    int64_t lds, const double *N, int64_t ldn, int32_t d, double *scores,
                                    int32_t flags, double *stats, void *stream);

int clane_pair_project_f32(const float *Z, int64_t table_rows, int32_t d, int64_t ldz, const int32_t *src,
                           const int32_t *dst, int64_t B, const float *W, float *A, float *Bm, void *stream);
int clane_pair_project_f64(const double *Z, int64_t table_rows, int32_t d, int64_t ldz, const int32_t *src,
                           const int32_t *dst, int64_t B, const double *W, double *A, double *Bm, void *stream);
int clane_pair_project_bf16(const uint16_t *Z, int64_t table_rows, int32_t d, int64_t ldz, const int32_t *src,
                            const int32_t *dst, int64_t B, const float *W, float *A, float *Bm, void *stream);
int clane_pair_loss_f32(const float *A, const float *Bm, int64_t B, int32_t d, const uint8_t *linked, const float *u,
                        float *g, uint8_t *mask, double *ws, double *stats, void *stream);
int clane_pair_loss_f64(const double *A, const double *Bm, int64_t B, int32_t d, const uint8_t *linked, const double *u,
                        double *g, uint8_t *mask, double *ws, double *stats, void *stream);
int64_t clane_pair_grad_ws_len(int64_t B, int32_t d);
int clane_pair_grad_f32(const float *Z, int64_t table_rows, int32_t d, int64_t ldz, const int32_t *src,
                        const int32_t *dst, int64_t B, const float *A, const float *Bm, const float *g,
                        const double *stats, float *ws, float *dW, void *stream);
int clane_pair_grad_f64(const double *Z, int64_t table_rows, int32_t d, int64_t ldz, const int32_t *src,
                        const int32_t *dst, int64_t B, const double *A, const double *Bm, const double *g,
                        const double *stats, double *ws, double *dW, void *stream);
int clane_pair_grad_bf16(const uint16_t *Z, int64_t table_rows, int32_t d, int64_t ldz, const int32_t *src,
                         const int32_t *dst, int64_t B, const float *A, const float *Bm, const float *g,
                         const double *stats, float *ws, float *dW, void *stream);
int clane_adam_step_f32(float *W, float *m, float *v, const float *dW, int64_t n, double lr, const double *stats,
                        double *state, void *stream);
int clane_adam_step_f64(double *W, double *m, double *v, const double *dW, int64_t n, double lr, const double *stats,
                        double *state, void *stream);
int clane_pair_labels(const int64_t *rowptr, const int32_t *colidx, int64_t nrows, const int32_t *src,
                      const int32_t *dst, int64_t B, uint8_t *linked, void *stream);

#define CLANE_RANK_MAX_K 32
int clane_rank_scores_f32(const float *S, int64_t lds, const float *N, int64_t ldn, int64_t table_rows, int32_t d,
                          const int32_t *q_rows, int64_t Q, int32_t mode, const double *sums2, const float *sq,
                          const int32_t *label, const int64_t *excl_rowptr, const int32_t *excl_colidx,
                          int32_t exclude_self, int32_t k, int32_t n_slabs, float *cand_score, int32_t *cand_id,
                          void *stream);
int clane_rank_scores_f64(const double *S, int64_t lds, const double *N, int64_t ldn, int64_t table_rows, int32_t d,
// ... 241 lines not shown
```

Measured before the change: 289.3 sweeps/s.

## Add held-rows SpMM path keeping mid-degree row accumulators in LDS per block

Adds a 'held' variant of the owned-rows SpMM update kernel for 32-lane-per-row tiles (d or tile width up to 128), which processes two rows per wave instruction. Rows in a degree band below the class threshold are assigned to groups with a capacity limit so their accumulators stay resident in LDS. A held_cutoff heuristic picks that band, and localize gains a separate sort threshold. The aim is to cut scattered slab/partial traffic and launch fragmentation for mid-degree rows. In exchange it adds planner complexity, capacity constraints that can raise errors, and another kernel instance with its own load-depth choices.

```diff
diff --git a/clane_amd/_hip.py b/clane_amd/_hip.py
--- a/clane_amd/_hip.py
+++ b/clane_amd/_hip.py
@@ -83,6 +83,8 @@
     C.c_int, [_p, _p, _p, _p, _i32, _i64, _p, _i64, _p, _i64, C.c_float, _p, _i64, _i32, _i32, _p, _p])
 SIGNATURES["clane_spmm_update_owned_tiles_rw_f32"] = (
     C.c_int, [_p, _p, _p, _p, _i32, _i64, _p, _i64, _p, _i64, C.c_float, _p, _i64, _i32, _i32, _i32, _p, _i64, _p])
+for _s in ("", "_tiles", "_rw", "_tiles_rw"):
+    SIGNATURES[f"clane_spmm_update_held{_s}_f32"] = SIGNATURES[f"clane_spmm_update_owned{_s}_f32"]
 for _s in ("f32", "f64"):
     SIGNATURES[f"clane_degree_weighted_sums_{_s}"] = (C.c_int, [_p, _p, _p, _i64, _p, _p, _p])
     SIGNATURES[f"clane_edge_score_finalize_{_s}"] = (C.c_int, [_p, _p, _i64, _i64, _i32, _p, _p, _p, _p])
@@ -639,6 +641,13 @@
                           partials, beyond_cache: bool = False, loads: int = 0, ahead: bool = False):
         raise NotImplementedError(f"{type(self).__name__} has no spmm_update_owned")
 
+    def has_spmm_held(self, dtype, d: int) -> bool:
+        return False
+
+    def spmm_update_held(self, colidx, P, plan, block_threads: int, row0: int, Z_old, X, gamma: float, Z_new, d: int,
+                         partials, beyond_cache: bool = False, loads: int = 0, ahead: bool = False):
+        raise NotImplementedError(f"{type(self).__name__} has no spmm_update_held")
+
     def has_spmm_tiles(self, dtype, d: int, tile_cols: int) -> bool:
         return False
 
@@ -1061,6 +1070,60 @@
                      zo, ldz, xp, ldx, gamma, zn, ldo, d, tile_cols,
                      self._spmm_flags(beyond_cache=beyond_cache, loads=loads, ahead=ahead),
                      _vec(partials, torch.float64, "partials"), partials_stride, self._stream(Z_old))
+
+    HELD_LOADS = (0, 4, 8)
+
+    def has_spmm_held(self, dtype, d: int) -> bool:
+        return dtype == torch.float32 and 64 < d <= 128
+
+    def _held(self, form: str, colidx, P, plan: OwnedPlan, block_threads: int, row0: int, Z_old, X, gamma: float, Z_new,
+              d: int, tile, partials, stride, beyond_cache: bool, loads: int, ahead: bool):
+        name = "spmm_update_held" + form
+        rw = form.endswith("_rw")
+        if loads not in self.HELD_LOADS:
+            raise ValueError(f"{name}: no instance with {loads} row loads in flight")
+        if not (64 <= int(block_threads) <= 1024 and int(block_threads) % 64 == 0):
+            raise ValueError(f"{name}: block_threads must be a multiple of 64 in [64, 1024]")
+        if tile:
+            zo, ldz, xp, ldx, zn, ldo = self._tile_args(name, Z_old, X, Z_new, d, tile[0], partials, stride[0],
+                                                        plan.max_part + 1)
+        else:
+            zo, ldz, xp, ldx, zn, ldo = self._tables(name, Z_old, X, Z_new, f32_only=True)
+        width = tile[0] if tile else d
+        if not self.has_spmm_held(torch.float32, width):
+            raise ValueError(f"{name}: no held instance for rows or tiles of {width} columns")
+        self._owned_plan_fits(name, plan, width, colidx, colidx if rw else P, row0, Z_old, X, Z_new,
+                              None if tile else partials)
+        weights = ((self._row_weights(name, P, plan.max_row + 1), C.cast(C.pointer(plan.c), _p),
+                    _vec(plan.seg_row, torch.int32, "seg_row")) if rw
+                   else (_vec(P, torch.float32, "P"), C.cast(C.pointer(plan.c), _p)))
+        self._invoke(getattr(self.lib, f"clane_{name}_f32"), f"clane_{name}", _vec(colidx, torch.int32, "colidx"),
+                     *weights, int(block_threads), row0, zo, ldz, xp, ldx, gamma, zn, ldo, d, *tile,
+                     self._spmm_flags(beyond_cache=beyond_cache, loads=loads, ahead=ahead),
+                     _vec(partials, torch.float64, "partials"), *stride, self._stream(Z_old))
+
+    def spmm_update_held(self, colidx, P, plan: OwnedPlan, block_threads: int, row0: int, Z_old, X, gamma: float, Z_new,
+                         d: int, partials, beyond_cache: bool = False, loads: int = 0, ahead: bool = False):
+        self._held("", colidx, P, plan, block_threads, row0, Z_old, X, gamma, Z_new, d, (), partials, (), beyond_cache,
+                   loads, ahead)
+
+    def spmm_update_held_tiles(self, colidx, P, plan: OwnedPlan, block_threads: int, row0: int, Z_old, X, gamma: float,
+                               Z_new, d: int, tile_cols: int, partials, partials_stride: int, beyond_cache: bool = False,
+                               loads: int = 0, ahead: bool = False):
+        self._held("_tiles", colidx, P, plan, block_threads, row0, Z_old, X, gamma, Z_new, d, (tile_cols,), partials,
+                   (partials_stride,), beyond_cache, loads, ahead)
+
+    def spmm_update_held_rw(self, colidx, row_weight, plan: OwnedPlan, block_threads: int, row0: int, Z_old, X,
+                            gamma: float, Z_new, d: int, partials, beyond_cache: bool = False, loads: int = 0,
+                            ahead: bool = False):
+        self._held("_rw", colidx, row_weight, plan, block_threads, row0, Z_old, X, gamma, Z_new, d, (), partials, (),
+                   beyond_cache, loads, ahead)
+
+    def spmm_update_held_tiles_rw(self, colidx, row_weight, plan: OwnedPlan, block_threads: int, row0: int, Z_old, X,
+                                  gamma: float, Z_new, d: int, tile_cols: int, partials, partials_stride: int,
+                                  beyond_cache: bool = False, loads: int = 0, ahead: bool = False):
+        self._held("_tiles_rw", colidx, row_weight, plan, block_threads, row0, Z_old, X, gamma, Z_new, d, (tile_cols,),
+                   partials, (partials_stride,), beyond_cache, loads, ahead)
 
     def reduce_partials(self, partials, n: int, ws, out):
         self._invoke(self.lib.clane_reduce_partials, "clane_reduce_partials",
diff --git a/clane_amd/blocks.py b/clane_amd/blocks.py
--- a/clane_amd/blocks.py
+++ b/clane_amd/blocks.py
@@ -30,6 +30,11 @@
     seg_row: torch.Tensor
 
 
+class HeldRows(NamedTuple):
+    plan: object
+    n_rows: int
+
+
 class OwnedRows(NamedTuple):
     plan: object
     rest: Optional[ClassItems]
@@ -44,18 +49,24 @@
     split: int
     klass: int
     end: int
+    held: Optional[int] = None
 
     @classmethod
-    def of(cls, row_pass: int, n_mid: int, n_hub: int, n_split: int, n_class: int, length: int) -> "PartialLayout":
-        starts = list(itertools.accumulate((row_pass, n_mid, n_hub, n_split, n_class), initial=0))
+    def of(cls, row_pass: int, n_mid: int, n_hub: int, n_split: int, n_class: int, length: int,
+           n_held: int = 0) -> "PartialLayout":
+        starts = list(itertools.accumulate((row_pass, n_mid, n_hub, n_split, n_class, n_held), initial=0))
         assert starts[-1] == length, (starts, length)
-        return cls(*starts)
+        return cls(*starts[:5], starts[6], starts[5] if n_held else None)
+
+    @property
+    def class_end(self) -> int:
+        return self.end if self.held is None else self.held
 
     def owned(self, n_rest: int) -> int:
         return self.klass + n_rest
 
     def owned_slots(self, n_rest: int, n_owned: int) -> np.ndarray:
-        assert self.owned(n_rest) + n_owned == self.end, (self, n_rest, n_owned)
+        assert self.owned(n_rest) + n_owned == self.class_end, (self, n_rest, n_owned)
         return self.owned(n_rest) - self.klass + np.arange(n_owned)
 
 
@@ -71,3 +82,5 @@
     n_slots: int = 0
     owned: Optional[OwnedRows] = None
     owned_inputs: Optional[tuple] = None
+    held: Optional[HeldRows] = None
+    held_inputs: Optional[tuple] = None
diff --git a/clane_amd/csrc/clane_abi.hip b/clane_amd/csrc/clane_abi.hip
--- a/clane_amd/csrc/clane_abi.hip
+++ b/clane_amd/csrc/clane_abi.hip
@@ -57,6 +57,9 @@
 #endif
 #ifndef CLANE_CLASS_U16B
 #define CLANE_CLASS_U16B 4
+#endif
+#ifndef CLANE_HELD_U
+#define CLANE_HELD_U 8
 #endif
 #ifndef CLANE_CLASS_U32
 #define CLANE_CLASS_U32 6
@@ -598,7 +601,7 @@
 constexpr int64_t kLdsPerCU = 160 * 1024;
 constexpr int64_t kLdsDefaultLimit = 64 * 1024;
 
-template <typename T, typename PT, bool UNIFORM = false>
+template <typename T, typename PT, bool UNIFORM = false, bool HELD = false>
 int spmm_update_owned_impl(const char *what, const int32_t *colidx, const PT *P, const clane_owned_plan_t *plan,
                            int32_t block_threads, int64_t row0, const Tables<T> &t, Tiles tiles, bool fused, int32_t flags,
                            double *delta_partials, void *stream, const int32_t *seg_row = nullptr) {
@@ -624,6 +627,7 @@
     const Layout L = t.layout(d);
     REQUIRE(L.vec && (L.lpr == 32 || L.lpr == 64) && d <= L.lpr * Elem<T>::kVec,
             "spmm_update_owned: no instance for d=%d with these operands (16-byte packs, 17..64 packs per row)", d);
+    if constexpr (HELD) REQUIRE(L.lpr == 32, "%s: no instance for d=%d (17..32 packs per row: two rows per instruction)", what, d);
     const int64_t lds = int64_t(plan->max_batch_vrows) * L.lpr * Elem<T>::kVec * int64_t(sizeof(A));
     REQUIRE(lds + kOwnedLdsReserve <= kLdsPerCU, "spmm_update_owned: %lld virtual rows per batch need %lld bytes of LDS",
             (long long)plan->max_batch_vrows, (long long)lds);
@@ -633,7 +637,10 @@
     const bool beyond = (flags & CLANE_SPMM_TABLE_BEYOND_CACHE) != 0;
     int rc = CLANE_OK;
     auto launch = [&]<int VEC, int LPR, int U>() {
-        auto *kernel = spmm_owned_kernel<T, PT, VEC, LPR, U, UNIFORM>;
+        auto *kernel = [] {
+            if constexpr (HELD) return spmm_held_kernel<T, PT, VEC, LPR, U, UNIFORM>;
+            else return spmm_owned_kernel<T, PT, VEC, LPR, U, UNIFORM>;
+        }();
         if (lds > kLdsDefaultLimit) {
             static int64_t granted = 0;
             if (lds > granted) {
@@ -653,16 +660,22 @@
     };
     constexpr int KV = Elem<T>::kVec;
     const int asked = (flags >> 8) & 0xff;
-    REQUIRE(asked == 0 || asked == 8 || asked == 12 || (L.lpr == 32 && asked == 6),
-            "spmm_update_owned: no instance with %d row loads in flight", asked);
-    const int loads = asked ? asked : (L.lpr == 32 && beyond) ? CLANE_CLASS_U32 : CLANE_LONG_U;
-    if (L.lpr == 32) {
-        if (loads == 6) launch.template operator()<KV, 32, 6>();
-        else if (loads == 12) launch.template operator()<KV, 32, 12>();
+    if constexpr (HELD) {
+        REQUIRE(asked == 0 || asked == 4 || asked == 8, "%s: no instance with %d row loads in flight", what, asked);
+        if ((asked ? asked : CLANE_HELD_U) == 4) launch.template operator()<KV, 32, 4>();
         else launch.template operator()<KV, 32, 8>();
     } else {
-        if (loads == 12) launch.template operator()<KV, 64, 12>();
-        else launch.template operator()<KV, 64, 8>();
+        REQUIRE(asked == 0 || asked == 8 || asked == 12 || (L.lpr == 32 && asked == 6),
+                "spmm_update_owned: no instance with %d row loads in flight", asked);
+        const int loads = asked ? asked : (L.lpr == 32 && beyond) ? CLANE_CLASS_U32 : CLANE_LONG_U;
+        if (L.lpr == 32) {
+            if (loads == 6) launch.template operator()<KV, 32, 6>();
+            else if (loads == 12) launch.template operator()<KV, 32, 12>();
+            else launch.template operator()<KV, 32, 8>();
+        } else {
+            if (loads == 12) launch.template operator()<KV, 64, 12>();
+            else launch.template operator()<KV, 64, 8>();
+        }
     }
     if (rc != CLANE_OK) return rc;
     return check_launch(what);
@@ -1727,6 +1740,41 @@
                                                       row0, TABLES(float), Tiles{tile_cols, partials_tile_stride}, true,
                                                       flags, delta_partials, stream, seg_row);
 }
+int clane_spmm_update_held_f32(const int32_t *colidx, const float *P, const clane_owned_plan_t *plan,
+                               int32_t block_threads, int64_t row0, const float *Z_old, int64_t ldz, const float *X,
+                               int64_t ldx, float gamma, float *Z_new, int64_t ldo, int32_t d, int32_t flags,
+                               double *delta_partials, void *stream) {
+    return spmm_update_owned_impl<float, float, false, true>("spmm_update_held", colidx, P, plan, block_threads, row0,
+                                                             TABLES(float), Tiles{d, 0}, false, flags, delta_partials,
+                                                             stream);
+}
+int clane_spmm_update_held_tiles_f32(const int32_t *colidx, const float *P, const clane_owned_plan_t *plan,
+                                     int32_t block_threads, int64_t row0, const float *Z_old, int64_t ldz,
+                                     const float *X, int64_t ldx, float gamma, float *Z_new, int64_t ldo, int32_t d,
+                                     int32_t tile_cols, int32_t flags, double *delta_partials,
+                                     int64_t partials_tile_stride, void *stream) {
+    return spmm_update_owned_impl<float, float, false, true>("spmm_update_held_tiles", colidx, P, plan, block_threads,
+                                                             row0, TABLES(float), Tiles{tile_cols, partials_tile_stride},
+                                                             true, flags, delta_partials, stream);
+}
+int clane_spmm_update_held_rw_f32(const int32_t *colidx, const float *row_weight, const clane_owned_plan_t *plan,
+                                  const int32_t *seg_row, int32_t block_threads, int64_t row0, const float *Z_old,
+                                  int64_t ldz, const float *X, int64_t ldx, float gamma, float *Z_new, int64_t ldo,
+                                  int32_t d, int32_t flags, double *delta_partials, void *stream) {
+    return spmm_update_owned_impl<float, float, true, true>("spmm_update_held_rw", colidx, row_weight, plan,
+                                                            block_threads, row0, TABLES(float), Tiles{d, 0}, false, flags,
+                                                            delta_partials, stream, seg_row);
+}
+int clane_spmm_update_held_tiles_rw_f32(const int32_t *colidx, const float *row_weight, const clane_owned_plan_t *plan,
+                                        const int32_t *seg_row, int32_t block_threads, int64_t row0, const float *Z_old,
+                                        int64_t ldz, const float *X, int64_t ldx, float gamma, float *Z_new, int64_t ldo,
+                                        int32_t d, int32_t tile_cols, int32_t flags, double *delta_partials,
+                                        int64_t partials_tile_stride, void *stream) {
+    return spmm_update_owned_impl<float, float, true, true>("spmm_update_held_tiles_rw", colidx, row_weight, plan,
+                                                            block_threads, row0, TABLES(float),
+                                                            Tiles{tile_cols, partials_tile_stride}, true, flags,
+                                                            delta_partials, stream, seg_row);
+}
 
 int64_t clane_spmm_class_slab_len(int64_t n_slots, int32_t d) { return n_slots * (ceil_div(d, 8) * 8); }
 int64_t clane_spmm_split_slab_len(int64_t n_segments, int32_t d) { return n_segments * (ceil_div(d, 8) * 8); }
diff --git a/clane_amd/csrc/spmm_update.h b/clane_amd/csrc/spmm_update.h
--- a/clane_amd/csrc/spmm_update.h
+++ b/clane_amd/csrc/spmm_update.h
@@ -903,6 +903,103 @@
     int chunk;
 };
 
+template <typename T, int VEC, int LPR>
+__device__ __forceinline__ void owned_epilogue(const OwnedPlan &plan, int b, int v0,
+                                               const typename Elem<T>::acc_t *s_sum, int64_t row0,
+                                               const T *__restrict__ Zold, int64_t ldz, const T *__restrict__ X, int64_t ldx,
+                                               typename Elem<T>::acc_t gamma, T *__restrict__ Znew, int64_t ldo, bool col_ok,
+                                               bool ahead, bool nt_store, double *__restrict__ partials) {
+    using A = typename Elem<T>::acc_t;
+    constexpr int W = LPR * VEC;
+    constexpr int kRows = kWave / LPR;
+    const int lane = lane_id();
+    const int wave = __builtin_amdgcn_readfirstlane(threadIdx.x / kWave);
+    const int nwaves = int(blockDim.x) / kWave;
+    const int sub = lane / LPR, sl = lane % LPR;
+    const int c0 = sl * VEC;
+    const int r0 = plan.bat_row_ptr[b];
+    const int nr = plan.bat_row_ptr[b + 1] - r0;
+    if (ahead) {
+        struct RowIds {
+            int r, va, vb, part;
+            bool live;
+        };
+        const int stride = nwaves * kRows;
+        auto ids_of = [&](int j0) -> RowIds {
+            RowIds m{0, 0, 0, 0, false};
+            const int j = j0 + sub;
+            if (j0 < nr && j < nr) {
+                m.r = plan.row_id[r0 + j];
+                m.va = plan.row_vptr[r0 + j] - v0;
+                m.vb = plan.row_vptr[r0 + j + 1] - v0;
+                m.part = plan.row_part[r0 + j];
+                m.live = true;
+            }
+            return m;
+        };
+        auto request = [&](const RowIds &m, Pack<T, VEC> &x, Pack<T, VEC> &zo) {
+            if (m.live && col_ok) {
+                x = load_pack_stream<T, VEC>(X + int64_t(m.r) * ldx + c0);
+                zo = load_pack_stream<T, VEC>(Zold + (row0 + m.r) * ldz + c0);
+            }
+        };
+        int j0 = wave * kRows;
+        RowIds cur = ids_of(j0), nxt = ids_of(j0 + stride);
+        Pack<T, VEC> x{}, zo{};
+        request(cur, x, zo);
+        for (; j0 < nr; j0 += stride) {
+            const RowIds far = ids_of(j0 + 2 * stride);
+            Pack<T, VEC> xn{}, zon{};
+            request(nxt, xn, zon);
+            A rsum = A(0);
+            if (cur.live && col_ok) {
+                A acc[VEC];
+                const Pack<A, VEC> first = load_pack<A, VEC>(s_sum + cur.va * W + c0);
+#pragma unroll
+                for (int k = 0; k < VEC; ++k) acc[k] = first.v[k];
+                for (int v = cur.va + 1; v < cur.vb; ++v) {
+                    const Pack<A, VEC> t = load_pack<A, VEC>(s_sum + v * W + c0);
+#pragma unroll
+                    for (int k = 0; k < VEC; ++k) acc[k] += t.v[k];
+                }
+                Pack<T, VEC> out{};
+                rsum = finish_pack<T, VEC>(x, zo, acc, gamma, true, Znew + int64_t(cur.r) * ldo + c0, out, nt_store);
+            }
+            rsum = group_sum<LPR>(rsum);
+            if (cur.live && sl == 0) partials[cur.part] = double(rsum);
+            cur = nxt;
+            nxt = far;
+            x = xn;
+            zo = zon;
+        }
+    } else
+    for (int j0 = wave * kRows; j0 < nr; j0 += nwaves * kRows) {
+        const int j = j0 + sub;
+        const bool live = j < nr;
+        const bool ok = live && col_ok;
+        A rsum = A(0);
+        if (ok) {
+            const int64_t r = plan.row_id[r0 + j];
+            const Pack<T, VEC> x = load_pack_stream<T, VEC>(X + r * ldx + c0);
+            const Pack<T, VEC> zo = load_pack_stream<T, VEC>(Zold + (row0 + r) * ldz + c0);
+            const int va = plan.row_vptr[r0 + j] - v0, vb = plan.row_vptr[r0 + j + 1] - v0;
+            A acc[VEC];
+            const Pack<A, VEC> first = load_pack<A, VEC>(s_sum + va * W + c0);
+#pragma unroll
+            for (int k = 0; k < VEC; ++k) acc[k] = first.v[k];
+            for (int v = va + 1; v < vb; ++v) {
+                const Pack<A, VEC> t = load_pack<A, VEC>(s_sum + v * W + c0);
+#pragma unroll
+                for (int k = 0; k < VEC; ++k) acc[k] += t.v[k];
+            }
+            Pack<T, VEC> out{};
+            rsum = finish_pack<T, VEC>(x, zo, acc, gamma, true, Znew + r * ldo + c0, out, nt_store);
+        }
+        rsum = group_sum<LPR>(rsum);
+        if (live && sl == 0) partials[plan.row_part[r0 + j]] = double(rsum);
+    }
+}
+
 template <typename T, typename PT, int VEC, int LPR, int U, bool UNIFORM = false>
 __global__ __launch_bounds__(kOwnedMaxBlock) void spmm_owned_kernel(
     const int32_t *__restrict__ colidx, const PT *__restrict__ P, OwnedPlan plan, int64_t row0,
@@ -911,14 +1008,11 @@
     double *__restrict__ partials, [[maybe_unused]] const int32_t *__restrict__ seg_row) {
     using A = typename Elem<T>::acc_t;
     constexpr int W = LPR * VEC;
-    constexpr int kRows = kWave / LPR;
     extern __shared__ __align__(16) unsigned char s_owned_raw[];
     A *s_sum = reinterpret_cast<A *>(s_owned_raw);
     __shared__ int s_cnt[kOwnedMaxSteps];
 
     const int lane = lane_id();
-    const int wave = __builtin_amdgcn_readfirstlane(threadIdx.x / kWave);
-    const int nwaves = int(blockDim.x) / kWave;
     const int sub = lane / LPR, sl = lane % LPR;
     const int c0 = sl * VEC;
     const int n_steps = plan.n_steps;
@@ -992,87 +1086,145 @@
             }
             __syncthreads();
         }
-        const int r0 = plan.bat_row_ptr[b];
-        const int nr = plan.bat_row_ptr[b + 1] - r0;
-        if (ahead) {
-            struct RowIds {
-                int r, va, vb, part;
-                bool live;
+        owned_epilogue<T, VEC, LPR>(plan, b, v0, s_sum, row0, Zold, ldz, X, ldx, gamma, Znew, ldo, col_ok, ahead, nt_store,
+                                    partials);
+        __syncthreads();
+    }
+    }
+}
+
+template <typename T, typename PT, int VEC, int LPR, int U, bool UNIFORM = false>
+__global__ __launch_bounds__(kOwnedMaxBlock) void spmm_held_kernel(
+    const int32_t *__restrict__ colidx, const PT *__restrict__ P, OwnedPlan plan, int64_t row0,
+    const T *__restrict__ Zold, int64_t ldz, const T *__restrict__ X, int64_t ldx, typename Elem<T>::acc_t gamma,
+    T *__restrict__ Znew, int64_t ldo, int d_left, int tile_cols, int64_t part_stride, bool ahead, bool nt_store,
+    double *__restrict__ partials, [[maybe_unused]] const int32_t *__restrict__ seg_row) {
+    using A = typename Elem<T>::acc_t;
+    static_assert(LPR < kWave, "held rows are walked by sub-waves");
+    static_assert(LPR % U == 0, "a sub-wave's edge buffer is consumed in whole groups of U");
+    constexpr int W = LPR * VEC;
+    extern __shared__ __align__(16) unsigned char s_held_raw[];
+    A *s_sum = reinterpret_cast<A *>(s_held_raw);
+    __shared__ int s_cnt[kOwnedMaxSteps];
+
+    const int lane = lane_id();
+    const int sl = lane % LPR;
+    const int sub_base = lane - sl;
+    const int c0 = sl * VEC;
+    const int n_steps = plan.n_steps;
+    const int b0 = plan.grp_bat_ptr[blockIdx.x], b1 = plan.grp_bat_ptr[blockIdx.x + 1];
+
+    for (; d_left > 0; d_left -= tile_cols, Zold += tile_cols, X += tile_cols, Znew += tile_cols, partials += part_stride) {
+    const int d = d_left < tile_cols ? d_left : tile_cols;
+    const bool col_ok = c0 < d;
+    const T *zcol = Zold + (col_ok ? c0 : 0);
+    for (int b = b0; b < b1; ++b) {
+        const int v0 = plan.bat_vrow_ptr[b];
+        const int nv = plan.bat_vrow_ptr[b + 1] - v0;
+        for (int i = threadIdx.x; i < nv * W; i += int(blockDim.x)) s_sum[i] = A(0);
+        if (int(threadIdx.x) < n_steps) s_cnt[threadIdx.x] = 0;
+        __syncthreads();
+        for (int s = 0; s < n_steps; ++s) {
+            const int sa = plan.bat_seg_ptr[b * n_steps + s];
+            const int n = plan.bat_seg_ptr[b * n_steps + s + 1] - sa;
+            auto claim = [&]() -> int {
+                int v = 0;
+                if (sl == 0) v = atomicAdd(&s_cnt[s], 1);
+                return lane_get(v, sub_base);
             };
-            const int stride = nwaves * kRows;
-            auto ids_of = [&](int j0) -> RowIds {
-                RowIds m{0, 0, 0, 0, false};
-                const int j = j0 + sub;
-                if (j0 < nr && j < nr) {
-                    m.r = plan.row_id[r0 + j];
-                    m.va = plan.row_vptr[r0 + j] - v0;
-                    m.vb = plan.row_vptr[r0 + j + 1] - v0;
-                    m.part = plan.row_part[r0 + j];
-                    m.live = true;
-                }
-                return m;
+            int nxt = 0, n_len = 0, n_vr = 0, n_c = 0;
+            int64_t n_e0 = 0;
+            A n_p = A(0);
+            auto request = [&]() {
+                nxt = claim();
+                n_e0 = 0, n_len = 0, n_vr = 0, n_c = 0, n_p = A(0);
+                if (nxt < n) {
+                    n_e0 = plan.seg_e0[sa + nxt];
+                    n_len = plan.seg_len[sa + nxt];
+                    n_vr = plan.seg_vrow[sa + nxt];
+                    if constexpr (UNIFORM) n_p = A(P[seg_row[sa + nxt]]);
+                    if (sl < n_len) {
+                        n_c = colidx[n_e0 + sl];
+                        if constexpr (!UNIFORM) n_p = A(P[n_e0 + sl]);
+                    }
+                }
             };
-            auto request = [&](const RowIds &m, Pack<T, VEC> &x, Pack<T, VEC> &zo) {
-                if (m.live && col_ok) {
-                    x = load_pack_stream<T, VEC>(X + int64_t(m.r) * ldx + c0);
-                    zo = load_pack_stream<T, VEC>(Zold + (row0 + m.r) * ldz + c0);
-                }
-            };
-            int j0 = wave * kRows;
-            RowIds cur = ids_of(j0), nxt = ids_of(j0 + stride);
-            Pack<T, VEC> x{}, zo{};
-            request(cur, x, zo);
-            for (; j0 < nr; j0 += stride) {
-                const RowIds far = ids_of(j0 + 2 * stride);
-                Pack<T, VEC> xn{}, zon{};
-                request(nxt, xn, zon);
-                A rsum = A(0);
-                if (cur.live && col_ok) {
-                    A acc[VEC];
-                    const Pack<A, VEC> first = load_pack<A, VEC>(s_sum + cur.va * W + c0);
-#pragma unroll
-                    for (int k = 0; k < VEC; ++k) acc[k] = first.v[k];
-                    for (int v = cur.va + 1; v < cur.vb; ++v) {
-                        const Pack<A, VEC> t = load_pack<A, VEC>(s_sum + v * W + c0);
-#pragma unroll
-                        for (int k = 0; k < VEC; ++k) acc[k] += t.v[k];
+            request();
+            bool have = false, done = false;
+            int64_t e_next = 0, e_end = 0;
+            int nbuf = 0, pos = 0, c = 0, vr = 0;
+            A p = A(0);
+            A acc[VEC];
+#pragma unroll
+            for (int k = 0; k < VEC; ++k) acc[k] = A(0);
+            for (;;) {
+                if (pos >= nbuf && !done) {
+                    if (e_next == e_end) {
+                        if (have) {
+                            if (col_ok) {
+                                A *sum = s_sum + vr * W + c0;
+                                Pack<A, VEC> t = load_pack<A, VEC>(sum);
+#pragma unroll
+                                for (int k = 0; k < VEC; ++k) t.v[k] += acc[k];
+                                store_pack<A, VEC>(sum, t);
+                            }
+                            have = false;
+                        }
+                        pos = 0, nbuf = 0, c = 0;
+                        if constexpr (!UNIFORM) p = A(0);
+                        if (nxt >= n) {
+                            done = true;
+                        } else {
+                            e_next = n_e0;
+                            e_end = n_e0 + n_len;
+                            vr = n_vr;
+                            c = n_c;
+                            p = n_p;
+                            nbuf = n_len < LPR ? n_len : LPR;
+                            e_next += nbuf;
+#pragma unroll
+                            for (int k = 0; k < VEC; ++k) acc[k] = A(0);
+                            have = true;
+                            request();
+                        }
+                    } else {
+                        const int64_t left = e_end - e_next;
+                        nbuf = left < LPR ? int(left) : LPR;
+                        pos = 0, c = 0;
+                        if constexpr (!UNIFORM) p = A(0);
+                        if (sl < nbuf) {
+                            c = colidx[e_next + sl];
+                            if constexpr (!UNIFORM) p = A(P[e_next + sl]);
+                        }
+                        e_next += nbuf;
                     }
-                    Pack<T, VEC> out{};
-                    rsum = finish_pack<T, VEC>(x, zo, acc, gamma, true, Znew + int64_t(cur.r) * ldo + c0, out, nt_store);
-                }
-                rsum = group_sum<LPR>(rsum);
-                if (cur.live && sl == 0) partials[cur.part] = double(rsum);
-                cur = nxt;
-                nxt = far;
-                x = xn;
-                zo = zon;
-            }
-        } else
-        for (int j0 = wave * kRows; j0 < nr; j0 += nwaves * kRows) {
-            const int j = j0 + sub;
-            const bool live = j < nr;
-            const bool ok = live && col_ok;
-            A rsum = A(0);
-            if (ok) {
-                const int64_t r = plan.row_id[r0 + j];
-                const Pack<T, VEC> x = load_pack_stream<T, VEC>(X + r * ldx + c0);
-                const Pack<T, VEC> zo = load_pack_stream<T, VEC>(Zold + (row0 + r) * ldz + c0);
-                const int va = plan.row_vptr[r0 + j] - v0, vb = plan.row_vptr[r0 + j + 1] - v0;
-                A acc[VEC];
-                const Pack<A, VEC> first = load_pack<A, VEC>(s_sum + va * W + c0);
-#pragma unroll
-                for (int k = 0; k < VEC; ++k) acc[k] = first.v[k];
-                for (int v = va + 1; v < vb; ++v) {
-                    const Pack<A, VEC> t = load_pack<A, VEC>(s_sum + v * W + c0);
-#pragma unroll
-                    for (int k = 0; k < VEC; ++k) acc[k] += t.v[k];
-                }
-                Pack<T, VEC> out{};
-                rsum = finish_pack<T, VEC>(x, zo, acc, gamma, true, Znew + r * ldo + c0, out, nt_store);
-            }
-            rsum = group_sum<LPR>(rsum);
-            if (live && sl == 0) partials[plan.row_part[r0 + j]] = double(rsum);
-        }
+                }
+                if (__all(done)) break;
+                Pack<T, VEC> z[U];
+                A pj[U];
+#pragma unroll
+                for (int u = 0; u < U; ++u) {
+                    const int src = sub_base + ((pos + u) & (LPR - 1));
+                    const int cj = lane_get(c, src);
+                    if constexpr (UNIFORM) pj[u] = pos + u < nbuf ? p : A(0);
+                    else pj[u] = lane_get(p, src);
+                    z[u] = load_pack<T, VEC>(zcol + int64_t(cj) * ldz);
+                }
+#pragma unroll
+                for (int u = 0; u < U; ++u) {
+#pragma unroll
+                    for (int k = 0; k < VEC; ++k) {
+                        A zv = Elem<T>::to_acc(z[u].v[k]);
+                        zv = pj[u] != A(0) ? zv : A(0);
+                        acc[k] = fma(pj[u], zv, acc[k]);
+                    }
+                }
+                pos += U;
+            }
+            __syncthreads();
+        }
+        owned_epilogue<T, VEC, LPR>(plan, b, v0, s_sum, row0, Zold, ldz, X, ldx, gamma, Znew, ldo, col_ok, ahead, nt_store,
+                                    partials);
         __syncthreads();
     }
     }
diff --git a/clane_amd/diagnostics.py b/clane_amd/diagnostics.py
--- a/clane_amd/diagnostics.py
+++ b/clane_amd/diagnostics.py
@@ -84,6 +84,8 @@
                 **({"owned_ahead": True} if getattr(self, "class_owned", False) and getattr(self, "owned_ahead", False)
                    else {}),
                 **({"uniform_weights": True} if self._sweeps_read_row_weights() else {}),
+                **({"held_rows": True, "held_min_edges": self.held_min_edges, "held_loads": self.held_loads}
+                   if getattr(self, "held_rows", False) else {}),
                 }
 
     def exchange_bytes_per_sweep(self) -> int:
diff --git a/clane_amd/engine.py b/clane_amd/engine.py
--- a/clane_amd/engine.py
+++ b/clane_amd/engine.py
@@ -13,11 +13,11 @@
 from .comm import TorchComm
 from .diagnostics import DiagnosticsMixin
 from .halo import build_halo_layout
-from .partition import Block, HostCSR, LocalCSR, RowPartition, localize
+from .partition import Block, HostCSR, LocalCSR, RowPartition, local_outdeg, localize
 from .plan import (HEAVY_ROW_EDGES, HUB_FACTOR, INFINITY_CACHE_BYTES, L2_BYTES_ALL_XCDS,
                    LONG_THRESHOLD_BY_ROWS_PER_WAVE, MIN_HOT_READ_SHARE, MIN_SEGMENT_EDGES, MIN_SLICE_ROW_BYTES,
                    SOFTMAX_EDGES_PER_WORKGROUP, SPLIT_EDGES, TARGET_SEGMENTS, UNSKEWED_LONG_THRESHOLD, _round_up,
-                   column_slice, hot_read_share, lanes_per_row, pick_exchange)
+                   column_slice, held_cutoff, hot_read_share, lanes_per_row, pick_exchange)
 from .staging import StagedZ, StagingMixin, place_piece
 from .xcd import (CLASS_CHUNK, CLASS_THRESHOLD_BY_ROWS_PER_WAVE, PHASE_THRESHOLD, PHASES_BY_ROWS_PER_WAVE,
                   class_items)
@@ -41,7 +41,7 @@
                  owned_groups: int = xcd.OWNED_GROUPS, owned_lds_bytes: int = xcd.OWNED_LDS_BYTES,
                  owned_block_threads: int = xcd.OWNED_BLOCK_THREADS, owned_chunk: Optional[int] = None,
                  owned_loads: int = xcd.OWNED_LOADS, owned_ahead: Optional[bool] = None, fused_tiles=None,
-                 uniform_weights=None):
+                 uniform_weights=None, held_rows: Optional[bool] = None, held_loads: int = xcd.HELD_LOADS):
         if X.dim() != 2 or X.shape[0] != csr.num_vertices:
             raise ValueError(f"X must be [V, d] with V={csr.num_vertices}, got {tuple(X.shape)}")
         if cosine_mode not in ("reference", "per_edge"):
@@ -67,6 +67,7 @@
         self.owned_ahead = bool(ahead and self.k.owned_epilogue_ahead)
         self._choose_fused_tiles(fused_tiles)
         self._choose_uniform(uniform_weights)
+        self._choose_held(held_rows, held_loads)
         self._build_layout(csr, chunks, shuffle, seed, hot_rows_first)
         self._choose_row_bins(long_threshold, hub_threshold)
         deg = self._upload_structure()
@@ -172,6 +173,22 @@
         if self.class_owned:
             self._check_owned_settings()
 
+    def _choose_held(self, held_rows, loads) -> None:
+        self.held_possible = owned.held_possible(self)
+        want = (xcd.HELD_DEFAULT and self.beyond_cache and self.class_affinity) if held_rows is None else bool(held_rows)
+        self.held_rows = bool(want and self.held_possible)
+        self.held_loads, self.held_min_edges, self.held_batch_rows = int(loads), 0, 0
+        if self.held_rows:
+            if self.held_loads not in (4, 8):
+                raise ValueError("held_loads must be 4 or 8")
+            self._check_owned_settings()
+            self._check_held_settings()
+
+    def _check_held_settings(self) -> None:
+        self.held_batch_rows = self._lds_bytes // 512
+        if self.held_batch_rows < 1 or self._lds_bytes > _hip.OWNED_LDS_LIMIT:
+            raise ValueError(f"owned_lds_bytes must hold one sum of 512 bytes and stay within {_hip.OWNED_LDS_LIMIT}")
+
     FUSED_PASSES = ("row", "class", "owned")
 
     def _choose_fused_tiles(self, asked) -> None:
@@ -257,8 +274,15 @@
             self.part = RowPartition.create(self.V, self.row_world, self.row_rank, chunks, live_mask=live, shuffle=shuffle,
                                             seed=seed, priority=hot)
             self.blocks = self.part.blocks(spans_for_one_rank=self._forced and not self.columns)
+            if self.held_rows:
+                deg = local_outdeg(csr, self.part)
+                self.held_min_edges = held_cutoff([deg[b.local_start:b.local_start + b.nrows] for b in self.blocks],
+                                                  self.class_threshold, self.owned_groups * self.held_batch_rows)
+                if self.held_min_edges >= self.class_threshold:
+                    self.held_rows, self.held_min_edges = False, 0
             self.local = localize(csr, self.part, self.device, class_threshold=self.class_threshold,
-                                  phase_threshold=self.phase_threshold, phases=self.class_phases)
+                                  phase_threshold=self.phase_threshold, phases=self.class_phases,
+                                  sort_threshold=self.held_min_edges if self.held_rows else None)
         if self.part.padded_vertices >= 2 ** 31:
             raise ValueError(f"{self.part.padded_vertices} table rows: column indices are 32-bit (ABI v1); divide the "
                              "rows over more GPUs (exchange='halo') or wait for 64-bit indices")
@@ -279,7 +303,13 @@
         if self.class_threshold:
             long_threshold = min(long_threshold, self.class_threshold) if long_threshold > 0 else self.class_threshold
         self.long_threshold = int(long_threshold)
+        self.row_pass_threshold = self._row_pass_stop(self.held_rows)
         self.hub_threshold = int(hub_threshold) if hub_threshold is not None else HUB_FACTOR * self.long_threshold
+
+    def _row_pass_stop(self, held_on: bool) -> int:
+        if not held_on:
+            return self.long_threshold
+        return min(self.long_threshold, self.held_min_edges) if self.long_threshold > 0 else self.held_min_edges
 
     def _upload_structure(self) -> np.ndarray:
         dev = self.device
@@ -316,9 +346,12 @@
             k1_long = (db > self.k1_threshold) & ~(is_class if self.class_k1 else np.zeros_like(is_class)) \
                 if self.k1_threshold > 0 else np.zeros_like(is_class)
             rows_c, rows_s = np.nonzero(is_class)[0], np.nonzero(is_split)[0]
+            rows_h = np.nonzero((db > self.held_min_edges) & (db <= self.class_threshold) & ~is_long)[0] \
+                if self.held_min_edges > 0 else np.empty(0, dtype=np.int64)
             layout = PartialLayout.of(row_pass=self.k.spmm_partials_len(b.nrows, 0), n_mid=int(is_mid.sum()),
                                       n_hub=int(is_hub.sum()), n_split=rows_s.size, n_class=rows_c.size,
-                                      length=self.k.spmm_partials_len(b.nrows, int(is_long.sum())))
+                                      length=self.k.spmm_partials_len(b.nrows, int(is_long.sum()) + rows_h.size),
+                                      n_held=rows_h.size)
             rows = BlockRows(long=to_dev(np.nonzero(db > self.score_threshold)[0] if self.score_threshold > 0
                                          else np.empty(0, dtype=np.int64)),
                              k1_long=to_dev(np.nonzero(k1_long)[0]), mid=to_dev(np.nonzero(is_mid)[0]),
@@ -338,6 +371,9 @@
                     rows.owned = owned.plan_block(self, layout, *rows.owned_inputs)
                 rows.klass, rows.n_slots = ClassItems.upload(items, rows_c, dev), int(items["slot_ptr"][-1])
                 max_slots = max(max_slots, rows.n_slots)
+            if rows_h.size:
+                rows.held_inputs = (rows_h, rows_h + b.local_start)
+                rows.held = owned.plan_held(self, layout, *rows.held_inputs)
             if rows_s.size:
                 nseg = -(-db[rows_s] // self.segment_edges)
                 seg_ptr = np.zeros(rows_s.size + 1, dtype=np.int64)
@@ -360,6 +396,7 @@
     long_rows, k1_long_rows = _per_block("long"), _per_block("k1_long")
     mid_rows, hub_rows, split_rows = _per_block("mid"), _per_block("hub"), _per_block("split")
     class_rows, class_slots, owned_rows = _per_block("klass"), _per_block("n_slots"), _per_block("owned")
+    held_plans = _per_block("held")
     del _per_block
 
     @property
@@ -383,6 +420,39 @@
             self._check_owned_settings()
         for r in self.block_rows:
             r.owned = owned.plan_block(self, r.partials, *r.owned_inputs) if on and r.owned_inputs is not None else None
+        self._plans = {}
+
+    def set_held(self, on: bool, **settings) -> None:
+        if self.held_min_edges == 0:
+            if on:
+                raise ValueError("this engine holds no rows: build it with held_rows=True (one GPU, fp32, column tiles "
+                                 "of 65..128 elements, rows that fit one batch)")
+            return
+        if self.device.type == "cuda":
+            torch.cuda.synchronize(self.device)
+        for name, value in settings.items():
+            if name == "lds_bytes":
+                self._lds_bytes = int(value)
+            elif name == "loads":
+                self.held_loads = int(value)
+            elif name in ("groups", "block_threads"):
+                setattr(self, "owned_" + name, int(value))
+            else:
+                raise TypeError(f"set_held: unknown setting {name!r}")
+        if on and settings:
+            if self.held_loads not in (4, 8):
+                raise ValueError("held_loads must be 4 or 8")
+            self._check_owned_settings()
+            self._check_held_settings()
+        if on and ("groups" in settings or "lds_bytes" in settings):
+            for r in self.block_rows:
+                if r.held_inputs is not None:
+                    if r.held_inputs[0].size > self.owned_groups * self.held_batch_rows:
+                        raise ValueError("set_held: the held rows no longer fit one batch per group")
+                    r.held = owned.plan_held(self, r.partials, *r.held_inputs)
+        self.held_rows = bool(on)
+        self.row_pass_threshold = self._row_pass_stop(self.held_rows)
+        self.partials.zero_()
         self._plans = {}
 
     def _setup_exchange(self, deg: np.ndarray, fused_pack: bool) -> None:
@@ -710,17 +780,20 @@
                         "spmm_update_long", rp, self.colidx, self.P, listed, waves, b.row0, v.Zold, v.X, gamma, v.Znew, v.d,
                         p, mirror=mir))[1], [])
                 own, split = rows.owned, rows.split
+                held = rows.held if self.held_rows else None
                 klass = rows.klass if own is None else own.rest
                 own_all, own_t = over_tiles("owned", own, lay.klass, lambda v, p: owned.bind_launch(
                     self, own.plan, b.row0, v, gamma, p, w))
+                held_all, held_t = over_tiles("owned", held, lay.held, lambda v, p: owned.bind_held(
+                    self, held.plan, b.row0, v, gamma, p, w))
                 class_all, class_t = over_tiles("class", klass, lay.klass, lambda v, p: fused.bind_class(
                     self, klass, b.row0, v, gamma, slab, p, mir, w))
                 _, split_t = over_tiles(None, split, lay.split, lambda v, p: self._bind(
                     "spmm_update_split", rp, self.colidx, self.P, split.rows, split.seg_ptr, split.seg_row,
                     self.segment_edges, b.row0, v.Zold, v.X, gamma, v.Znew, v.d, slab, p, mirror=mir))
-                steps += own_all + class_all
+                steps += own_all + held_all + class_all
                 for t in range(T):
-                    steps += own_t[t] + class_t[t] + split_t[t]
+                    steps += own_t[t] + held_t[t] + class_t[t] + split_t[t]
                 steps.append(("event", i, 4))
                 steps += long_rows(rows.hub, 16, lay.hub)
                 steps.append(("event", i, 1))
diff --git a/clane_amd/fused.py b/clane_amd/fused.py
--- a/clane_amd/fused.py
+++ b/clane_amd/fused.py
@@ -33,7 +33,7 @@
 def bind_row(eng, rowptr, nrows: int, row0: int, v: Tables, gamma: float, partials, mirror=None, w=None):
     assert w is None or mirror is None
     return eng._bind(v.method("spmm_update", w), rowptr, eng.colidx, eng.P if w is None else w, nrows, row0, v.Zold, v.X,
-                     gamma, v.Znew, v.d, *v.cols, eng.long_threshold, partials, *v.strides, sinks_untouched=True,
+                     gamma, v.Znew, v.d, *v.cols, eng.row_pass_threshold, partials, *v.strides, sinks_untouched=True,
                      **({} if w is not None else v.mirrored(mirror)), beyond_cache=eng.beyond_cache)
 
 
diff --git a/clane_amd/owned.py b/clane_amd/owned.py
--- a/clane_amd/owned.py
+++ b/clane_amd/owned.py
@@ -5,7 +5,8 @@
 import numpy as np
 
 from . import xcd
-from .blocks import ClassItems, OwnedRows, PartialLayout
+from .blocks import ClassItems, HeldRows, OwnedRows, PartialLayout
+from .plan import lanes_per_row
 
 
 def possible(eng) -> bool:
@@ -43,3 +44,28 @@
     return eng._bind(v.method("spmm_update_owned", w), eng.colidx, eng.P if w is None else w, plan,
                      eng.owned_block_threads, row0, v.Zold, v.X, gamma, v.Znew, v.d, *v.cols, partials, *v.strides,
                      beyond_cache=eng.beyond_cache, loads=eng.owned_loads, **ahead)
+
+
+def held_possible(eng) -> bool:
+    widths = [c1 - c0 for c0, c1 in eng.tiles]
+    return bool(possible(eng) and all(lanes_per_row(w, eng.dtype) == 32 and eng.k.has_spmm_held(eng.dtype, w)
+                                      for w in widths))
+
+
+def plan_held(eng, layout: PartialLayout, rows_h: np.ndarray, rows_abs: np.ndarray) -> Optional[HeldRows]:
+    if rows_h.size == 0:
+        return None
+    segments = xcd.row_segments(eng.local.rowptr, eng.local.colidx, rows_abs, getattr(eng, "colidx", None))
+    plan = xcd.owned_plan(*segments, rows_h, np.arange(rows_h.size), row_edges=max(eng.class_threshold, 64),
+                          groups=eng.owned_groups, batch_vrows=eng.held_batch_rows, group_vrows=eng.held_batch_rows)
+    if int(np.diff(plan["grp_bat_ptr"]).max()) != 1 or plan["row_vptr"][-1] != rows_h.size:
+        raise AssertionError("held rows: every group takes its rows in exactly one batch, one sum per row")
+    eng.held_balance = plan["group_step_edges"]
+    return HeldRows(eng.k.make_owned_plan(plan, eng.owned_chunk, eng.device), int(rows_h.size))
+
+
+def bind_held(eng, plan, row0: int, v, gamma: float, partials, w=None):
+    ahead = {"ahead": True} if getattr(eng, "owned_ahead", False) else {}
+    return eng._bind(v.method("spmm_update_held", w), eng.colidx, eng.P if w is None else w, plan,
+                     eng.owned_block_threads, row0, v.Zold, v.X, gamma, v.Znew, v.d, *v.cols, partials, *v.strides,
+                     beyond_cache=eng.beyond_cache, loads=eng.held_loads, **ahead)
diff --git a/clane_amd/partition.py b/clane_amd/partition.py
--- a/clane_amd/partition.py
+++ b/clane_amd/partition.py
@@ -163,6 +163,14 @@
 LOCALIZE_PIECE_EDGES = 1 << 28
 
 
+def local_outdeg(csr: HostCSR, part: RowPartition) -> np.ndarray:
+    pos = part.position_of_vertex()
+    vertex_at = np.full(part.padded_vertices, -1, dtype=np.int64)
+    vertex_at[pos] = np.arange(csr.num_vertices, dtype=np.int64)
+    verts = vertex_at[part.local_positions()]
+    return np.where(verts >= 0, csr.outdeg()[np.where(verts >= 0, verts, 0)], 0).astype(np.int64)
+
+
 def edge_order(row_of, cols, sub, table_rows: int, n_sub: int = XCD_CLASSES, two_pass: Optional[bool] = None):
     import torch
     n_rows = int(row_of.max()) + 1 if row_of.numel() else 1
@@ -180,8 +188,10 @@
 
 
 def localize(csr: HostCSR, part: RowPartition, device=None, class_threshold: int = 0, phase_threshold: int = 0,
-             phases: int = 1) -> LocalCSR:
+             phases: int = 1, sort_threshold: Optional[int] = None) -> LocalCSR:
     V = csr.num_vertices
+    if sort_threshold is None:
+        sort_threshold = class_threshold
     if V != part.num_vertices:
         raise ValueError("partition built for a different vertex count")
     pos = part.position_of_vertex()
@@ -194,7 +204,7 @@
     rowptr = np.zeros(part.n_local + 1, dtype=np.int64)
     np.cumsum(deg, out=rowptr[1:])
     indeg = np.where(valid, csr.indeg()[safe], 0).astype(np.int32)
-    by_class = deg > class_threshold if class_threshold > 0 else np.zeros_like(deg, dtype=bool)
+    by_class = deg > sort_threshold if sort_threshold > 0 else np.zeros_like(deg, dtype=bool)
     identity = (part.world_size == 1 and part.chunks == 1 and not by_class.any()
                 and np.array_equal(pos, np.arange(V)))
     if identity:
@@ -215,7 +225,7 @@
         row_of = torch.repeat_interleave(torch.arange(b - a, device=dev), deg_t)
         origin = start_t[a:b][row_of] + (torch.arange(e1 - e0, device=dev) - (t(rowptr[a:b]) - e0)[row_of])
         cols = pos_t[colidx_t[origin].long()]
-        sub = (xcd_subclass(cols, deg_t[row_of], class_threshold, phase_threshold, phases)
+        sub = (xcd_subclass(cols, deg_t[row_of], class_threshold, phase_threshold, phases, sort_threshold)
                if by_class[a:b].any() else None)
         order = edge_order(row_of, cols, sub, part.padded_vertices, XCD_CLASSES * max(1, phases))
         cols_out[e0:e1] = cols[order].to(torch.int32).cpu().numpy()
diff --git a/clane_amd/plan.py b/clane_amd/plan.py
--- a/clane_amd/plan.py
+++ b/clane_amd/plan.py
@@ -17,6 +17,16 @@
 MIN_HOT_READ_SHARE = 0.2
 HEAVY_ROW_EDGES = 4096
 UNSKEWED_LONG_THRESHOLD = 128
+
+
+def held_cutoff(block_degrees, class_threshold: int, capacity: int) -> int:
+    h = 1
+    for deg in block_degrees:
+        above = np.cumsum(np.bincount(np.minimum(deg, class_threshold + 1), minlength=class_threshold + 2)[::-1])[::-1]
+        held = above[1:class_threshold + 1] - above[class_threshold + 1]
+        fits = np.nonzero(held <= capacity)[0]
+        h = max(h, int(fits[0]) if fits.size else class_threshold)
+    return min(h, class_threshold)
 
 
 def hot_read_share(csr: HostCSR, row_bytes: int) -> float:
diff --git a/clane_amd/xcd.py b/clane_amd/xcd.py
--- a/clane_amd/xcd.py
+++ b/clane_amd/xcd.py
@@ -13,11 +13,12 @@
     return (p ^ (p >> 3) ^ (p >> 6) ^ (p >> 9)) & (XCD_CLASSES - 1)
 
 
-def xcd_subclass(position, row_degree, class_threshold: int, phase_threshold: int = 0, phases: int = 1):
+def xcd_subclass(position, row_degree, class_threshold: int, phase_threshold: int = 0, phases: int = 1,
+                 sort_threshold: Optional[int] = None):
     cls = xcd_class(position)
     if phases > 1 and phase_threshold > 0:
         cls = cls + XCD_CLASSES * (((position >> 6) % phases) * (row_degree > phase_threshold))
-    return cls * (row_degree > class_threshold)
+    return cls * (row_degree > (class_threshold if sort_threshold is None else sort_threshold))
 
 
 CLASS_THRESHOLD_BY_ROWS_PER_WAVE = {1: 64, 2: 64, 4: 256, 8: 256}
@@ -147,10 +148,12 @@
 FUSED_TILES_DEFAULT = ("row", "class", "owned")
 UNIFORM_WEIGHTS_DEFAULT = "auto"
 OWNED_EPILOGUE_AHEAD = True
+HELD_DEFAULT = True
+HELD_LOADS = 8
 
 
 def owned_plan(sizes: np.ndarray, seg_len: np.ndarray, seg_e0: np.ndarray, row_ids: np.ndarray, row_parts: np.ndarray,
-               *, row_edges: int, groups: int, batch_vrows: int) -> Optional[dict]:
+               *, row_edges: int, groups: int, batch_vrows: int, group_vrows: int = 0) -> Optional[dict]:
     n = int(sizes.size)
     if n == 0:
         return None
@@ -178,10 +181,19 @@
     cum = np.zeros((groups, S))
     group_of = np.empty(n, dtype=np.int64)
     dealt = np.argsort(-sizes, kind="stable")
+    room = np.full(groups, group_vrows if group_vrows > 0 else np.iinfo(np.int64).max, dtype=np.int64)
+    if group_vrows > 0 and int(nv.sum()) > groups * group_vrows:
+        raise ValueError(f"owned_plan: {int(nv.sum())} virtual rows do not fit {groups} groups of {group_vrows}")
     for i in dealt.tolist():
-        g = int((cum + row_cum[i]).max(1).argmin())
+        load = (cum + row_cum[i]).max(1)
+        if group_vrows > 0:
+            load[room < nv[i]] = np.inf
+            if not np.isfinite(load).any():
+                raise ValueError("owned_plan: no group has room left for a row's virtual rows")
+        g = int(load.argmin())
         group_of[i] = g
         cum[g] += row_cum[i]
+        room[g] -= nv[i]
     order = dealt[np.argsort(group_of[dealt], kind="stable")]
     g_sorted, nv_sorted = group_of[order], nv[order]
     bat_of_row = np.empty(n, dtype=np.int64)
diff --git a/include/clane_hip.h b/include/clane_hip.h
--- a/include/clane_hip.h
+++ b/include/clane_hip.h
@@ -238,6 +238,25 @@
                                          int64_t ldz, const float *X, int64_t ldx, float gamma, float *Z_new, int64_t ldo,
                                          int32_t d, int32_t tile_cols, int32_t flags, double *delta_partials,
                                          int64_t partials_tile_stride, void *stream);
+
+int clane_spmm_update_held_f32(const int32_t *colidx, const float *P, const clane_owned_plan_t *plan,
+                               int32_t block_threads, int64_t row0, const float *Z_old, int64_t ldz, const float *X,
+                               int64_t ldx, float gamma, float *Z_new, int64_t ldo, int32_t d, int32_t flags,
+                               double *delta_partials, void *stream);
+int clane_spmm_update_held_tiles_f32(const int32_t *colidx, const float *P, const clane_owned_plan_t *plan,
+                                     int32_t block_threads, int64_t row0, const float *Z_old, int64_t ldz,
+                                     const float *X, int64_t ldx, float gamma, float *Z_new, int64_t ldo, int32_t d,
+                                     int32_t tile_cols, int32_t flags, double *delta_partials,
+                                     int64_t partials_tile_stride, void *stream);
+int clane_spmm_update_held_rw_f32(const int32_t *colidx, const float *row_weight, const clane_owned_plan_t *plan,
+                                  const int32_t *seg_row, int32_t block_threads, int64_t row0, const float *Z_old,
+                                  int64_t ldz, const float *X, int64_t ldx, float gamma, float *Z_new, int64_t ldo,
+                                  int32_t d, int32_t flags, double *delta_partials, void *stream);
+int clane_spmm_update_held_tiles_rw_f32(const int32_t *colidx, const float *row_weight, const clane_owned_plan_t *plan,
+                                        const int32_t *seg_row, int32_t block_threads, int64_t row0, const float *Z_old,
+                                        int64_t ldz, const float *X, int64_t ldx, float gamma, float *Z_new, int64_t ldo,
+                                        int32_t d, int32_t tile_cols, int32_t flags, double *delta_partials,
+                                        int64_t partials_tile_stride, void *stream);
 
 int clane_reduce_partials(const double *partials, int64_t n, double *ws, double *out, void *stream);
 
```

Measured after the change: 283.1 sweeps/s. 2.1% lower.
